# StarsX/FluidX12

Measured on AMD Instinct MI355X. Metric: voxel-updates/sec (advect+40 Jacobi) at 256^3; achieved HBM GB/s vs peak, higher is better.
Workload: dtype f32

## Files before the change

### fluidx12_amd/capi.py

```python
import ctypes as C
import os

from . import build as _build

FX_OK = 0
FX_E_INVALID, FX_E_DEVICE, FX_E_NOMEM, FX_E_STATE, FX_E_COMM, FX_E_HALO = -1, -2, -3, -4, -5, -6

RAY_MARCH_DIRECT, RAY_MARCH_CUBEMAP, SEPARATE_LIGHT_PASS, OPTIMIZED = 0, 1, 2, 3
FRAME_COUNT = 3
STORAGE_FP32, STORAGE_FP16 = 0, 1
JACOBI_FIXED, JACOBI_FAITHFUL = 0, 1
ADDRESS_CLAMP, ADDRESS_MIRROR = 0, 1
FLAG_JACOBI_FUSE_MASK, FLAG_NO_OVERLAP, FLAG_RENDER_ONLY = 0xF, 0x10, 0x20
OPT_OVERLAP, OPT_JACOBI_ROUND, OPT_ADAPTIVE_HALO, OPT_COUNT_SAMPLES, OPT_RENDER_ACCEL = 1, 2, 3, 4, 5
ABI_VERSION = 7
(FIELD_VELOCITY, FIELD_VELOCITY1, FIELD_COLOR, FIELD_COLOR_PREV, FIELD_PRESSURE, FIELD_DIVERGENCE,
 FIELD_LIGHTMAP, FIELD_CUBEMAP, FIELD_TARGET, FIELD_TARGET_FLOAT, FIELD_CUBE_DEPTH) = range(11)
DEPTH_DEVICE = 0x1
LIGHT_DIRECTIONAL, LIGHT_POINT = 0, 1
MAX_EMITTERS = 16
OBSTACLES_DEVICE = 0x1


class Desc(C.Structure):
    _fields_ = [("struct_size", C.c_uint32), ("grid_x", C.c_uint32), ("grid_y", C.c_uint32), ("grid_z", C.c_uint32),
                ("viewport_w", C.c_uint32), ("viewport_h", C.c_uint32), ("storage", C.c_uint32),
                ("jacobi_iters", C.c_uint32), ("jacobi_mode", C.c_uint32), ("advect_address", C.c_uint32),
                ("device", C.c_int32), ("slab_z0", C.c_uint32), ("slab_nz", C.c_uint32),
                ("halo_advect", C.c_uint32), ("halo_jacobi", C.c_uint32), ("flags", C.c_uint32)]


class FrameInfo(C.Structure):
    _fields_ = [("cube_lod", C.c_uint32), ("cube_size", C.c_uint32), ("ray_samples", C.c_uint32),
                ("visibility_mask", C.c_uint32), ("frame_parity", C.c_uint32), ("edge_pixels", C.c_float),
                ("time_step", C.c_float), ("world_view_proj_i", C.c_float * 16), ("screen_to_world", C.c_float * 16)]


class Light(C.Structure):
    _fields_ = [("struct_size", C.c_uint32), ("kind", C.c_uint32), ("position", C.c_float * 3), ("color", C.c_float * 4),
                ("ambient", C.c_float * 4)]


class Emitter(C.Structure):
    _fields_ = [("struct_size", C.c_uint32), ("flags", C.c_uint32), ("center", C.c_float * 3), ("radius", C.c_float),
                ("color_rate", C.c_float * 4), ("force", C.c_float * 3), ("swirl", C.c_float)]


class Timing(C.Structure):
    _fields_ = [("advect_ms", C.c_double), ("divergence_ms", C.c_double), ("jacobi_ms", C.c_double),
                ("project_ms", C.c_double), ("light_ms", C.c_double), ("view_ms", C.c_double),
                ("exchange_ms", C.c_double), ("steps", C.c_uint64), ("jacobi_launches", C.c_uint64),
                ("jacobi_sweeps", C.c_uint64), ("renders", C.c_uint64), ("resolve_ms", C.c_double),
                ("jacobi_main_ms", C.c_double), ("jacobi_main_launches", C.c_uint64), ("jacobi_main_sweeps", C.c_uint64),
                ("exchange_bytes", C.c_uint64), ("advect_halo_planes", C.c_uint64), ("chain_ms", C.c_double),
                ("freeze_solves", C.c_uint64), ("freeze_sweeps", C.c_uint64), ("exchange_calls", C.c_uint64),
                ("view_samples", C.c_uint64), ("light_samples", C.c_uint64), ("lightmap_fetches", C.c_uint64),
                ("freeze_strip_launches", C.c_uint64)]


_vp, _fp = C.c_void_p, C.POINTER(C.c_float)
SYMBOLS = {
    "fx_abi_version": (C.c_int, []),
    "fx_error_string": (C.c_char_p, [C.c_int]),
    "fx_create": (C.c_int, [C.POINTER(_vp), C.POINTER(Desc)]),
    "fx_destroy": (C.c_int, [_vp]),
    "fx_set_max_samples": (C.c_int, [_vp, C.c_uint32, C.c_uint32]),
    "fx_set_sh": (C.c_int, [_vp, _fp]),
    "fx_update_frame": (C.c_int, [_vp, C.c_float, C.c_uint8, _fp, _fp, _fp]),
    "fx_simulate": (C.c_int, [_vp, _vp, C.c_uint8]),
    "fx_render": (C.c_int, [_vp, _vp, C.c_uint8, C.c_uint8]),
    "fx_get_frame_info": (C.c_int, [_vp, C.POINTER(FrameInfo)]),
    "fx_synchronize": (C.c_int, [_vp]),
    "fx_last_error": (C.c_char_p, [_vp]),
    "fx_upload": (C.c_int, [_vp, C.c_int, _vp, C.c_size_t]),
    "fx_download": (C.c_int, [_vp, C.c_int, _vp, C.c_size_t]),
    "fx_field_bytes": (C.c_size_t, [_vp, C.c_int]),
    "fx_field_digest": (C.c_int, [_vp, C.c_int, C.c_uint32, C.c_uint32, C.POINTER(C.c_uint64)]),
    "fx_checkpoint_save": (C.c_int, [_vp, C.c_char_p]),
    "fx_checkpoint_load": (C.c_int, [_vp, C.c_char_p]),
    "fx_advect": (C.c_int, [_vp, _vp]),
    "fx_divergence": (C.c_int, [_vp, _vp]),
    "fx_jacobi": (C.c_int, [_vp, _vp, C.c_uint32]),
    "fx_project": (C.c_int, [_vp, _vp]),
    "fx_set_vorticity_confinement": (C.c_int, [_vp, C.c_float]),
    "fx_confine_vorticity": (C.c_int, [_vp, _vp]),
    "fx_set_emitters": (C.c_int, [_vp, C.POINTER(Emitter), C.c_uint32]),
    "fx_get_emitters": (C.c_int, [_vp, C.POINTER(Emitter), C.c_uint32, C.POINTER(C.c_uint32)]),
    "fx_set_impulse": (C.c_int, [_vp, C.c_int]),
    "fx_emit": (C.c_int, [_vp, _vp]),
    "fx_set_obstacles": (C.c_int, [_vp, _vp, _vp, C.c_size_t, C.c_uint32]),
    "fx_get_obstacles": (C.c_int, [_vp, _vp, C.c_size_t, C.POINTER(C.c_uint64)]),
    "fx_enforce_obstacles": (C.c_int, [_vp, _vp]),
    "fx_sh_transform": (C.c_int, [_vp, _fp, C.c_uint32, _fp]),
    "fx_set_environment": (C.c_int, [_vp, _fp, C.c_uint32]),
    "fx_render_environment": (C.c_int, [_vp, _vp, C.c_uint8]),
    "fx_clear_render_target": (C.c_int, [_vp, _vp, _fp]),
    "fx_render_cube": (C.c_int, [_vp, _vp, C.c_uint8]),
    "fx_set_scene_depth": (C.c_int, [_vp, _vp, _vp, C.c_uint32, C.c_uint32, C.c_float, C.c_float, C.c_uint32]),
    "fx_set_light": (C.c_int, [_vp, C.POINTER(Light)]),
    "fx_get_light": (C.c_int, [_vp, C.POINTER(Light)]),
    "fx_dds_cube_info": (C.c_int, [_vp, C.c_size_t, C.POINTER(C.c_uint32), C.POINTER(C.c_uint32)]),
    "fx_dds_decode_cube": (C.c_int, [_vp, _vp, C.c_size_t, C.c_uint32, _fp, C.c_size_t]),
    "fx_timing_enable": (C.c_int, [_vp, C.c_int]),
    "fx_set_option": (C.c_int, [_vp, C.c_uint32, C.c_uint32]),
    "fx_set_knob": (C.c_int, [C.c_char_p, C.c_char_p]),
    "fx_knob_name": (C.c_char_p, [C.c_uint32]),
    "fx_comm_gather_color": (C.c_int, [_vp, _vp, _vp, C.c_int, C.POINTER(C.c_uint32), C.POINTER(C.c_uint32)]),
    "fx_timing_read": (C.c_int, [_vp, C.POINTER(Timing), C.c_int]),
    "fx_comm_id_bytes": (C.c_size_t, []),
    "fx_comm_get_unique_id": (C.c_int, [_vp, C.c_size_t]),
    "fx_comm_init_rank": (C.c_int, [_vp, _vp, C.c_size_t, C.c_int, C.c_int]),
    "fx_comm_init_local": (C.c_int, [C.POINTER(_vp), C.c_int]),
    "fx_comm_init_peer": (C.c_int, [C.POINTER(_vp), C.c_int]),
}

_lib = None
LAB_KNOBS = {"ADVECT_BLOCK", "ADVECT_FAST", "ADVECT_LDS_HALF", "ADVECT_TILE_ROWS", "ADVECT_ZCHUNK", "BLOCK_REMAP", "BLOCK_SHAPE", "DEBUG_NO_COPY",
             "FREEZE_DENSE_LEVELS", "FREEZE_DENSE_ONE", "FREEZE_FAST", "FREEZE_FUSE_DIV", "FREEZE_NT", "FREEZE_SHRINK", "FREEZE_T", "FREEZE_WGS",
             "JACOBI2D_TILE", "JACOBI_BLOCK", "JACOBI_BLOCKG", "LIGHT_FILL_DIRTY", "LIGHT_RAY_NT", "LIGHT_RAY_WGS", "OBSTACLE_V4", "PROJECT_V4", "ROW_VW",
             "STRIP3H_PAIRS", "STRIP3_COOP", "STRIP3_NO512", "STRIP3_OFF", "STRIP3_ZCHUNK", "STRIP4T", "STRIP4T_256", "STRIP4T_512", "STRIP4T_FROM", "STRIP4T_GRID", "STRIP4T_NARROW", "STRIP4T_NARROW_FROM", "STRIP4T_PIECES", "STRIP4X", "STRIP4X_MINP", "STRIP4X_NT", "STRIP4X_ORDER", "STRIP4X_WGS",
             "STRIP4_OCTET", "STRIP4_ZCHUNK", "STRIP4_ZFLOOR", "STRIP_GENERIC", "STRIP_R", "STRIP_REMAP", "STRIP_WGS", "STRIP_WIDE", "STRIP_ZCHUNK", "VIEW_ORDER", "VIEW_WGS", "VORT_ZCHUNK", "XCD_REMAP"}


def lib_path():
    return _build.LIB


def load():
    global _lib
    if _lib is not None:
        return _lib
    try:
        import torch
    except Exception:
        pass
    path = _build.ensure_built()
    if os.environ.get("FLUIDX_LIB_PATH"):
        path = os.environ["FLUIDX_LIB_PATH"]
    if not os.path.exists(path):
        raise RuntimeError("libfluidx_hip.so is missing and could not be built")
    lib = C.CDLL(path, mode=C.RTLD_GLOBAL)
    lib.fx_abi_version.restype, lib.fx_abi_version.argtypes = C.c_int, []
    have = lib.fx_abi_version()
    if have != ABI_VERSION:
        raise RuntimeError("fluidx ABI version mismatch: %s speaks version %d, this harness version %d" % (path, have, ABI_VERSION))
    for name, (res, args) in SYMBOLS.items():
        fn = getattr(lib, name)
        fn.restype = res
        fn.argtypes = args
    _lib = lib
    offered = knob_names()
    for name in offered:
        v = os.environ.get("FLUIDX_" + name)
        if v is not None:
            set_knob(name, v)
    import sys
    for k in os.environ:
        if k.startswith("FLUIDX_") and k[7:] in LAB_KNOBS and k[7:] not in offered:
            sys.stderr.write("fluidx12_amd: %s is a lab-build switch (FLUIDX_BUILD_LAB=1 python -m fluidx12_amd.build); this library ignores it\n" % k)
    return lib


def knob_names():
    lib, out, i = load(), [], 0
    while True:
        n = lib.fx_knob_name(i)
        if n is None:
# ... 20 lines not shown
```

### fluidx12_amd/csrc/fx_advect_lds.hip

```cpp
#include "fx_internal.h"
#include <algorithm>
#include <cstdlib>
#include <cstdio>

namespace fx {

namespace {

constexpr int TX = 64;
constexpr int HX = TX + 2;
constexpr int NSLOT = 4;
template <bool HALF, int TY> struct Lay {
	static constexpr int NCELL = HX * (TY + 2);
	static constexpr int VEL_BYTES = NCELL * 4;
	static constexpr int COL_BYTES = HALF ? 2 * NCELL * 4 : NCELL * 16;
	static constexpr int SLOT_BYTES = COL_BYTES + 3 * VEL_BYTES;
};
typedef _Float16 h16;
typedef _Float16 h16x4 __attribute__((ext_vector_type(4)));
__device__ __forceinline__ h16 to_h16(float v) { asm("" : "+v"(v)); return (h16)v; }
__device__ __forceinline__ float lo_half(uint32_t d) { return (float)__builtin_bit_cast(h16, (uint16_t)(d & 0xffffu)); }
__device__ __forceinline__ float hi_half(uint32_t d) { return (float)__builtin_bit_cast(h16, (uint16_t)(d >> 16)); }

__device__ __forceinline__ float lerpf(float a, float b, float f) { return fmaf(f, b - a, a); }
__device__ __forceinline__ float saturatef(float x) { return fminf(fmaxf(x, 0.0f), 1.0f); }

__device__ __forceinline__ int addr_tap(int i, int n, int mode)
{
	if (mode == FX_ADDRESS_MIRROR) {
		const int period = 2 * n;
		int m = i % period;
		if (m < 0) m += period;
		return m < n ? m : period - 1 - m;
	}
	return min(max(i, 0), n - 1);
}

typedef __attribute__((address_space(3))) void lds_void;
typedef const __attribute__((address_space(1))) void glb_void;

template <int VEL_BYTES>
__device__ __forceinline__ void stage64(const void* col, const void* v0, const void* v1, const void* v2, uint32_t off_col, uint32_t off_vel, uint32_t lds_col, uint32_t lds_vel)
{
	uint32_t keep;
	lds_col = __builtin_amdgcn_readfirstlane(lds_col);
	lds_vel = __builtin_amdgcn_readfirstlane(lds_vel);
	asm volatile(
		"s_mov_b32 %0, m0\n\t"
		"s_mov_b32 m0, %7\n\t"
		"s_nop 0\n\t"
		"global_load_lds_dwordx4 %5, %1\n\t"
		"s_mov_b32 m0, %8\n\t"
		"s_nop 0\n\t"
		"global_load_lds_dword %6, %2\n\t"
		"s_add_u32 m0, m0, %9\n\t"
		"s_nop 0\n\t"
		"global_load_lds_dword %6, %3\n\t"
		"s_add_u32 m0, m0, %9\n\t"
		"s_nop 0\n\t"
		"global_load_lds_dword %6, %4\n\t"
		"s_mov_b32 m0, %0"
		: "=&s"(keep)
		: "s"(col), "s"(v0), "s"(v1), "s"(v2), "v"(off_col), "v"(off_vel), "s"(lds_col), "s"(lds_vel), "n"(VEL_BYTES)
		: "scc");
}

template <int VEL_BYTES>
__device__ __forceinline__ void stage64h(const void* col, const void* v0, const void* v1, const void* v2, uint32_t off_col, uint32_t off_vel, uint32_t lds_col, uint32_t lds_vel)
{
	uint32_t keep;
	lds_col = __builtin_amdgcn_readfirstlane(lds_col);
	lds_vel = __builtin_amdgcn_readfirstlane(lds_vel);
	const uint32_t off_col_hi = off_col + 4u;
	asm volatile(
		"s_mov_b32 %0, m0\n\t"
		"s_mov_b32 m0, %8\n\t"
		"s_nop 0\n\t"
		"global_load_lds_dword %5, %1\n\t"
		"s_add_u32 m0, m0, %10\n\t"
		"s_nop 0\n\t"
		"global_load_lds_dword %6, %1\n\t"
		"s_mov_b32 m0, %9\n\t"
		"s_nop 0\n\t"
		"global_load_lds_ushort %7, %2\n\t"
		"s_add_u32 m0, m0, %10\n\t"
		"s_nop 0\n\t"
		"global_load_lds_ushort %7, %3\n\t"
		"s_add_u32 m0, m0, %10\n\t"
		"s_nop 0\n\t"
		"global_load_lds_ushort %7, %4\n\t"
		"s_mov_b32 m0, %0"
		: "=&s"(keep)
		: "s"(col), "s"(v0), "s"(v1), "s"(v2), "v"(off_col), "v"(off_col_hi), "v"(off_vel), "s"(lds_col), "s"(lds_vel), "n"(VEL_BYTES)
		: "scc");
}

template <typename T>
__device__ __forceinline__ T ldg32(const void* base, uint32_t byte_off)
{
	return *reinterpret_cast<const T*>(static_cast<const char*>(base) + byte_off);
}


template <bool P2> __device__ __forceinline__ uint32_t rows(uint32_t y, int lgX, const Geom& g) { return P2 ? y << lgX : y * (uint32_t)g.X; }
template <bool P2> __device__ __forceinline__ uint32_t planes(uint32_t z, int lgP, const Geom& g) { return P2 ? z << lgP : z * ((uint32_t)g.X * (uint32_t)g.Y); }

template <bool HALF, bool P2>
__device__ __forceinline__ void advect_gather(const Geom& g, const SimParams& sp, int ix, int iy, int z0, int z1, bool z_present, float fx, float fy, float fz,
	const char* v0, const char* v1, const char* v2, const void* __restrict__ col_in, int lgX, int lgP, unsigned* halo_overflow, float (&u)[3], float (&c)[4])
{
	const int xa0 = addr_tap(ix, g.X, sp.address), xa1 = addr_tap(ix + 1, g.X, sp.address);
	const int ya0 = addr_tap(iy, g.Y, sp.address), ya1 = addr_tap(iy + 1, g.Y, sp.address);
	if (!z_present) {
		atomicOr(halo_overflow, 1u);
		z0 = min(max(z0, g.zlo), g.zhi);
		z1 = min(max(z1, g.zlo), g.zhi);
	}
	const uint32_t p0 = planes<P2>((uint32_t)g.lz(z0), lgP, g), p1 = planes<P2>((uint32_t)g.lz(z1), lgP, g);
	const uint32_t ry0 = rows<P2>((uint32_t)ya0, lgX, g), ry1 = rows<P2>((uint32_t)ya1, lgX, g);
	const uint32_t c000 = p0 + ry0 + (uint32_t)xa0, c100 = p0 + ry0 + (uint32_t)xa1;
	const uint32_t c010 = p0 + ry1 + (uint32_t)xa0, c110 = p0 + ry1 + (uint32_t)xa1;
	const uint32_t c001 = p1 + ry0 + (uint32_t)xa0, c101 = p1 + ry0 + (uint32_t)xa1;
	const uint32_t c011 = p1 + ry1 + (uint32_t)xa0, c111 = p1 + ry1 + (uint32_t)xa1;
	const char* vb[3] = { v0, v1, v2 };
	auto gv = [](const char* b, uint32_t cell) -> float { return HALF ? (float)ldg32<h16>(b, cell * 2u) : ldg32<float>(b, cell * 4u); };
	auto gc = [&](uint32_t cell) -> float4 {
		if (HALF) { const h16x4 h = ldg32<h16x4>(col_in, cell * 8u); return make_float4((float)h.x, (float)h.y, (float)h.z, (float)h.w); }
		return ldg32<float4>(col_in, cell * 16u);
	};
#pragma unroll
	for (int a = 0; a < 3; ++a) {
		const float c00 = lerpf(gv(vb[a], c000), gv(vb[a], c100), fx);
		const float c10 = lerpf(gv(vb[a], c010), gv(vb[a], c110), fx);
		const float c01 = lerpf(gv(vb[a], c001), gv(vb[a], c101), fx);
		const float c11 = lerpf(gv(vb[a], c011), gv(vb[a], c111), fx);
		u[a] = lerpf(lerpf(c00, c10, fy), lerpf(c01, c11, fy), fz);
	}
	const float4 t000 = gc(c000), t100 = gc(c100), t010 = gc(c010), t110 = gc(c110);
	const float4 t001 = gc(c001), t101 = gc(c101), t011 = gc(c011), t111 = gc(c111);
#define FX_TRI(m) lerpf(lerpf(lerpf(t000.m, t100.m, fx), lerpf(t010.m, t110.m, fx), fy), \
	lerpf(lerpf(t001.m, t101.m, fx), lerpf(t011.m, t111.m, fx), fy), fz)
	c[0] = FX_TRI(x); c[1] = FX_TRI(y); c[2] = FX_TRI(z); c[3] = FX_TRI(w);
#undef FX_TRI
}

template <bool HALF, bool ALPHA>
__device__ __forceinline__ void advect_finish(const SimParams& sp, float (&u)[3], float (&c)[4], float ex, float dx, float dz, float dt, float atten,
	uint32_t id, uint32_t stride, void* __restrict__ vel_out, void* __restrict__ col_out, float* __restrict__ alpha_out)
{
	if (__builtin_amdgcn_ballot_w64(sp.impulse && ex > -6.5f) != 0) {
		const float basis = exp2f(ex);
		if (basis >= 0.0183156393f) {
			float Fx, Fy, Fz;
			if (sp.is3d) {
				Fx = fmaf(basis, 0.0f, dz * -200.0f);
				Fy = fmaf(basis, 192.0f, 0.0f);
				Fz = fmaf(basis, 0.0f, dx * 200.0f);
			} else {
				Fx = 0.0f; Fy = basis * 48.0f; Fz = 0.0f;
			}
			u[0] = fmaf(Fx, dt, u[0]); u[1] = fmaf(Fy, dt, u[1]); u[2] = fmaf(Fz, dt, u[2]);
			const float bdt = basis * dt;
			c[0] = saturatef(fmaf(bdt, 8.0f, c[0]));
			c[1] = saturatef(fmaf(bdt, 16.0f, c[1]));
			c[2] = saturatef(fmaf(bdt, 40.0f, c[2]));
			c[3] = saturatef(fmaf(bdt, 40.0f, c[3]));
		}
	}
	char* vo = static_cast<char*>(vel_out);
	char* co = static_cast<char*>(col_out);
	if (HALF) {
		*reinterpret_cast<h16*>(vo + id * 2u) = to_h16(u[0] * atten);
		*reinterpret_cast<h16*>(vo + (stride + id) * 2u) = to_h16(u[1] * atten);
		*reinterpret_cast<h16*>(vo + (2u * stride + id) * 2u) = to_h16(u[2] * atten);
		h16x4 hc;
		hc.x = to_h16(c[0] * atten); hc.y = to_h16(c[1] * atten); hc.z = to_h16(c[2] * atten); hc.w = to_h16(c[3] * atten);
		*reinterpret_cast<h16x4*>(co + id * 8u) = hc;
		if (ALPHA) *reinterpret_cast<float*>(reinterpret_cast<char*>(alpha_out) + id * 4u) = (float)hc.w;
	} else {
		*reinterpret_cast<float*>(vo + id * 4u) = u[0] * atten;
		*reinterpret_cast<float*>(vo + (stride + id) * 4u) = u[1] * atten;
		*reinterpret_cast<float*>(vo + (2u * stride + id) * 4u) = u[2] * atten;
		*reinterpret_cast<float4*>(co + id * 16u) = make_float4(c[0] * atten, c[1] * atten, c[2] * atten, c[3] * atten);
		if (ALPHA) *reinterpret_cast<float*>(reinterpret_cast<char*>(alpha_out) + id * 4u) = c[3] * atten;
	}
}

}

template <bool HALF, int TY, bool DEFER, bool P2, bool ALPHA>
__global__ __launch_bounds__(64 * TY) __attribute__((amdgpu_waves_per_eu(4, 4))) void k_advect_lds(const Geom g, const SimParams sp,
	const void* __restrict__ vel_in, const void* __restrict__ col_in, void* __restrict__ vel_out, void* __restrict__ col_out, float* __restrict__ alpha_out,
	int z_begin, int nzp, int zchunk, int nchunks, unsigned* halo_overflow, float rX, float rY, float rZ, float inv_rr,
	int lgX, int lgY, int lg_gx, int lg_gy, uint32_t* __restrict__ far_list, uint32_t* __restrict__ far_flat, uint32_t* __restrict__ far_total, uint32_t far_cap)
{
	__shared__ uint32_t far_n, far_base;
	extern __shared__ __attribute__((aligned(16))) char lds[];

	const int tid = (int)threadIdx.x, lane = tid & 63, wave = __builtin_amdgcn_readfirstlane(tid >> 6);
	const int ntx = P2 ? 1 << lg_gx : lg_gx, nty = P2 ? 1 << lg_gy : lg_gy;
	const int ntiles = ntx * nty * nchunks;
	int tl = (int)blockIdx.x;
	{
		const int q = ntiles >> 3, r = ntiles & 7, xcd = tl & 7, j = tl >> 3;
		tl = xcd * q + min(xcd, r) + j;
	}
	const int tx = P2 ? tl & (ntx - 1) : tl % ntx, ty = P2 ? (tl >> lg_gx) & (nty - 1) : (tl / ntx) % nty, chunk = P2 ? tl >> (lg_gx + lg_gy) : tl / (ntx * nty);
	const int x0t = tx << 6, y0t = ty * TY;
	const int zb = z_begin + chunk * zchunk, ze = min(zb + zchunk, z_begin + nzp);
	if (zb >= ze) return;

	const int lgP = lgX + lgY;
	constexpr int COL_BYTES = Lay<HALF, TY>::COL_BYTES, SLOT_BYTES = Lay<HALF, TY>::SLOT_BYTES;
	constexpr int NCELL = Lay<HALF, TY>::NCELL, VEL_BYTES = Lay<HALF, TY>::VEL_BYTES, NT = 64 * TY;
	constexpr uint32_t ES = HALF ? 2 : 4, CS = HALF ? 8 : 16;
	const uint32_t stride = planes<P2>((uint32_t)g.nzl(), lgP, g);
	const char* v0 = reinterpret_cast<const char*>(vel_in);
	const char* v1 = v0 + (size_t)stride * ES;
	const char* v2 = v1 + (size_t)stride * ES;

	uint32_t src_a, src_b = 0;
	{
		const int c = tid, r = c / HX, cc = c - r * HX;
		src_a = rows<P2>((uint32_t)addr_tap(y0t - 1 + r, g.Y, sp.address), lgX, g) + (uint32_t)addr_tap(x0t - 1 + cc, g.X, sp.address);
	}
	const bool has_b = NT + tid < NCELL;
	if (has_b) {
		const int c = NT + tid, r = c / HX, cc = c - r * HX;
		src_b = rows<P2>((uint32_t)addr_tap(y0t - 1 + r, g.Y, sp.address), lgX, g) + (uint32_t)addr_tap(x0t - 1 + cc, g.X, sp.address);
	}
	const bool wave_has_b = NT + wave * 64 < NCELL;

	const uint32_t lds0 = (uint32_t)(size_t)(__attribute__((address_space(3))) char*)lds;
	auto fill = [&](int zq) {
		const int za = min(max(addr_tap(zq, g.Zg, sp.address), g.zlo), g.zhi);
		const size_t pz = planes<P2>((uint32_t)g.lz(za), lgP, g);
		const uint32_t slot = __builtin_amdgcn_readfirstlane(lds0 + (uint32_t)(((zq + 4) & 3) * SLOT_BYTES));
		const char* bc = reinterpret_cast<const char*>(col_in) + pz * CS;
		const char *b0 = v0 + pz * ES, *b1 = v1 + pz * ES, *b2 = v2 + pz * ES;
		if (HALF) stage64h<VEL_BYTES>(bc, b0, b1, b2, src_a * CS, src_a * ES, slot + (uint32_t)wave * (64 * 4), slot + COL_BYTES + (uint32_t)wave * (64 * 4));
		else stage64<VEL_BYTES>(bc, b0, b1, b2, src_a * CS, src_a * ES, slot + (uint32_t)wave * (64 * 16), slot + COL_BYTES + (uint32_t)wave * (64 * 4));
		if (wave_has_b) {
			if (has_b) {
				if (HALF) stage64h<VEL_BYTES>(bc, b0, b1, b2, src_b * CS, src_b * ES, slot + (NT + (uint32_t)wave * 64) * 4, slot + COL_BYTES + (NT + (uint32_t)wave * 64) * 4);
				else stage64<VEL_BYTES>(bc, b0, b1, b2, src_b * CS, src_b * ES, slot + (NT + (uint32_t)wave * 64) * 16, slot + COL_BYTES + (NT + (uint32_t)wave * 64) * 4);
			}
		}
	};

	if (DEFER && tid == 0) far_n = 0u;
	fill(zb - 1);
	fill(zb);
	fill(zb + 1);
	asm volatile("s_waitcnt vmcnt(0)" ::: "memory");
	__syncthreads();

	const int x = x0t + lane, y = y0t + wave;
	const bool has_voxel = P2 || (x < g.X && y < g.Y);
	const float dt = sp.dt;
	const float px = P2 ? ((float)x + 0.5f) * rX : ((float)x + 0.5f) / (float)g.X;
	const float py = P2 ? ((float)y + 0.5f) * rY : ((float)y + 0.5f) / (float)g.Y;
	const float dx = px + -0.5f, dy = py + -0.100000001f;
	const float dxy2 = fmaf(dy, dy, dx * dx);
	const uint32_t own = (uint32_t)((wave + 1) * HX + lane + 1);
	const float atten = fmaxf(fmaf(-dt, 0.200000003f, 1.0f), 0.0f);

	auto compute = [&](int z) {
		if (!has_voxel) return;
		const float pz = P2 ? ((float)z + 0.5f) * rZ : ((float)z + 0.5f) / (float)g.Zg;
		const float dz = pz + -0.5f;
		const float d2 = fmaf(dz, dz, dxy2);
		const float ex = ((d2 * -4.0f) * inv_rr) * 1.44269502f;

		const char* sc = lds + ((z + 4) & 3) * SLOT_BYTES;
		const uint32_t* vs = reinterpret_cast<const uint32_t*>(sc + COL_BYTES);
		auto vval = [](uint32_t d) -> float { return HALF ? lo_half(d) : __uint_as_float(d); };
		const float u0x = vval(vs[own]), u0y = vval(vs[NCELL + own]), u0z = vval(vs[2 * NCELL + own]);
		const float ax = fmaf(-u0x, dt, px), ay = fmaf(-u0y, dt, py), az = fmaf(-u0z, dt, pz);
		const float tx_ = ax * (float)g.X - 0.5f, ty_ = ay * (float)g.Y - 0.5f, tz_ = az * (float)g.Zg - 0.5f;
		const float flx = floorf(tx_), fly = floorf(ty_), flz = floorf(tz_);
		const float fx = tx_ - flx, fy = ty_ - fly, fz = tz_ - flz;
		const int ix = (int)flx, iy = (int)fly, iz = (int)flz;
		const int jx = ix - x, jy = iy - y, jz = iz - z;
		int z0 = addr_tap(iz, g.Zg, sp.address), z1 = addr_tap(iz + 1, g.Zg, sp.address);
		const bool z_present = z0 >= g.zlo && z0 <= g.zhi && z1 >= g.zlo && z1 <= g.zhi;
		const bool inwin = (unsigned)(jx + 1) <= 1u && (unsigned)(jy + 1) <= 1u && (unsigned)(jz + 1) <= 1u && z_present;

		float u[3], c[4];
		if (DEFER && !inwin) {
			const uint32_t slot = atomicAdd(&far_n, 1u);
			far_list[(size_t)blockIdx.x * far_cap + slot] = P2 ? (uint32_t)x | (uint32_t)y << lgX | (uint32_t)z << lgP
				: ((uint32_t)z * (uint32_t)g.Y + (uint32_t)y) * (uint32_t)g.X + (uint32_t)x;
		}
		if (DEFER || inwin) {
			const int kx = DEFER && !inwin ? 0 : jx, ky = DEFER && !inwin ? 0 : jy, kz = DEFER && !inwin ? z : iz;
			const uint32_t c0 = (uint32_t)((int)own + ky * HX + kx);
			const char* s0 = lds + ((kz + 4) & 3) * SLOT_BYTES;
			const char* s1 = lds + ((kz + 5) & 3) * SLOT_BYTES;
#pragma unroll
			for (int a = 0; a < 3; ++a) {
				const uint32_t* p0 = reinterpret_cast<const uint32_t*>(s0 + COL_BYTES + a * VEL_BYTES) + c0;
				const uint32_t* p1 = reinterpret_cast<const uint32_t*>(s1 + COL_BYTES + a * VEL_BYTES) + c0;
				const float c00 = lerpf(vval(p0[0]), vval(p0[1]), fx);
				const float c10 = lerpf(vval(p0[HX]), vval(p0[HX + 1]), fx);
				const float c01 = lerpf(vval(p1[0]), vval(p1[1]), fx);
				const float c11 = lerpf(vval(p1[HX]), vval(p1[HX + 1]), fx);
				u[a] = lerpf(lerpf(c00, c10, fy), lerpf(c01, c11, fy), fz);
			}
			float4 t000, t100, t010, t110, t001, t101, t011, t111;
			if (HALF) {
				auto tex = [](const char* slot, uint32_t c) -> float4 {
					const uint32_t rg = reinterpret_cast<const uint32_t*>(slot)[c], ba = reinterpret_cast<const uint32_t*>(slot)[NCELL + c];
					return make_float4(lo_half(rg), hi_half(rg), lo_half(ba), hi_half(ba));
				};
				t000 = tex(s0, c0); t100 = tex(s0, c0 + 1); t010 = tex(s0, c0 + HX); t110 = tex(s0, c0 + HX + 1);
				t001 = tex(s1, c0); t101 = tex(s1, c0 + 1); t011 = tex(s1, c0 + HX); t111 = tex(s1, c0 + HX + 1);
			} else {
				const float4* q0 = reinterpret_cast<const float4*>(s0) + c0;
				const float4* q1 = reinterpret_cast<const float4*>(s1) + c0;
				t000 = q0[0]; t100 = q0[1]; t010 = q0[HX]; t110 = q0[HX + 1];
				t001 = q1[0]; t101 = q1[1]; t011 = q1[HX]; t111 = q1[HX + 1];
			}
#define FX_TRI(m) lerpf(lerpf(lerpf(t000.m, t100.m, fx), lerpf(t010.m, t110.m, fx), fy), \
	lerpf(lerpf(t001.m, t101.m, fx), lerpf(t011.m, t111.m, fx), fy), fz)
			c[0] = FX_TRI(x); c[1] = FX_TRI(y); c[2] = FX_TRI(z); c[3] = FX_TRI(w);
#undef FX_TRI
		} else {
			advect_gather<HALF, P2>(g, sp, ix, iy, z0, z1, z_present, fx, fy, fz, v0, v1, v2, col_in, lgX, lgP, halo_overflow, u, c);
		}

		const uint32_t id = planes<P2>((uint32_t)g.lz(z), lgP, g) + rows<P2>((uint32_t)y, lgX, g) + (uint32_t)x;
		advect_finish<HALF, ALPHA>(sp, u, c, ex, dx, dz, dt, atten, id, stride, vel_out, col_out, alpha_out);
	};

	for (int z = zb; z < ze; ++z) {
		if (z + 2 <= ze) fill(z + 2);
		compute(z);
		if (!(P2 || y < g.Y)) asm volatile("s_waitcnt vmcnt(0)" ::: "memory");
		else if (ALPHA) asm volatile("s_waitcnt vmcnt(5)" ::: "memory");
		else asm volatile("s_waitcnt vmcnt(4)" ::: "memory");
		__syncthreads();
	}
	if (DEFER) {
		const uint32_t n = far_n;
		if (n != 0u) {
			if (tid == 0) far_base = atomicAdd(far_total, n);
			__syncthreads();
			const uint32_t base = far_base;
			const uint32_t* seg = far_list + (size_t)blockIdx.x * far_cap;
			for (uint32_t i = (uint32_t)tid; i < n; i += (uint32_t)NT) far_flat[base + i] = seg[i];
		}
	}
}

template <bool HALF, bool P2, bool ALPHA>
__global__ __launch_bounds__(256) void k_advect_far(const Geom g, const SimParams sp,
	const void* __restrict__ vel_in, const void* __restrict__ col_in, void* __restrict__ vel_out, void* __restrict__ col_out, float* __restrict__ alpha_out,
	const uint32_t* __restrict__ far_flat, const uint32_t* __restrict__ far_total, uint32_t* __restrict__ far_total_next, unsigned* halo_overflow,
	float rX, float rY, float rZ, float inv_rr, int lgX, int lgY)
{
	const uint32_t n = *far_total;
	if (blockIdx.x == 0 && threadIdx.x == 0) *far_total_next = 0u;
	const int lgP = lgX + lgY;
	constexpr uint32_t ES = HALF ? 2 : 4;
	const uint32_t stride = planes<P2>((uint32_t)g.nzl(), lgP, g);
	const char* v0 = reinterpret_cast<const char*>(vel_in);
	const char* v1 = v0 + (size_t)stride * ES;
	const char* v2 = v1 + (size_t)stride * ES;
	const float dt = sp.dt;
	const float atten = fmaxf(fmaf(-dt, 0.200000003f, 1.0f), 0.0f);
	for (uint32_t i = blockIdx.x * 256u + threadIdx.x; i < n; i += gridDim.x * 256u) {
		const uint32_t code = far_flat[i];
		int x, y, z;
		if (P2) { x = (int)(code & (uint32_t)(g.X - 1)); y = (int)((code >> lgX) & (uint32_t)(g.Y - 1)); z = (int)(code >> lgP); }
		else { const uint32_t XY = (uint32_t)g.X * (uint32_t)g.Y, rem = code % XY; z = (int)(code / XY); y = (int)(rem / (uint32_t)g.X); x = (int)(rem % (uint32_t)g.X); }
		const float px = P2 ? ((float)x + 0.5f) * rX : ((float)x + 0.5f) / (float)g.X;
		const float py = P2 ? ((float)y + 0.5f) * rY : ((float)y + 0.5f) / (float)g.Y;
		const float pz = P2 ? ((float)z + 0.5f) * rZ : ((float)z + 0.5f) / (float)g.Zg;
		const float dx = px + -0.5f, dy = py + -0.100000001f, dz = pz + -0.5f;
		const float dxy2 = fmaf(dy, dy, dx * dx);
		const float d2 = fmaf(dz, dz, dxy2);
		const float ex = ((d2 * -4.0f) * inv_rr) * 1.44269502f;
		const uint32_t id = planes<P2>((uint32_t)g.lz(z), lgP, g) + rows<P2>((uint32_t)y, lgX, g) + (uint32_t)x;
		auto gv = [](const char* b, uint32_t cell) -> float { return HALF ? (float)ldg32<h16>(b, cell * 2u) : ldg32<float>(b, cell * 4u); };
		const float u0x = gv(v0, id), u0y = gv(v1, id), u0z = gv(v2, id);
		const float ax = fmaf(-u0x, dt, px), ay = fmaf(-u0y, dt, py), az = fmaf(-u0z, dt, pz);
		const float tx_ = ax * (float)g.X - 0.5f, ty_ = ay * (float)g.Y - 0.5f, tz_ = az * (float)g.Zg - 0.5f;
		const float flx = floorf(tx_), fly = floorf(ty_), flz = floorf(tz_);
		const float fx = tx_ - flx, fy = ty_ - fly, fz = tz_ - flz;
		const int ix = (int)flx, iy = (int)fly, iz = (int)flz;
		const int z0 = addr_tap(iz, g.Zg, sp.address), z1 = addr_tap(iz + 1, g.Zg, sp.address);
		const bool z_present = z0 >= g.zlo && z0 <= g.zhi && z1 >= g.zlo && z1 <= g.zhi;
		float u[3], c[4];
		advect_gather<HALF, P2>(g, sp, ix, iy, z0, z1, z_present, fx, fy, fz, v0, v1, v2, col_in, lgX, lgP, halo_overflow, u, c);
		advect_finish<HALF, ALPHA>(sp, u, c, ex, dx, dz, dt, atten, id, stride, vel_out, col_out, alpha_out);
	}
}


hipError_t launch_advect_lds(const Geom& g, const SimParams& sp, int half_store, const void* vel_in, const void* col_in,
	void* vel_out, void* col_out, int z_begin, int z_end, unsigned* halo_overflow, uint32_t* far_scratch, size_t far_words, int far_parity, bool* far_used, hipStream_t s, bool force,
	AdvectAlpha* alpha)
{
	if (far_used) *far_used = false;
	if (alpha) alpha->written = false;
	auto pow2 = [](int v) { return v > 0 && (v & (v - 1)) == 0; };
	const int nzp = z_end - z_begin;
	const bool p2 = pow2(g.X) && pow2(g.Y) && pow2(g.Zg);
	const int TY = p2 && FX_KNOB_INT("ADVECT_TILE_ROWS", 8) == 16 ? 16 : 8;
	const size_t min_voxels = (size_t)1 << 22;
	if (g.Zg <= 1 || g.X < TX || g.Y < TY || nzp < 12 || (!force && (size_t)g.X * g.Y * (size_t)nzp < min_voxels) ||
		g.cells_local() * 16 >= ((size_t)1 << 32))
		return hipErrorNotSupported;
	const int half_on = FX_KNOB_INT("ADVECT_LDS_HALF", 1);
	if (half_store && !half_on) return hipErrorNotSupported;
	auto lg = [](int v) { int k = 0; while ((1 << k) < v) ++k; return k; };
	const int ntx = (g.X + TX - 1) / TX, nty = (g.Y + TY - 1) / TY;
	const int lgX = lg(g.X), lgY = lg(g.Y), lg_gx = p2 ? lg(ntx) : ntx, lg_gy = p2 ? lg(nty) : nty;
	const int tiles_xy = ntx * nty;
	const bool want_defer = far_scratch && FX_KNOB_INT("ADVECT_DEFER", 1) != 0;
	int zchunk = FX_KNOB_INT("ADVECT_ZCHUNK", want_defer ? 32 : 16);
	if (!p2 && !FX_KNOB("ADVECT_ZCHUNK")) {
		const int chunks = std::max(1, 512 / tiles_xy);
		zchunk = std::max(8, (nzp + chunks - 1) / chunks);
	}
	if (zchunk < 4) zchunk = 4;
	if (zchunk > nzp) zchunk = nzp;
	const int nchunks = (nzp + zchunk - 1) / zchunk;
	const float rX = 1.0f / (float)g.X, rY = 1.0f / (float)g.Y, rZ = 1.0f / (float)g.Zg, inv_rr = sp.is3d ? 256.0f : 1024.0f;
	const uint32_t nwg = (uint32_t)(tiles_xy * nchunks), far_cap = (uint32_t)(TX * TY * zchunk);
	const size_t flat_words = (size_t)g.X * g.Y * (size_t)nzp;
	const bool defer = want_defer && far_words >= 2 + flat_words + (size_t)nwg * far_cap && ((uint64_t)g.Zg << (lgX + lgY)) <= ((uint64_t)1 << 32);
	if (far_used) *far_used = defer;
	uint32_t* far_total = far_scratch ? far_scratch + (far_parity & 1) : nullptr;
	uint32_t* far_total_next = far_scratch ? far_scratch + ((far_parity & 1) ^ 1) : nullptr;
	uint32_t* far_flat = far_scratch ? far_scratch + 2 : nullptr;
	uint32_t* far_list = far_scratch ? far_scratch + 2 + flat_words : nullptr;
#define FX_ADV(H_, TY_, D_, P_, A_) do { \
		static bool attr_set = false; \
		if (!attr_set) { (void)hipFuncSetAttribute(reinterpret_cast<const void*>(k_advect_lds<H_, TY_, D_, P_, A_>), hipFuncAttributeMaxDynamicSharedMemorySize, NSLOT * Lay<H_, TY_>::SLOT_BYTES); attr_set = true; } \
		hipLaunchKernelGGL((k_advect_lds<H_, TY_, D_, P_, A_>), dim3(tiles_xy * nchunks), dim3(64 * TY_), (NSLOT * Lay<H_, TY_>::SLOT_BYTES), s, g, sp, vel_in, col_in, vel_out, col_out, alpha_out, \
			z_begin, nzp, zchunk, nchunks, halo_overflow, rX, rY, rZ, inv_rr, lgX, lgY, lg_gx, lg_gy, far_list, far_flat, far_total, far_cap); } while (0)
#define FX_FAR(H_, P_, A_) hipLaunchKernelGGL((k_advect_far<H_, P_, A_>), dim3(far_wgs), dim3(256), 0, s, g, sp, vel_in, col_in, vel_out, col_out, alpha_out, far_flat, far_total, far_total_next, halo_overflow, rX, rY, rZ, inv_rr, lgX, lgY)
	const int far_wgs = 1024;
	float* alpha_out = alpha && alpha->out && defer && TY == 8 && g.nzl() == g.Zg && z_begin == 0 && z_end == g.Zg ? alpha->out : nullptr;
	if (alpha_out) {
		if (half_store) { if (p2) { FX_ADV(true, 8, true, true, true); FX_FAR(true, true, true); } else { FX_ADV(true, 8, true, false, true); FX_FAR(true, false, true); } }
		else { if (p2) { FX_ADV(false, 8, true, true, true); FX_FAR(false, true, true); } else { FX_ADV(false, 8, true, false, true); FX_FAR(false, false, true); } }
		alpha->written = true;
	} else if (!p2) {
		if (defer) {
			if (half_store) { FX_ADV(true, 8, true, false, false); FX_FAR(true, false, false); } else { FX_ADV(false, 8, true, false, false); FX_FAR(false, false, false); }
		} else { if (half_store) FX_ADV(true, 8, false, false, false); else FX_ADV(false, 8, false, false, false); }
	} else if (defer) {
		if (TY == 16) { if (half_store) FX_ADV(true, 16, true, true, false); else FX_ADV(false, 16, true, true, false); }
		else { if (half_store) FX_ADV(true, 8, true, true, false); else FX_ADV(false, 8, true, true, false); }
		if (half_store) FX_FAR(true, true, false); else FX_FAR(false, true, false);
	} else {
		if (TY == 16) { if (half_store) FX_ADV(true, 16, false, true, false); else FX_ADV(false, 16, false, true, false); }
		else { if (half_store) FX_ADV(true, 8, false, true, false); else FX_ADV(false, 8, false, true, false); }
	}
#undef FX_FAR
#undef FX_ADV
	return hipGetLastError();
}

size_t advect_far_words(const Geom& g, int nzp)
{
	if (g.Zg <= 1 || g.X < TX || g.Y < 16 || nzp < 12) return 0;
	const size_t tiled = (size_t)((g.X + TX - 1) / TX * TX) * (size_t)((g.Y + 7) / 8 * 8);
	return 2 + (size_t)g.X * g.Y * (size_t)nzp + tiled * (size_t)(nzp + 32);
}

}
```

### fluidx12_amd/csrc/fx_api.cpp

```cpp
#include "fx_host.h"
#include <cstring>
#include "fx_hostmath.h"

using namespace fx;
using namespace fxh;

extern "C" {

int fx_abi_version(void) { return FX_ABI_VERSION; }

int fx_set_max_samples(fx_ctx* ctx, uint32_t max_ray, uint32_t max_light)
{
	if (!ctx || !max_ray || !max_light) return FX_E_INVALID;
	ctx->max_ray_samples = max_ray;
	ctx->max_light_samples = max_light;
	return FX_OK;
}

int fx_set_sh(fx_ctx* ctx, const float* coeffs27)
{
	if (!ctx) return FX_E_INVALID;
	if (!ctx->sh_dev) return FX_E_STATE;
	if (!coeffs27) { ctx->has_sh = false; return FX_OK; }
	DeviceGuard dg(ctx->device);
// ... 539 lines not shown
	if (!ctx || !out_cube) return FX_E_INVALID;
	DdsCube d;
	if (!dds_cube_layout(dds, bytes, &d) || mip >= d.mips) return FX_E_INVALID;
	const size_t* fo = d.face_offset; const size_t* mo = d.mip_offset;
	const uint32_t n = std::max<uint32_t>(d.size >> mip, 1), nb = (n + 3) / 4;
	const size_t face_floats = (size_t)n * n * 3, face_blocks = (size_t)nb * nb * 16;
	if (out_floats != 6 * face_floats) return FX_E_INVALID;
	if (d.kind != DDS_BC6H_UF16) {
		for (int f = 0; f < 6; ++f) dds_linear_face_to_rgb(static_cast<const char*>(dds) + fo[f] + mo[mip], d.kind, n, out_cube + f * face_floats);
		return FX_OK;
	}
	DeviceGuard dg(ctx->device);
	const size_t float_bytes = (6 * face_floats * 4 + 15) & ~(size_t)15;
	int rc = ensure_stage(ctx, float_bytes + 6 * face_blocks);
	if (rc) return rc;
	char* blocks_dev = reinterpret_cast<char*>(ctx->stage) + float_bytes;
	for (int f = 0; f < 6; ++f)
		FX_HIP(hipMemcpyAsync(blocks_dev + f * face_blocks, static_cast<const char*>(dds) + fo[f] + mo[mip], face_blocks, hipMemcpyHostToDevice, ctx->stream));
	for (int f = 0; f < 6; ++f)
		FX_HIP(launch_bc6h_decode(blocks_dev + f * face_blocks, (int)nb, (int)nb, (int)n, ctx->stage + f * face_floats, ctx->stream));
	FX_HIP(hipMemcpyAsync(out_cube, ctx->stage, 6 * face_floats * 4, hipMemcpyDeviceToHost, ctx->stream));
	FX_HIP(hipStreamSynchronize(ctx->stream));
	return FX_OK;
}

size_t fx_comm_id_bytes(void) { return rccl_id_bytes(); }

int fx_comm_get_unique_id(void* id_out, size_t bytes)
{
	if (!id_out) return FX_E_INVALID;
	std::string err;
	const int rc = rccl_get_unique_id(id_out, bytes, &err);
	if (rc) std::fprintf(stderr, "fluidx: %s\n", err.c_str());
	return rc;
}

static int check_slab_chain(fx_ctx* c, int rank, int nranks)
{
	if (nranks < 1 || rank < 0 || rank >= nranks) return FX_E_INVALID;
	if (c->group) return FX_E_STATE;
	if (nranks > 1 && c->g.nz == c->g.Zg) return FX_E_INVALID;
	if (rank == 0 && c->g.z0 != 0) return FX_E_INVALID;
	if (rank == nranks - 1 && c->g.z0 + c->g.nz != c->g.Zg) return FX_E_INVALID;
	return FX_OK;
}

static int make_lane(fx_comm_group* g, int device, hipStream_t compute)
{
	fx_lane l{};
	l.device = device;
	l.compute = compute;
	DeviceGuard dg(device);
	int lo = 0, hi = 0, prio = 0;
	const char* pe = FX_KNOB("COMM_PRIORITY");
	if (pe && pe[0] == '1' && hipDeviceGetStreamPriorityRange(&lo, &hi) == hipSuccess) prio = hi;
	bool ok = hipStreamCreateWithPriority(&l.comm, hipStreamNonBlocking, prio) == hipSuccess;
	ok = ok && hipStreamCreateWithFlags(&l.face, hipStreamNonBlocking) == hipSuccess;
	for (hipEvent_t* e : { &l.ev_ready, &l.ev_done, &l.ev_col_ready, &l.ev_col_done, &l.ev_int, &l.ev_face1, &l.x_ready, &l.x_done })
		ok = ok && hipEventCreateWithFlags(e, hipEventDisableTiming) == hipSuccess;
	g->lanes.push_back(l);
	return ok ? FX_OK : FX_E_DEVICE;
}

static int make_step_record(fx_ctx* ctx, int nrec, bool gathered)
{
	DeviceGuard dg(ctx->device);
	if (ctx->step_rec) return FX_OK;
	FX_HIP(hipMalloc((void**)&ctx->step_rec, 4 * sizeof(int)));
	FX_HIP(hipMemset(ctx->step_rec, 0, 4 * sizeof(int)));
	if (gathered) FX_HIP(hipMalloc((void**)&ctx->gath_dev, 4 * sizeof(int) * (size_t)nrec));
	FX_HIP(hipHostMalloc((void**)&ctx->rec_host, 4 * sizeof(int) * (size_t)nrec, hipHostMallocDefault));
	std::memset(ctx->rec_host, 0, 4 * sizeof(int) * (size_t)nrec);
	FX_HIP(hipEventCreateWithFlags(&ctx->rec_ev, hipEventDisableTiming));
	return FX_OK;
}

int fx_comm_init_rank(fx_ctx* ctx, const void* id, size_t bytes, int rank, int nranks)
{
	if (!ctx || !id) return FX_E_INVALID;
	int rc = check_slab_chain(ctx, rank, nranks);
	if (rc) return rc;
	Transport* t = make_rccl_transport(id, bytes, rank, nranks, ctx->device, &ctx->last_error);
	if (!t) { std::fprintf(stderr, "fluidx: %s\n", ctx->last_error.c_str()); return FX_E_COMM; }
	fx_comm_group* g = new fx_comm_group();
	g->members.push_back(ctx);
	g->transport = t;
	g->refs = 1;
	g->per_member = false; g->shared_stream = nullptr; g->broken = false;
	if ((rc = make_lane(g, ctx->device, nullptr))) { destroy_lanes(g); delete t; delete g; return rc; }
	if ((rc = t->min_over_ranks(ctx->g.nz, ctx->stream, &g->min_nz))) { destroy_lanes(g); delete t; delete g; return rc; }
	{
		const fx_desc& d = ctx->desc;
		uint32_t h = 2166136261u;
		for (uint32_t v : { d.grid_x, d.grid_y, d.grid_z, d.halo_advect, d.halo_jacobi, d.jacobi_iters, d.jacobi_mode, d.storage, d.advect_address, (uint32_t)nranks,
				d.flags & (FX_FLAG_NO_OVERLAP | FX_FLAG_JACOBI_FUSE_MASK), (uint32_t)ctx->opt_overlap, (uint32_t)ctx->opt_round, (uint32_t)ctx->opt_adaptive })
			h = (h ^ v) * 16777619u;
		const int digest = (int)(h & 0x3FFFFFFFu);
		int lo = 0, hi = 0;
		if ((rc = t->min_over_ranks(digest, ctx->stream, &lo)) || (rc = t->min_over_ranks(-digest, ctx->stream, &hi))) { destroy_lanes(g); delete t; delete g; return rc; }
		if (lo != digest || -hi != digest) {
			ctx->last_error = "fx_comm_init_rank: the ranks were created with different descriptors";
			std::fprintf(stderr, "fluidx: %s\n", ctx->last_error.c_str());
			destroy_lanes(g); delete t; delete g;
			return FX_E_INVALID;
		}
	}
	if (!ctx->step_rec && (rc = make_step_record(ctx, nranks, true))) { destroy_lanes(g); delete t; delete g; return rc; }
	{
		DeviceGuard dg(ctx->device);
		const int mine[4] = { ctx->g.z0, ctx->g.nz, 0, 0 };
		bool ok = hipMemcpy(ctx->step_rec, mine, sizeof mine, hipMemcpyHostToDevice) == hipSuccess &&
			t->allgather(ctx->step_rec, 4, ctx->gath_dev, ctx->stream) == FX_OK &&
			hipMemcpyAsync(ctx->rec_host, ctx->gath_dev, 4 * sizeof(int) * (size_t)nranks, hipMemcpyDeviceToHost, ctx->stream) == hipSuccess &&
			hipStreamSynchronize(ctx->stream) == hipSuccess;
		bool tiles = ok;
		for (int r = 0; ok && r + 1 < nranks; ++r) tiles = tiles && ctx->rec_host[4 * r] + ctx->rec_host[4 * r + 1] == ctx->rec_host[4 * (r + 1)];
		if (ok) ok = hipMemset(ctx->step_rec, 0, 4 * sizeof(int)) == hipSuccess;
		if (!ok || !tiles) {
			ctx->last_error = ok ? "fx_comm_init_rank: the slabs of the ranks do not tile the grid in rank order" : "fx_comm_init_rank: exchanging the slab ranges failed";
			std::fprintf(stderr, "fluidx: %s\n", ctx->last_error.c_str());
			destroy_lanes(g); delete t; delete g;
			return ok ? FX_E_INVALID : FX_E_COMM;
		}
	}
	ctx->group = g; ctx->rank = rank; ctx->nranks = nranks;
	return FX_OK;
}

int fx_comm_gather_color(fx_ctx* ctx, void* stream, fx_ctx* full, int root, const uint32_t* slab_z0, const uint32_t* slab_nz)
{
	if (!ctx || !ctx->group || root < 0 || root >= ctx->nranks) return FX_E_INVALID;
	if (group_broken(ctx)) return FX_E_STATE;
	if (!is_driver(ctx)) return FX_OK;
	const bool local = ctx->group->transport->is_local();
	const bool am_root = local || ctx->rank == root;
	if (am_root) {
		if (!full || full->g.X != ctx->g.X || full->g.Y != ctx->g.Y || full->g.Zg != ctx->g.Zg || full->g.nz != full->g.Zg ||
			full->half != ctx->half) return FX_E_INVALID;
		if (!local && full->device != ctx->device) return FX_E_INVALID;
		if (local && full->device != ctx->group->members[(size_t)root]->device) return FX_E_INVALID;
	}
	if (!local && (!slab_z0 || !slab_nz)) return FX_E_INVALID;
	const size_t plane_bytes = ctx->g.plane() * 4 * elem_size(ctx);
	std::vector<GatherPart> parts((size_t)ctx->nranks);
	for (int r = 0; r < ctx->nranks; ++r) {
		const fx_ctx* m = local ? ctx->group->members[r] : (r == ctx->rank ? ctx : nullptr);
		const uint32_t z0 = local ? (uint32_t)m->g.z0 : slab_z0[r], nz = local ? (uint32_t)m->g.nz : slab_nz[r];
		if (z0 > (uint32_t)ctx->g.Zg || nz > (uint32_t)ctx->g.Zg - z0) return FX_E_INVALID;
		if (!local && r == ctx->rank && (z0 != (uint32_t)ctx->g.z0 || nz != (uint32_t)ctx->g.nz)) return FX_E_INVALID;
		parts[r].rank = r;
		parts[r].bytes = (size_t)nz * plane_bytes;
		parts[r].src = m ? (const char*)m->col[m->frame_parity] + (size_t)m->g.H * plane_bytes : nullptr;
		parts[r].dst = am_root ? (char*)full->col[full->frame_parity] + (size_t)z0 * plane_bytes : nullptr;
		if (am_root) full->accel_alpha_of = nullptr;
	}
	DeviceGuard dg(ctx->device);
	hipStream_t s = pick_stream(ctx, stream);
	if (ctx->halo_fault) return FX_E_HALO;
	std::vector<hipStream_t> streams;
	if (ctx->group->per_member) for (fx_ctx* m : ctx->group->members) streams.push_back(m->stream);
	else streams.push_back(s);
	hipStream_t done_on = ctx->group->per_member ? streams[(size_t)root] : s;
	ScopedMark mk(ctx, s, MK_EXCH);
	int rc = ctx->group->transport->gather(ctx->group, parts, root, streams);
	if (rc) return rc;
	if (am_root && full->stream != done_on) {
		fx_lane& L = ctx->group->per_member ? ctx->group->lanes[(size_t)root] : ctx->group->lanes[0];
		DeviceGuard dgr(L.device);
		FX_HIP(hipEventRecord(L.ev_done, done_on));
		DeviceGuard dgf(full->device);
		FX_HIP(hipStreamWaitEvent(full->stream, L.ev_done, 0));
	}
	return FX_OK;
}

static int check_local_members(fx_ctx** ctxs, int nranks, bool one_device)
{
	if (!ctxs || nranks < 1) return FX_E_INVALID;
	int zexp = 0;
	for (int r = 0; r < nranks; ++r) {
		if (!ctxs[r]) return FX_E_INVALID;
		int rc = check_slab_chain(ctxs[r], r, nranks);
		if (rc) return rc;
		if (ctxs[r]->g.z0 != zexp || (one_device && ctxs[r]->device != ctxs[0]->device)) return FX_E_INVALID;
		const fx_desc &a = ctxs[r]->desc, &b = ctxs[0]->desc;
		if (a.grid_x != b.grid_x || a.grid_y != b.grid_y || a.grid_z != b.grid_z || a.halo_advect != b.halo_advect ||
			a.halo_jacobi != b.halo_jacobi || a.jacobi_iters != b.jacobi_iters || a.jacobi_mode != b.jacobi_mode ||
			a.storage != b.storage || a.advect_address != b.advect_address)
			return FX_E_INVALID;
		for (int q = 0; q < r; ++q) if (ctxs[q] == ctxs[r]) return FX_E_INVALID;
		zexp += ctxs[r]->g.nz;
	}
	return FX_OK;
}

static int init_in_process_group(fx_ctx** ctxs, int nranks, bool peer)
{
	int rc = check_local_members(ctxs, nranks, !peer);
	if (rc) return rc;
	if (peer) {
		for (int r = 0; r + 1 < nranks; ++r) {
			const int a = ctxs[r]->device, b = ctxs[r + 1]->device;
			if (a == b) continue;
			int ab = 0, ba = 0;
			if (hipDeviceCanAccessPeer(&ab, a, b) != hipSuccess || hipDeviceCanAccessPeer(&ba, b, a) != hipSuccess || !ab || !ba) {
				ctxs[0]->last_error = "fx_comm_init_peer: two neighbouring slabs live on devices without peer access";
				return FX_E_DEVICE;
			}
			for (int k = 0; k < 2; ++k) {
				DeviceGuard dg(k ? b : a);
				const hipError_t e = hipDeviceEnablePeerAccess(k ? a : b, 0);
				if (e != hipSuccess && e != hipErrorPeerAccessAlreadyEnabled) { (void)hipGetLastError(); return FX_E_DEVICE; }
				(void)hipGetLastError();
			}
		}
	}
	for (int r = 0; r < nranks; ++r)
		if (!ctxs[r]->step_rec) { if ((rc = make_step_record(ctxs[r], 1, false))) return rc; }
	fx_comm_group* g = new fx_comm_group();
	g->transport = make_local_transport();
	g->refs = nranks;
	g->per_member = peer; g->shared_stream = nullptr; g->broken = false;
	for (int r = 0; r < (peer ? nranks : 1); ++r)
		if ((rc = make_lane(g, ctxs[r]->device, peer ? ctxs[r]->stream : nullptr))) { destroy_lanes(g); delete g->transport; delete g; return rc; }
	g->min_nz = ctxs[0]->g.nz;
	for (int r = 1; r < nranks; ++r) g->min_nz = std::min(g->min_nz, ctxs[r]->g.nz);
	for (int r = 0; r < nranks; ++r) {
		g->members.push_back(ctxs[r]);
		ctxs[r]->group = g; ctxs[r]->rank = r; ctxs[r]->nranks = nranks;
		if (peer) continue;
		if (r > 0) {
			if (ctxs[r]->owns_stream) (void)hipStreamDestroy(ctxs[r]->stream);
			ctxs[r]->stream = ctxs[0]->stream;
		}
		ctxs[r]->owns_stream = false;
		g->shared_stream = ctxs[0]->stream;
	}
	return FX_OK;
}

int fx_comm_init_local(fx_ctx** ctxs, int nranks) { return init_in_process_group(ctxs, nranks, false); }
int fx_comm_init_peer(fx_ctx** ctxs, int nranks) { return init_in_process_group(ctxs, nranks, true); }

}
```

### fluidx12_amd/csrc/fx_context.cpp

```cpp
#include "fx_host.h"
#include <time.h>

using namespace fx;
using namespace fxh;

namespace fx {
bool digest_range_ok(const Geom& g, uint32_t z_begin, uint32_t z_count)
{
	if (!z_count) return true;
	if (g.nz < 0 || z_count > (uint32_t)g.nz) return false;
	const int64_t first = (int64_t)z_begin, end = first + (int64_t)z_count;
	return first >= (int64_t)g.z0 && end <= (int64_t)g.z0 + (int64_t)g.nz;
}
}

namespace fxh {

size_t ev_record(fx_ctx* c, hipStream_t s)
{
	if (c->ev_used == c->ev.size()) {
		hipEvent_t e;
		if (hipEventCreate(&e) != hipSuccess) return (size_t)-1;
		c->ev.push_back(e);
	}
	(void)hipEventRecord(c->ev[c->ev_used], s);
	return c->ev_used++;
}

int drain_timing(fx_ctx* c)
{
	for (const auto& m : c->marks) {
		float ms = 0.0f;
		if (hipEventSynchronize(c->ev[m.e1]) != hipSuccess) return FX_E_DEVICE;
		if (hipEventElapsedTime(&ms, c->ev[m.e0], c->ev[m.e1]) != hipSuccess) return FX_E_DEVICE;
		switch (m.kind) {
		case MK_ADVECT: c->acc.advect_ms += ms; break;
		case MK_DIV: c->acc.divergence_ms += ms; break;
		case MK_JACOBI: c->acc.jacobi_ms += ms; c->acc.jacobi_launches += m.launches; c->acc.jacobi_sweeps += m.sweeps;
			c->acc.jacobi_main_ms += ms; c->acc.jacobi_main_launches += m.launches; c->acc.jacobi_main_sweeps += m.sweeps; break;
		case MK_JACOBI_TAIL: c->acc.jacobi_ms += ms; c->acc.jacobi_launches += m.launches; c->acc.jacobi_sweeps += m.sweeps; break;
		case MK_PROJECT: c->acc.project_ms += ms; break;
		case MK_LIGHT: c->acc.light_ms += ms; break;
		case MK_VIEW: c->acc.view_ms += ms; break;
		case MK_EXCH: c->acc.exchange_ms += ms; break;
		case MK_RESOLVE: c->acc.resolve_ms += ms; break;
		case MK_CHAIN: c->acc.chain_ms += ms; break;
		}
	}
	c->marks.clear();
	c->ev_used = 0;
	return FX_OK;
}

int ensure_stage(fx_ctx* ctx, size_t bytes)
{
	if (ctx->stage_bytes >= bytes) return FX_OK;
	if (ctx->stage) { FX_HIP(hipFree(ctx->stage)); ctx->stage = nullptr; ctx->stage_bytes = 0; }
	FX_HIP(hipMalloc((void**)&ctx->stage, bytes));
	ctx->stage_bytes = bytes;
	return FX_OK;
}

void destroy_lanes(fx_comm_group* g)
{
	for (fx_lane& l : g->lanes) {
		DeviceGuard dg(l.device);
		if (l.comm) (void)hipStreamDestroy(l.comm);
		if (l.face) (void)hipStreamDestroy(l.face);
		for (hipEvent_t e : { l.ev_ready, l.ev_done, l.ev_col_ready, l.ev_col_done, l.ev_int, l.ev_face1, l.x_ready, l.x_done }) if (e) (void)hipEventDestroy(e);
	}
	g->lanes.clear();
}

void group_release(fx_comm_group* g)
{
	{
		DeviceGuard dg(g->lanes.empty() ? 0 : g->lanes[0].device);
		if (g->shared_stream) (void)hipStreamDestroy(g->shared_stream);
	}
	destroy_lanes(g);
	delete g->transport;
	delete g;
}

void free_all(fx_ctx* c)
{
	for (int i = 0; i < 2; ++i) {
		if (c->vel[i]) (void)hipFree(c->vel[i]);
		if (c->col[i]) (void)hipFree(c->col[i]);
		if (c->p[i]) (void)hipFree(c->p[i]);
	}
	void* others[] = { c->env, c->cube_depth, c->depth_own, c->accel.occ, c->accel.alpha, c->accel.bits, c->accel.list, c->accel.cells, c->accel.gi, c->accel.ctr, c->target, c->target_float, c->p_face[0], c->p_face[1], c->b, c->frozen, c->frozen_alt, c->lightmap, c->cube, c->sh_dev, c->halo_overflow, c->stage,
		c->sh_scratch[0], c->sh_scratch[1], c->sh_scratch[2], c->sh_scratch[3], c->p_aux, c->fz_mask[0], c->fz_mask[1], c->fz_mask[2], c->fz_tile_next, c->fz_stat, c->fz_list[0], c->fz_list[1], c->fz_counts, c->sample_counters, c->adv_far, c->obst_code, c->obst_spare, c->obst_stats };
	for (void* q : others) if (q) (void)hipFree(q);
	for (hipEvent_t e : c->ev) (void)hipEventDestroy(e);
	if (c->step_rec) (void)hipFree(c->step_rec);
	if (c->gath_dev) (void)hipFree(c->gath_dev);
	if (c->rec_host) (void)hipHostFree(c->rec_host);
	if (c->fz_active_host) (void)hipHostFree(c->fz_active_host);
	if (c->fz_active_ev) (void)hipEventDestroy(c->fz_active_ev);
	if (c->rec_ev) (void)hipEventDestroy(c->rec_ev);
	if (c->owns_stream && c->stream) (void)hipStreamDestroy(c->stream);
}

}

extern "C" {

const char* fx_error_string(int status)
{
	switch (status) {
	case FX_OK: return "ok";
	case FX_E_INVALID: return "invalid argument";
	case FX_E_DEVICE: return "HIP device/runtime error";
	case FX_E_NOMEM: return "out of memory";
	case FX_E_STATE: return "invalid call order";
	case FX_E_COMM: return "RCCL communication error";
	case FX_E_HALO: return "advection back-trace left the exchanged halo";
	default: return "unknown status";
	}
}

int fx_create(fx_ctx** out, const fx_desc* d)
{
	if (!out || !d || d->struct_size != sizeof(fx_desc)) return FX_E_INVALID;
	*out = nullptr;
	if (!d->grid_x || !d->grid_y || !d->grid_z) return FX_E_INVALID;
	if (d->grid_x != d->grid_y) return FX_E_INVALID;
	if (d->grid_x > 65535 || d->grid_z > 65535) return FX_E_INVALID;
	if (d->storage > FX_STORAGE_FP16 || d->jacobi_mode > FX_JACOBI_FAITHFUL || d->advect_address > FX_ADDRESS_MIRROR) return FX_E_INVALID;
	if (!d->jacobi_iters) return FX_E_INVALID;
	uint32_t z0 = d->slab_z0, nz = d->slab_nz ? d->slab_nz : d->grid_z;
	if (z0 + nz > d->grid_z) return FX_E_INVALID;
	const bool slab = nz != d->grid_z;

	int ndev = 0;
	if (hipGetDeviceCount(&ndev) != hipSuccess || ndev <= 0) return FX_E_DEVICE;
	int dev = d->device;
	if (dev < 0 && hipGetDevice(&dev) != hipSuccess) return FX_E_DEVICE;
	if (dev >= ndev) return FX_E_INVALID;

	fx_ctx* ctx = new (std::nothrow) fx_ctx();
	if (!ctx) return FX_E_NOMEM;
	ctx->desc = *d;
	ctx->desc.slab_z0 = z0; ctx->desc.slab_nz = nz;
	default_light(ctx);
	if (!ctx->desc.halo_advect) ctx->desc.halo_advect = kDefaultAdvectHalo;
	if (!ctx->desc.halo_jacobi) ctx->desc.halo_jacobi = kDefaultJacobiHalo;
	if (!slab) { ctx->desc.halo_advect = 0; }
	const int H = slab ? (int)std::max(ctx->desc.halo_advect, ctx->desc.halo_jacobi) : 0;
	if (slab && (int)nz < H) { delete ctx; return FX_E_INVALID; }
	if (slab && (d->flags & FX_FLAG_RENDER_ONLY)) { delete ctx; return FX_E_INVALID; }
	ctx->g = Geom{ (int)d->grid_x, (int)d->grid_y, (int)d->grid_z, (int)z0, (int)nz, H,
		std::max((int)z0 - H, 0), std::min((int)(z0 + nz) + H, (int)d->grid_z) - 1 };
	ctx->half = d->storage == FX_STORAGE_FP16;
	ctx->device = dev;
	ctx->max_ray_samples = 192; ctx->max_light_samples = 64;
	ctx->rank = 0; ctx->nranks = 1;
	ctx->opt_overlap = (d->flags & FX_FLAG_NO_OVERLAP) ? 0 : 2;
	ctx->opt_round = (int)ctx->desc.halo_jacobi;

	DeviceGuard dg(dev);
	if (!dg.ok) { delete ctx; return FX_E_DEVICE; }
	int rc = [&]() -> int {
		FX_HIP(hipStreamCreateWithFlags(&ctx->stream, hipStreamNonBlocking));
		ctx->owns_stream = true;
		const size_t cells = ctx->g.cells_local();
		const size_t es = elem_size(ctx);
		if (d->flags & FX_FLAG_RENDER_ONLY) {
			FX_HIP(hipMalloc(&ctx->col[0], 4 * cells * es));
			FX_HIP(hipMemsetAsync(ctx->col[0], 0, 4 * cells * es, ctx->stream));
		}
		for (int i = 0; i < 2 && !(d->flags & FX_FLAG_RENDER_ONLY); ++i) {
			FX_HIP(hipMalloc(&ctx->vel[i], 3 * cells * es));
			FX_HIP(hipMalloc(&ctx->col[i], 4 * cells * es));
			FX_HIP(hipMalloc((void**)&ctx->p[i], cells * 4));
			FX_HIP(hipMemsetAsync(ctx->vel[i], 0, 3 * cells * es, ctx->stream));
			FX_HIP(hipMemsetAsync(ctx->col[i], 0, 4 * cells * es, ctx->stream));
			FX_HIP(hipMemsetAsync(ctx->p[i], 0, cells * 4, ctx->stream));
		}
		if (slab && !(d->flags & FX_FLAG_RENDER_ONLY))
			for (int i = 0; i < 2; ++i) {
				FX_HIP(hipMalloc((void**)&ctx->p_face[i], cells * 4));
				FX_HIP(hipMemsetAsync(ctx->p_face[i], 0, cells * 4, ctx->stream));
			}
		if (!(d->flags & FX_FLAG_RENDER_ONLY)) {
			FX_HIP(hipMalloc((void**)&ctx->b, cells * 4));
			FX_HIP(hipMemsetAsync(ctx->b, 0, cells * 4, ctx->stream));
		}
		if (d->jacobi_mode == FX_JACOBI_FAITHFUL && !(d->flags & FX_FLAG_RENDER_ONLY)) {
			FX_HIP(hipMalloc((void**)&ctx->frozen, cells));
			FX_HIP(hipMemsetAsync(ctx->frozen, 0, cells, ctx->stream));
			if (ctx->g.Zg == 1) {
				FX_HIP(hipMalloc((void**)&ctx->frozen_alt, cells));
				FX_HIP(hipMemsetAsync(ctx->frozen_alt, 0, cells, ctx->stream));
			}
			if (jacobi_freeze_supported(ctx->g)) {
				const size_t mb = jacobi_freeze_mask_bytes(ctx->g), nt = (size_t)jacobi_freeze_tiles(ctx->g);
				FX_HIP(hipMalloc((void**)&ctx->p_aux, cells * 4));
				FX_HIP(hipMemsetAsync(ctx->p_aux, 0, cells * 4, ctx->stream));
				for (int i = 0; i < 3; ++i) {
					FX_HIP(hipMalloc((void**)&ctx->fz_mask[i], mb));
					FX_HIP(hipMemsetAsync(ctx->fz_mask[i], 0, mb, ctx->stream));
				}
				FX_HIP(hipMalloc((void**)&ctx->fz_tile_next, nt * sizeof(uint32_t)));
				FX_HIP(hipMemsetAsync(ctx->fz_tile_next, 0, nt * sizeof(uint32_t), ctx->stream));
				for (int i = 0; i < 2; ++i) FX_HIP(hipMalloc(&ctx->fz_list[i], jacobi_freeze_list_bytes(ctx->g)));
				FX_HIP(hipMalloc((void**)&ctx->fz_counts, 2 * jacobi_freeze_count_words() * sizeof(uint32_t)));
				FX_HIP(hipMemsetAsync(ctx->fz_counts, 0, 2 * jacobi_freeze_count_words() * sizeof(uint32_t), ctx->stream));
				FX_HIP(hipMalloc((void**)&ctx->fz_stat, kFreezeStatRing * sizeof(uint32_t)));
				FX_HIP(hipMemsetAsync(ctx->fz_stat, 0, kFreezeStatRing * sizeof(uint32_t), ctx->stream));
				ctx->fz_iters.assign(kFreezeStatRing, 0);
				if (jacobi_freeze_strip_supported(ctx->g) && hipHostMalloc((void**)&ctx->fz_active_host, 64, hipHostMallocMapped) == hipSuccess) {
					ctx->fz_active_host[0] = 0u;
					if (hipHostGetDevicePointer((void**)&ctx->fz_active_dev, ctx->fz_active_host, 0) != hipSuccess) ctx->fz_active_dev = nullptr;
				} else (void)hipGetLastError();
			}
		}
		FX_HIP(hipMalloc((void**)&ctx->halo_overflow, sizeof(unsigned)));
		FX_HIP(hipMemsetAsync(ctx->halo_overflow, 0, sizeof(unsigned), ctx->stream));
		if (!(d->flags & FX_FLAG_RENDER_ONLY)) {
			ctx->adv_far_tried = true;
			const size_t words = advect_far_words(ctx->g, ctx->g.nz);
			if (words) {
				if (hipMalloc((void**)&ctx->adv_far, words * sizeof(uint32_t)) == hipSuccess) {
					FX_HIP(hipMemsetAsync(ctx->adv_far, 0, 2 * sizeof(uint32_t), ctx->stream));
					ctx->adv_far_words = words;
				} else { (void)hipGetLastError(); ctx->adv_far = nullptr; }
			}
		}
		if (d->grid_z > 1) {
			FX_HIP(hipMalloc((void**)&ctx->lightmap, ctx->g.cells_owned() * 4));
			FX_HIP(hipMemsetAsync(ctx->lightmap, 0, ctx->g.cells_owned() * 4, ctx->stream));
			size_t off = 0;
			for (uint32_t m = 0; m < kNumMips; ++m) {
				ctx->cube_mip_offset[m] = off;
				const size_t sz = std::max<uint32_t>(d->grid_x >> m, 1);
				off += 6 * sz * sz * 4;
			}
			FX_HIP(hipMalloc((void**)&ctx->cube, off));
			FX_HIP(hipMemsetAsync(ctx->cube, 0, off, ctx->stream));
			if (d->viewport_w && d->viewport_h) {
				FX_HIP(hipMalloc((void**)&ctx->cube_depth, off));
				FX_HIP(hipMemsetD32Async((hipDeviceptr_t)ctx->cube_depth, 0x3f800000, off / 4, ctx->stream));
			}
			if (!slab && ctx->g.cells_owned() <= ((size_t)1 << 28) && ctx->g.X >= 4) {
				RenderAccel& A = ctx->accel;
				render_accel_layout(ctx->g, &A);
				const size_t ncell = (size_t)A.CX * A.CY * A.CZ, vox = ctx->g.cells_owned(), bw = render_accel_bits_words(A);
				FX_HIP(hipMalloc((void**)&A.occ, 2 * ncell * sizeof(float)));
				FX_HIP(hipMalloc((void**)&A.alpha, vox * sizeof(float)));
				FX_HIP(hipMalloc((void**)&A.bits, bw * sizeof(uint32_t)));
				FX_HIP(hipMemsetAsync(A.bits, 0, bw * sizeof(uint32_t), ctx->stream));
				FX_HIP(hipMalloc((void**)&A.list, vox * sizeof(uint32_t)));
				FX_HIP(hipMalloc((void**)&A.cells, ncell * sizeof(uint32_t)));
				FX_HIP(hipMalloc((void**)&A.ctr, render_accel_ctr_words(ctx->g) * sizeof(uint32_t)));
				FX_HIP(hipMemsetAsync(A.ctr, 0, render_accel_ctr_words(ctx->g) * sizeof(uint32_t), ctx->stream));
				ctx->accel_ok = true;
			}
			FX_HIP(hipMalloc((void**)&ctx->sh_dev, 27 * sizeof(float)));
			FX_HIP(hipMemsetAsync(ctx->sh_dev, 0, 27 * sizeof(float), ctx->stream));
		}
		FX_HIP(hipStreamSynchronize(ctx->stream));
		return FX_OK;
	}();
	if (rc != FX_OK) { free_all(ctx); delete ctx; return rc; }
	*out = ctx;
	return FX_OK;
}

int fx_destroy(fx_ctx* ctx)
{
	if (!ctx) return FX_E_INVALID;
	DeviceGuard dg(ctx->device);
	(void)hipDeviceSynchronize();
	if (ctx->group) {
		fx_comm_group* g = ctx->group;
		for (auto& m : g->members) if (m == ctx) m = nullptr;
		g->broken = true;
		if (--g->refs == 0) group_release(g);
	}
	free_all(ctx);
	delete ctx;
	return FX_OK;
}

static int halo_fault_status(fx_ctx* c)
{
	if (!c->halo_overflow) return FX_OK;
	unsigned flag = 0;
	if (hipMemcpy(&flag, c->halo_overflow, sizeof flag, hipMemcpyDeviceToHost) != hipSuccess) return FX_E_DEVICE;
	if (flag) c->halo_fault = true;
	return c->halo_fault ? FX_E_HALO : FX_OK;
}

static int wait_for_device(fx_ctx* c)
{
	Transport* t = c->group && c->group->transport && !c->group->transport->is_local() ? c->group->transport : nullptr;
	if (!t || !t->can_poll()) return hipDeviceSynchronize() == hipSuccess ? FX_OK : FX_E_DEVICE;
	std::vector<hipStream_t> streams{ c->stream, c->last_step_stream };
	for (const fx_lane& L : c->group->lanes) { streams.push_back(L.comm); streams.push_back(L.face); }
	std::vector<hipEvent_t> evs;
	int rc = FX_OK;
	for (hipStream_t s : streams) {
		if (!s) continue;
		hipEvent_t e;
		if (hipEventCreateWithFlags(&e, hipEventDisableTiming) != hipSuccess) { rc = FX_E_DEVICE; break; }
		evs.push_back(e);
		if (hipEventRecord(e, s) != hipSuccess) { rc = FX_E_DEVICE; break; }
	}
	for (size_t i = 0; i < evs.size() && rc == FX_OK;) {
		const hipError_t q = hipEventQuery(evs[i]);
		if (q == hipSuccess) { ++i; continue; }
		if (q != hipErrorNotReady) { rc = FX_E_DEVICE; break; }
		if ((rc = t->poll_error(&c->last_error))) break;
		struct timespec ts = { 0, 200000 };
		nanosleep(&ts, nullptr);
	}
	for (hipEvent_t e : evs) (void)hipEventDestroy(e);
	if (rc == FX_OK && (rc = t->poll_error(&c->last_error)) == FX_OK && hipDeviceSynchronize() != hipSuccess) rc = FX_E_DEVICE;
	return rc;
}

const char* fx_last_error(fx_ctx* ctx) { return ctx ? ctx->last_error.c_str() : ""; }

int fx_synchronize(fx_ctx* ctx)
{
	if (!ctx) return FX_E_INVALID;
	std::vector<fx_ctx*> M;
	for_members(ctx, M);
	int rc = FX_OK;
	for (fx_ctx* c : M) {
		DeviceGuard dg(c->device);
		if (const int w = wait_for_device(c)) return w;
		unsigned f3 = 0, f4 = 0;
		if (strip3_fault_take(&f3) != hipSuccess || strip4_fault_take(&f4) != hipSuccess) return FX_E_DEVICE;
		if (f3 | f4) {
			c->last_error = f4 ? "k_jacobi_strip4o / k_freeze_strip4o: an LDS hand-over wait ran out (pressure field invalid)"
			                   : "k_jacobi_strip3c / k_jacobi_strip3h: an LDS hand-over wait ran out (pressure field invalid)";
			return FX_E_DEVICE;
		}
		const int st = halo_fault_status(c);
		if (st == FX_E_DEVICE) return st;
		if (st == FX_E_HALO) {
			(void)hipMemset(c->halo_overflow, 0, sizeof(unsigned));
			(void)hipDeviceSynchronize();
			c->halo_fault = false;
			rc = FX_E_HALO;
		}
	}
	return rc;
}

static int field_info(fx_ctx* c, int field, size_t* host_bytes)
{
	const size_t n = c->g.cells_owned();
	switch (field) {
	case FX_FIELD_VELOCITY: case FX_FIELD_VELOCITY1: if (!c->vel[0]) return FX_E_STATE; *host_bytes = 3 * n * 4; return FX_OK;
	case FX_FIELD_COLOR_PREV: if (!c->col[1]) return FX_E_STATE;
	case FX_FIELD_COLOR: *host_bytes = 4 * n * 4; return FX_OK;
	case FX_FIELD_PRESSURE: case FX_FIELD_DIVERGENCE: if (!c->b) return FX_E_STATE; *host_bytes = n * 4; return FX_OK;
	case FX_FIELD_LIGHTMAP: if (!c->lightmap) return FX_E_INVALID; *host_bytes = 3 * n * 4; return FX_OK;
	case FX_FIELD_CUBEMAP: {
		if (!c->cube) return FX_E_INVALID;
		const size_t s = (size_t)c->g.X >> c->cube_lod;
		*host_bytes = 6 * s * s * 4;
		return FX_OK;
	}
	case FX_FIELD_CUBE_DEPTH: {
		if (!c->cube_depth) return FX_E_INVALID;
		const size_t s = (size_t)c->g.X >> c->cube_lod;
		*host_bytes = 6 * s * s * 4;
		return FX_OK;
	}
	case FX_FIELD_TARGET: case FX_FIELD_TARGET_FLOAT:
		if (!c->target) return FX_E_STATE;
		*host_bytes = (size_t)c->desc.viewport_w * c->desc.viewport_h * (field == FX_FIELD_TARGET ? 4 : 16);
		return FX_OK;
	}
	return FX_E_INVALID;
}

size_t fx_field_bytes(fx_ctx* ctx, int field)
{
	size_t b = 0;
	if (!ctx || field_info(ctx, field, &b) != FX_OK) return 0;
	return b;
}

int fx_field_digest(fx_ctx* ctx, int field, uint32_t z_begin, uint32_t z_count, uint64_t out[2])
{
	if (!ctx || !out) return FX_E_INVALID;
	size_t need = 0;
	int rc = field_info(ctx, field, &need);
	if (rc) return rc;
	if (field > FX_FIELD_DIVERGENCE) return FX_E_INVALID;
	const Geom& g = ctx->g;
	if (!digest_range_ok(g, z_begin, z_count)) return FX_E_INVALID;
	if (!z_count) { z_begin = (uint32_t)g.z0; z_count = (uint32_t)g.nz; }
	DeviceGuard dg(ctx->device);
	FX_HIP(hipDeviceSynchronize());
	if ((rc = halo_fault_status(ctx))) return rc;
	if ((rc = ensure_stage(ctx, 16))) return rc;
	unsigned long long* acc = reinterpret_cast<unsigned long long*>(ctx->stage);
	FX_HIP(hipMemsetAsync(acc, 0, 16, ctx->stream));
	const size_t plane = g.plane(), cl = g.cells_local(), first = (size_t)g.lz((int)z_begin) * plane, n = (size_t)z_count * plane;
	const size_t es = elem_size(ctx);
	const unsigned long long gfirst = (unsigned long long)z_begin * plane, gcells = (unsigned long long)g.Zg * plane;
	switch (field) {
	case FX_FIELD_VELOCITY: case FX_FIELD_VELOCITY1: {
		const char* src = (const char*)ctx->vel[field == FX_FIELD_VELOCITY1];
		for (int a = 0; a < 3; ++a) FX_HIP(launch_digest(src + (a * cl + first) * es, n, (int)es, a * gcells + gfirst, acc, ctx->stream));
		break;
	}
	case FX_FIELD_COLOR: case FX_FIELD_COLOR_PREV: {
		const char* src = (const char*)ctx->col[field == FX_FIELD_COLOR ? ctx->frame_parity : 1 - ctx->frame_parity];
		FX_HIP(launch_digest(src + first * 4 * es, 4 * n, (int)es, 4 * gfirst, acc, ctx->stream));
		break;
	}
	case FX_FIELD_PRESSURE: FX_HIP(launch_digest(ctx->p[ctx->p_cur] + first, n, 4, gfirst, acc, ctx->stream)); break;
	default: FX_HIP(launch_digest(ctx->b + first, n, 4, gfirst, acc, ctx->stream)); break;
	}
	FX_HIP(hipStreamSynchronize(ctx->stream));
	FX_HIP(hipMemcpy(out, acc, 16, hipMemcpyDeviceToHost));
	return FX_OK;
}

int fx_upload(fx_ctx* ctx, int field, const void* host, size_t bytes)
{
	if (!ctx || !host) return FX_E_INVALID;
	size_t need = 0;
	int rc = field_info(ctx, field, &need);
	if (rc) return rc;
	if (bytes != need) return FX_E_INVALID;
	DeviceGuard dg(ctx->device);
	FX_HIP(hipDeviceSynchronize());
	if (field <= FX_FIELD_DIVERGENCE) { ctx->fz_dense_n = 0; ctx->fz_active_pending = false; }
	const size_t n = ctx->g.cells_owned(), off = (size_t)ctx->g.H * ctx->g.plane(), cl = ctx->g.cells_local();
	const size_t es = elem_size(ctx);
	switch (field) {
	case FX_FIELD_VELOCITY: case FX_FIELD_VELOCITY1: {
		if (field == FX_FIELD_VELOCITY && ctx->group) {
			if (!ctx->group->transport->is_local() && ctx->opt_adaptive && ctx->rec_pending && !ctx->collective_upload) return FX_E_STATE;
			ctx->need_valid = false;
		}
		char* dst = (char*)ctx->vel[field == FX_FIELD_VELOCITY1];
		if ((rc = ensure_stage(ctx, need))) return rc;
		FX_HIP(hipMemcpy(ctx->stage, host, need, hipMemcpyHostToDevice));
		for (int a = 0; a < 3; ++a)
			FX_HIP(launch_to_storage(ctx->stage + a * n, dst + (a * cl + off) * es, n, ctx->half, ctx->stream));
		break;
	}
	case FX_FIELD_COLOR: case FX_FIELD_COLOR_PREV: {
		if (ctx->col_halo_buf >= 0 && ctx->group) {
			if (!ctx->group->transport->is_local() && !ctx->collective_upload) return FX_E_STATE;
			if (ctx->group->transport->is_local()) { for (fx_ctx* m : ctx->group->members) if (m) m->col_halo_buf = -1; }
			else ctx->col_halo_buf = -1;
		}
		char* dst = (char*)ctx->col[field == FX_FIELD_COLOR ? ctx->frame_parity : 1 - ctx->frame_parity];
		if (ctx->accel_alpha_of == dst) ctx->accel_alpha_of = nullptr;
		if ((rc = ensure_stage(ctx, need))) return rc;
		FX_HIP(hipMemcpy(ctx->stage, host, need, hipMemcpyHostToDevice));
		FX_HIP(launch_to_storage(ctx->stage, dst + off * 4 * es, 4 * n, ctx->half, ctx->stream));
		break;
	}
	case FX_FIELD_PRESSURE:
		FX_HIP(hipMemcpy(ctx->p[ctx->p_cur] + off, host, need, hipMemcpyHostToDevice));
		break;
	case FX_FIELD_DIVERGENCE:
		FX_HIP(hipMemcpy(ctx->b + off, host, need, hipMemcpyHostToDevice));
		break;
	case FX_FIELD_CUBEMAP:
		FX_HIP(hipMemcpy(ctx->cube + ctx->cube_mip_offset[ctx->cube_lod], host, need, hipMemcpyHostToDevice));
		ctx->cube_depth_on[ctx->cube_lod] = false;
		break;
	default:
		return FX_E_INVALID;
	}
	FX_HIP(hipStreamSynchronize(ctx->stream));
	return FX_OK;
}

int fx_download(fx_ctx* ctx, int field, void* host, size_t bytes)
{
	if (!ctx || !host) return FX_E_INVALID;
	size_t need = 0;
	int rc = field_info(ctx, field, &need);
	if (rc) return rc;
	if (bytes != need) return FX_E_INVALID;
	DeviceGuard dg(ctx->device);
	FX_HIP(hipDeviceSynchronize());
	if (field <= FX_FIELD_DIVERGENCE && (rc = halo_fault_status(ctx))) return rc;
	const size_t n = ctx->g.cells_owned(), off = (size_t)ctx->g.H * ctx->g.plane(), cl = ctx->g.cells_local();
	const size_t es = elem_size(ctx);
	switch (field) {
	case FX_FIELD_VELOCITY: case FX_FIELD_VELOCITY1: {
		const char* src = (const char*)ctx->vel[field == FX_FIELD_VELOCITY1];
		if ((rc = ensure_stage(ctx, need))) return rc;
		for (int a = 0; a < 3; ++a)
			FX_HIP(launch_from_storage(src + (a * cl + off) * es, ctx->stage + a * n, n, ctx->half, ctx->stream));
		FX_HIP(hipStreamSynchronize(ctx->stream));
		FX_HIP(hipMemcpy(host, ctx->stage, need, hipMemcpyDeviceToHost));
		break;
	}
	case FX_FIELD_COLOR: case FX_FIELD_COLOR_PREV: {
		const char* src = (const char*)ctx->col[field == FX_FIELD_COLOR ? ctx->frame_parity : 1 - ctx->frame_parity];
		if ((rc = ensure_stage(ctx, need))) return rc;
		FX_HIP(launch_from_storage(src + off * 4 * es, ctx->stage, 4 * n, ctx->half, ctx->stream));
		FX_HIP(hipStreamSynchronize(ctx->stream));
		FX_HIP(hipMemcpy(host, ctx->stage, need, hipMemcpyDeviceToHost));
		break;
	}
	case FX_FIELD_PRESSURE:
		FX_HIP(hipMemcpy(host, ctx->p[ctx->p_cur] + off, need, hipMemcpyDeviceToHost));
		break;
	case FX_FIELD_DIVERGENCE:
		FX_HIP(hipMemcpy(host, ctx->b + off, need, hipMemcpyDeviceToHost));
		break;
	case FX_FIELD_LIGHTMAP:
		if ((rc = ensure_stage(ctx, need))) return rc;
		FX_HIP(launch_lightmap_decode(ctx->lightmap, ctx->stage, n, ctx->stream));
		FX_HIP(hipStreamSynchronize(ctx->stream));
		FX_HIP(hipMemcpy(host, ctx->stage, need, hipMemcpyDeviceToHost));
		break;
	case FX_FIELD_CUBEMAP:
		FX_HIP(hipMemcpy(host, ctx->cube + ctx->cube_mip_offset[ctx->cube_lod], need, hipMemcpyDeviceToHost));
		break;
	case FX_FIELD_CUBE_DEPTH:
		FX_HIP(hipMemcpy(host, (const char*)ctx->cube_depth + ctx->cube_mip_offset[ctx->cube_lod], need, hipMemcpyDeviceToHost));
		break;
	case FX_FIELD_TARGET:
		FX_HIP(hipMemcpy(host, ctx->target, need, hipMemcpyDeviceToHost));
		break;
	case FX_FIELD_TARGET_FLOAT:
		FX_HIP(hipMemcpy(host, ctx->target_float, need, hipMemcpyDeviceToHost));
		break;
	default:
		return FX_E_INVALID;
	}
	return FX_OK;
}

int fx_timing_enable(fx_ctx* ctx, int enable)
{
	if (!ctx) return FX_E_INVALID;
	std::vector<fx_ctx*> M;
	for_members(ctx, M);
	for (fx_ctx* c : M) {
		c->timing_on = enable != 0;
		if (enable) {
			DeviceGuard dg(c->device);
			while (c->ev.size() < 4096) {
				hipEvent_t e;
				if (hipEventCreate(&e) != hipSuccess) return FX_E_DEVICE;
				c->ev.push_back(e);
			}
		}
	}
	return FX_OK;
}

int fx_timing_read(fx_ctx* ctx, fx_timing* out, int reset)
{
	if (!ctx || !out) return FX_E_INVALID;
	DeviceGuard dg(ctx->device);
	int rc = drain_timing(ctx);
	if (rc) return rc;
	if (ctx->sample_counters) {
		unsigned long long h[kSampleShards * 3];
		FX_HIP(hipDeviceSynchronize());
		FX_HIP(hipMemcpy(h, ctx->sample_counters, sizeof h, hipMemcpyDeviceToHost));
		FX_HIP(hipMemset(ctx->sample_counters, 0, sizeof h));
		for (int i = 0; i < kSampleShards; ++i) { ctx->acc.view_samples += h[3 * i]; ctx->acc.light_samples += h[3 * i + 1]; ctx->acc.lightmap_fetches += h[3 * i + 2]; }
	}
	*out = ctx->acc;
	if (ctx->fz_stat && ctx->fz_gen > ctx->fz_gen_mark) {
		std::vector<uint32_t> ring(kFreezeStatRing);
		FX_HIP(hipDeviceSynchronize());
		FX_HIP(hipMemcpy(ring.data(), ctx->fz_stat, kFreezeStatRing * sizeof(uint32_t), hipMemcpyDeviceToHost));
		const uint32_t first = std::max(ctx->fz_gen_mark + 1, ctx->fz_gen >= kFreezeStatRing ? ctx->fz_gen - kFreezeStatRing + 1 : 1u);
		for (uint32_t gtag = first; gtag <= ctx->fz_gen; ++gtag) {
			const uint32_t w = ring[gtag % kFreezeStatRing], lvl = (w >> 8) == gtag ? (w & 0xFFu) : 0u;
			out->freeze_sweeps += std::min(ctx->fz_iters[gtag % kFreezeStatRing], 1u + lvl);
			out->freeze_solves += 1;
		}
	}
	if (reset) { std::memset(&ctx->acc, 0, sizeof ctx->acc); ctx->fz_gen_mark = ctx->fz_gen; }
	return FX_OK;
}

int fx_set_option(fx_ctx* ctx, uint32_t option, uint32_t value)
{
	if (!ctx) return FX_E_INVALID;
	int* slot = nullptr;
	switch (option) {
	case FX_OPT_OVERLAP: if (value > 3) return FX_E_INVALID; slot = &ctx->opt_overlap; break;
	case FX_OPT_JACOBI_ROUND: if (value < 1 || value > ctx->desc.halo_jacobi) return FX_E_INVALID; slot = &ctx->opt_round; break;
	case FX_OPT_ADAPTIVE_HALO: if (value > 1) return FX_E_INVALID; slot = &ctx->opt_adaptive; break;
	case FX_OPT_RENDER_ACCEL:
		if (value > 1) return FX_E_INVALID;
		ctx->opt_render_accel = (int)value;
		return FX_OK;
	case FX_OPT_COUNT_SAMPLES: {
		if (value > 1) return FX_E_INVALID;
		DeviceGuard dgc(ctx->device);
		if (value && !ctx->sample_counters) {
			FX_HIP(hipMalloc((void**)&ctx->sample_counters, kSampleShards * 3 * sizeof(unsigned long long)));
			FX_HIP(hipMemset(ctx->sample_counters, 0, kSampleShards * 3 * sizeof(unsigned long long)));
		}
		ctx->opt_count_samples = (int)value;
		return FX_OK;
	}
	default: return FX_E_INVALID;
	}
	if (ctx->group && !ctx->group->transport->is_local() && ctx->nranks > 1) {
		DeviceGuard dg(ctx->device);
		const int key = (int)(((option & 0xFu) << 8) | (value & 0xFFu));
		int lo = 0, hi = 0, rc;
		if ((rc = ctx->group->transport->min_over_ranks(key, ctx->stream, &lo)) || (rc = ctx->group->transport->min_over_ranks(-key, ctx->stream, &hi))) return rc;
		if (lo != key || -hi != key) {
			ctx->last_error = "fx_set_option: the ranks of the chain asked for different options";
			return FX_E_INVALID;
		}
	}
	*slot = (int)value;
	if (option == FX_OPT_ADAPTIVE_HALO) {
		std::vector<fx_ctx*> M;
		for_members(ctx, M);
		for (fx_ctx* m : M) { m->need_valid = false; if (m != ctx) m->opt_adaptive = (int)value; }
	}
	return FX_OK;
}

}
```

### fluidx12_amd/csrc/fx_context.h

```cpp
#pragma once
#include "fx_internal.h"
#include <vector>
#include <string>

struct fx_comm_group;
struct fx_lane;

struct fx_ctx {
	fx_desc desc;
	fx::Geom g;
	int half;
	int device;
	hipStream_t stream;
	bool owns_stream;

	void* vel[2];
	void* col[2];
	float* p[2];
	int p_cur;
	float* p_face[2];
	float* b;
	uint8_t* frozen;
	uint8_t* frozen_alt = nullptr;
	float* p_aux = nullptr;
	uint32_t* fz_active_host = nullptr;
	uint32_t* fz_active_dev = nullptr;
	hipEvent_t fz_active_ev = nullptr;
	bool fz_active_pending = false;
	int fz_dense_n = 0;
	uint8_t* fz_mask[3] = { nullptr, nullptr, nullptr };
	uint32_t* fz_tile_next = nullptr;
	void* fz_list[2] = { nullptr, nullptr };
	uint32_t* fz_counts = nullptr;
	uint32_t* fz_stat = nullptr;
	float* fz_x_p = nullptr;
	uint8_t* fz_x_m = nullptr;
	bool fz_fuse_div = false;
	uint32_t* adv_far = nullptr;
	bool adv_far_tried = false;
	size_t adv_far_words = 0;
	uint32_t adv_far_turn = 0;
	uint32_t fz_gen = 0;
	uint32_t fz_gen_mark = 0;
	std::vector<uint32_t> fz_iters;
	uint32_t* lightmap;
	uint8_t* cube;
	size_t cube_mip_offset[5];
	float* cube_depth;
	bool cube_depth_on[5];
	const float* depth;
	float* depth_own;
	float depth_zn, depth_zf;
	float vort_eps = 0.0f;
	std::vector<fx_emitter> emitters;
	bool impulse_on = true;
	uint8_t* obst_code = nullptr;
	uint8_t* obst_spare = nullptr;
	unsigned* obst_stats = nullptr;
	uint64_t obst_cells = 0;
	int obst_lo[3] = { 0, 0, 0 }, obst_hi[3] = { 0, 0, 0 };
	uint32_t light_kind = 0;
	float wvp[16];
	float* env;
	uint32_t env_n;
	fx::RenderAccel accel = {};
	bool accel_ok = false;
	const void* accel_alpha_of = nullptr;
	bool rendered_since_step = false;
	bool lightmap_filled = false;
	float lightmap_key[9] = {};
	hipStream_t last_step_stream = nullptr;
	hipStream_t rendered_on = nullptr;
	int opt_render_accel = 1;
	uint8_t* target;
	float* target_float;
	float* sh_dev;
	bool has_sh;
	unsigned* halo_overflow;
	float* stage;
	size_t stage_bytes;
	float* sh_scratch[4];
	size_t sh_scratch_n;

	uint32_t max_ray_samples, max_light_samples;
	uint32_t ray_samples, cube_lod, visibility_mask;
	uint8_t frame_parity;
	float time_step;
	float edge_pixels;
	bool frame_valid, view_valid;
	fx::FrameConsts fc;

	bool timing_on;
	std::vector<hipEvent_t> ev;
	size_t ev_used;
	struct Mark { int kind; size_t e0, e1; uint64_t launches, sweeps; };
	std::vector<Mark> marks;
	fx_timing acc;

	fx_comm_group* group;
	int rank, nranks;
	int opt_overlap;
	int opt_round;
	int opt_count_samples = 0;
	unsigned long long* sample_counters = nullptr;
	std::string last_error;
	int col_halo_buf = -1;
	uint64_t steps_simulated = 0;
	int* step_rec = nullptr;
	int* gath_dev = nullptr;
	int* rec_host = nullptr;
	hipEvent_t rec_ev = nullptr;
	bool rec_pending = false;
	bool need_valid = false;
	float rec_dt = 0.0f;
	int opt_adaptive = 1;
	int adv_w_lo = 0, adv_w_hi = 0;
	bool halo_fault = false;
	bool collective_upload = false;
	bool rec_in_project = false;
};

namespace fx {

struct ExchItem { char* base; size_t plane_bytes; int ncomp; int k; char* recv_base; int k_lo = -1, k_hi = -1; };

struct Seg { char* send; char* recv; size_t bytes; int dir; };

struct GatherPart { int rank; const char* src; char* dst; size_t bytes; };

struct Transport {
	virtual ~Transport() {}
	virtual int exchange(fx_comm_group* grp, const std::vector<std::vector<Seg>>& segs, const std::vector<hipStream_t>& streams, int channel = 0) = 0;
	virtual int gather(fx_comm_group* grp, const std::vector<GatherPart>& parts, int root, const std::vector<hipStream_t>& streams) = 0;
	virtual bool is_local() const = 0;
	virtual int min_over_ranks(int v, hipStream_t s, int* out) = 0;
	virtual int allgather(const int* send_dev, int count, int* recv_dev, hipStream_t s) = 0;
	virtual int poll_error(std::string* err) { (void)err; return FX_OK; }
	virtual bool can_poll() const { return false; }
};

}

struct fx_lane {
	int device;
	hipStream_t compute;
	hipStream_t comm;
	hipEvent_t ev_ready, ev_done;
	hipStream_t face;
	hipEvent_t ev_col_ready, ev_col_done;
	hipEvent_t ev_int, ev_face1;
	hipEvent_t x_ready, x_done;
};

struct fx_comm_group {
	std::vector<fx_ctx*> members;
	fx::Transport* transport;
	int refs;
	std::vector<fx_lane> lanes;
	bool per_member;
	int min_nz;
	hipStream_t shared_stream;
	bool broken;
	fx_lane& lane_of(const fx_ctx* m);
};

inline fx_lane& fx_comm_group::lane_of(const fx_ctx* m) { return per_member ? lanes[(size_t)m->rank] : lanes[0]; }

namespace fx {
enum ExchSet {
	EX_ADVECT_IN = 0,
	EX_UZ1 = 1,
	EX_DIV = 2,
	EX_PRESSURE = 3,
	EX_PRESSURE_FACE = 4,
	EX_ADVECT_VEL = 5,
	EX_COLOR_CUR = 6,
	EX_FREEZE = 7
};
int exchange_items(fx_ctx* c, int which_set, int k, int pidx, ExchItem out[4]);
void halo_segments(const fx_ctx* c, const ExchItem* items, int n, std::vector<Seg>& out);
Transport* make_local_transport();
Transport* make_rccl_transport(const void* id, size_t bytes, int rank, int nranks, int device, std::string* err);
size_t rccl_id_bytes();
int rccl_get_unique_id(void* out, size_t bytes, std::string* err);
}
```

### fluidx12_amd/csrc/fx_internal.h

```cpp
#pragma once
#include <hip/hip_runtime.h>
#include <stdint.h>
#include <stddef.h>
#include "../../include/fluidx_hip.h"
#include "fx_knobs.h"

namespace fx {

struct Geom {
	int X, Y;
	int Zg;
	int z0;
	int nz;
	int H;
	int zlo, zhi;
	__host__ __device__ size_t plane() const { return (size_t)X * Y; }
	__host__ __device__ int nzl() const { return nz + 2 * H; }
	__host__ __device__ size_t cells_local() const { return plane() * (size_t)nzl(); }
	__host__ __device__ size_t cells_owned() const { return plane() * (size_t)nz; }
	__host__ __device__ int lz(int z) const { return z - z0 + H; }
};

struct FrameConsts {
	float world_i[12];
	float world[12];
	float eye_pt[3];
	float light_pt[3];
	float light_color[4];
	float ambient[4];
	float wvp_i[16];
	float s2w[16];
};

struct DepthArgs {
	const float* depth;
	int W, H;
	float wvp[16];
	float z_near, z_far;
	float* cube_depth;
};

struct SimParams {
	float dt;
	int address;
	int is3d;
	int impulse = 1;
};

struct AdvectAlpha { float* out; bool written; };
hipError_t launch_advect(const Geom& g, const SimParams& sp, int half_store, const void* vel_in, const void* col_in,
	void* vel_out, void* col_out, int z_begin, int z_end, unsigned* halo_overflow, hipStream_t s, uint32_t* far_scratch = nullptr, size_t far_words = 0, int far_parity = 0, bool* far_used = nullptr,
	AdvectAlpha* alpha = nullptr);
hipError_t launch_advect_lds(const Geom& g, const SimParams& sp, int half_store, const void* vel_in, const void* col_in,
	void* vel_out, void* col_out, int z_begin, int z_end, unsigned* halo_overflow, uint32_t* far_scratch, size_t far_words, int far_parity, bool* far_used, hipStream_t s, bool force,
	AdvectAlpha* alpha = nullptr);
size_t advect_far_words(const Geom& g, int nzp);
hipError_t launch_confine_vorticity(const Geom& g, int half_store, const void* vel_in, void* vel_out, float eps, float dt, hipStream_t s);
const int kEmitTileX = 64, kEmitTileY = 4;
struct EmitBall { float c[3], rr, rate[4], force[3], swirl; int lo[3], hi[3]; };
struct EmitArgs { int n, x0, y0, z0, tiles_x, tiles_y, tiles_z; EmitBall e[FX_MAX_EMITTERS]; };
int emit_plan(const Geom& g, const fx_emitter* list, int count, EmitArgs* out);
hipError_t launch_emit(const Geom& g, int half_store, void* vel, void* col, float* alpha, const fx_emitter* list, int count, float dt, hipStream_t s);
hipError_t launch_divergence(const Geom& g, int half_store, const void* vel, float* b, int z_begin, int z_end, hipStream_t s);
hipError_t launch_obstacle_codes(const Geom& g, const uint8_t* solid_dev, uint8_t* code, unsigned* stats_dev, hipStream_t s);
hipError_t launch_obstacle_mask(const uint8_t* code, uint8_t* solid_dev, size_t n, hipStream_t s);
long long obstacle_enforce_tiles(const int lo[3], const int hi[3], int* x0, int* y0, int* tiles_x, int* tiles_y);
hipError_t launch_obstacle_enforce(const Geom& g, int half_store, const uint8_t* code, const int lo[3], const int hi[3], void* vel, void* col,
	float* alpha, hipStream_t s);
hipError_t launch_divergence_obs(const Geom& g, int half_store, const void* vel, const uint8_t* code, float* b, int z_begin, int z_end, hipStream_t s);
bool jacobi_obs_takes_v4(const Geom& g);
hipError_t launch_jacobi_obs(const Geom& g, const float* p_in, const float* b, const uint8_t* code, float* p_out, int z_begin, int z_end, hipStream_t s);
hipError_t launch_project_obs(const Geom& g, const SimParams& sp, int half_store, const void* vel_in, const float* p, const uint8_t* code,
	void* vel_out, int z_begin, int z_end, hipStream_t s);
enum SimStage { SIM_DIVERGENCE = 0, SIM_PROJECT = 1 };
enum SimRowKernel { ROW_SCALAR = 0, ROW_V4 = 4, ROW_VW2 = 2, ROW_VW3 = 3 };
int sim_row_kernel(const Geom& g, int half_store, int stage, int is3d);
bool digest_range_ok(const Geom& g, uint32_t z_begin, uint32_t z_count);
hipError_t launch_jacobi_sweep(const Geom& g, const float* p_in, const float* b, float* p_out, uint8_t* frozen,
	int z_begin, int z_end, hipStream_t s);
hipError_t launch_jacobi_sweep2(const Geom& g, const float* p_in, const float* b, float* p_out, uint8_t* frozen,
	int z_begin, int z_end, int z_begin2, int z_end2, hipStream_t s);
bool jacobi_strip_supported(const Geom& g);
bool jacobi_strip_wide(const Geom& g);
hipError_t launch_jacobi_strip(const Geom& g, const float* p_in, const float* b, float* p_out, int sweeps, int z_begin, int z_end, hipStream_t s);
bool jacobi_strip3_supported(const Geom& g);
hipError_t launch_jacobi_strip3(const Geom& g, const float* p_in, const float* b, float* p_out, int z_begin, int z_end, hipStream_t s);
bool jacobi_strip4_supported(const Geom& g);
hipError_t launch_jacobi_strip4(const Geom& g, const float* p_in, const float* b, float* p_out, int z_begin, int z_end, hipStream_t s);
bool jacobi_block2_supported(const Geom& g);
hipError_t launch_jacobi_block2(const Geom& g, const float* p_in, const float* b, float* p_out, int z_begin, int z_end, hipStream_t s);
bool jacobi_blockg_supported(const Geom& g);
hipError_t launch_jacobi_blockg(const Geom& g, const float* p_in, const float* b, float* p_out, int z_begin, int z_end, hipStream_t s);
bool jacobi_freeze_supported(const Geom& g);
int jacobi_freeze_tiles(const Geom& g);
size_t jacobi_freeze_mask_bytes(const Geom& g);
size_t jacobi_freeze_list_bytes(const Geom& g);
const int kFreezeSlots = 128;
size_t jacobi_freeze_count_words();
int jacobi_freeze_levels_per_launch();
struct FreezeWork { uint32_t* tile_mark; uint32_t gen; void* list[2]; int cap; uint32_t* counts; uint32_t* counts_next; };
Geom jacobi_freeze_view(const Geom& g, int* first_plane, int* own_begin);
hipError_t launch_freeze_dense(const Geom& g, const float* p_in, const float* b, float* pA, float* pB, uint8_t* mA, uint8_t* mB,
	const FreezeWork& w, hipStream_t s, const void* vel = nullptr, int vel_half = 0, int z_begin = 0, int nzp = 0, size_t vel_comp_cells = 0);
bool jacobi_freeze_can_fuse_divergence(const Geom& g);
hipError_t launch_freeze_tiles(const Geom& g, const float* p_src, const float* b, float* p_dst, const uint8_t* m_src, uint8_t* m_dst,
	const FreezeWork& w, int n, int levels, int level_base, uint32_t* stat, uint32_t stat_hi, hipStream_t s, int z_begin = 0, int nzp = 0, uint32_t flag_tag = 0);
bool jacobi_freeze_strip_supported(const Geom& g);
hipError_t launch_count_marks(const uint32_t* tile_mark, uint32_t gen, int ntiles, uint32_t* out, hipStream_t s);
hipError_t launch_freeze_strip3(const Geom& g, const float* p_in, const float* b, float* p_outA, float* p_outB, const uint8_t* m_in, uint8_t* m_outA, uint8_t* m_outB,
	uint32_t* tile_mark, uint32_t tag, uint32_t* stat, uint32_t stat_hi, int level_in, hipStream_t s);
bool jacobi_freeze_strip4_supported(const Geom& g);
hipError_t launch_freeze_strip4(const Geom& g, const float* p_in, const float* b, float* p_outA, float* p_outB, const uint8_t* m_in, uint8_t* m_outA, uint8_t* m_outB,
	uint32_t* tile_mark, uint32_t tag, uint32_t* stat, uint32_t stat_hi, int level_in, hipStream_t s);
int jacobi2d_max_sweeps(const Geom& g);
hipError_t launch_jacobi2d(const Geom& g, const float* p_in, const float* b, float* p_out, const uint8_t* frozen_in, uint8_t* frozen_out, int sweeps, hipStream_t s);
enum JacobiFamily { JF_NONE = 0, JF_SWEEP1, JF_TILE2D, JF_STRIP, JF_STRIP3, JF_STRIP4, JF_BLOCK2, JF_BLOCKG };
struct JacobiLaunch { int family, sweeps; };
struct JacobiPolicy { int fam[5]; int unit, three, four; };
JacobiPolicy jacobi_policy(const Geom& g, int fuse, bool frozen, bool second_mask);
int jacobi_plan(const JacobiPolicy& p, int n, JacobiLaunch* out);
hipError_t launch_jacobi(const Geom& g, JacobiLaunch l, const float* p_in, const float* b, float* p_out, uint8_t* frozen, uint8_t* frozen_out,
	int z_begin, int z_end, hipStream_t s);
int jacobi_group_sweeps(const JacobiPolicy* p, int n);
int jacobi_group_parts(const JacobiPolicy& lead, int t, int cnt, int* parts);
const int kFreezeHalo = 4;
bool freeze_takes_sparse_solver(const Geom& g, uint32_t iters, bool masks, bool slab, int min_nz);
enum FreezeKind { FZ_DENSE = 0, FZ_DENSE_ONE, FZ_STRIP, FZ_TILES };
struct FreezeLaunch { int kind, levels, base; };
int freeze_plan(const Geom& g, uint32_t iters, bool slab, bool third_mask, int strips_in_use, FreezeLaunch* out);
int freeze_strip_width(const Geom& g, bool slab, bool third_mask, int* forced);
struct FreezeCadence { bool count, take_over; };
FreezeCadence freeze_cadence(uint32_t gen);
int freeze_strip_hysteresis(int n, uint32_t active, uint32_t tiles, bool four);
hipError_t launch_digest(const void* v, size_t count, int elem_bytes, unsigned long long key0, unsigned long long* out, hipStream_t s);
hipError_t strip3_fault_take(unsigned* out);
hipError_t strip4_fault_take(unsigned* out);
hipError_t launch_project(const Geom& g, const SimParams& sp, int half_store, const void* vel_in, const float* p,
	void* vel_out, int z_begin, int z_end, hipStream_t s, int* rec = nullptr, int digest = 0, const unsigned* halo_overflow = nullptr,
	bool* rec_done = nullptr);
hipError_t launch_face_need(const Geom& g, int half_store, const void* vel, float dt, int address, int digest, const unsigned* halo_overflow, int* rec, hipStream_t s);
hipError_t launch_copy_bytes(void* dst, const void* src, size_t bytes, hipStream_t s);
hipError_t launch_copy_velocity(const Geom& g, int half_store, const void* vel_in, void* vel_out, hipStream_t s);

hipError_t launch_to_storage(const float* src, void* dst, size_t n, int half_store, hipStream_t s);
hipError_t launch_from_storage(const void* src, float* dst, size_t n, int half_store, hipStream_t s);

const int kSampleShards = 64;
hipError_t launch_raymarch_light(const Geom& g, int half_store, const void* color, uint32_t* lightmap,
	const FrameConsts& fc, const float* sh, uint32_t num_samples, hipStream_t s, unsigned long long* counters = nullptr, int point_light = 0);
hipError_t launch_raymarch_view(const Geom& g, int half_store, const void* color, const uint32_t* lightmap,
	const FrameConsts& fc, const float* sh, int cube_size, uint32_t mask, uint32_t num_samples,
	uint32_t num_light_samples, int separate, uint8_t* cube, hipStream_t s, unsigned long long* counters = nullptr, const DepthArgs* depth = nullptr, int point_light = 0);
hipError_t launch_raycast_direct(const Geom& g, int half_store, const void* color, const uint32_t* lightmap,
	const FrameConsts& fc, const float* sh, int W, int H, uint32_t num_samples, uint32_t num_light_samples, int separate,
	uint8_t* target, float* out_float, hipStream_t s, unsigned long long* counters = nullptr, const DepthArgs* depth = nullptr, int point_light = 0);
struct RenderAccel {
	float* occ;
	float* alpha;
	uint32_t* bits;
	uint32_t* list;
	float* gi;
	uint32_t* cells;
	uint32_t* ctr;
	int CX, CY, CZ;
	int msh, MX, MY, MZ;
	uint32_t fine_words, mask_words;
	uint32_t frame;
	uint32_t fill_frame;
};
void render_accel_layout(const Geom& g, RenderAccel* a);
size_t render_accel_bits_words(const RenderAccel& a);
size_t render_accel_ctr_words(const Geom& g);
struct LightFill { uint32_t* lightmap; const FrameConsts* fc; int has_sh; bool incremental; };
hipError_t launch_accel_build(const Geom& g, int half_store, const void* color, const RenderAccel& a, hipStream_t s, bool alpha_current = false,
	const LightFill* fill = nullptr, bool* filled = nullptr);
hipError_t launch_accel_light(const Geom& g, const RenderAccel& a, uint32_t* lightmap, const FrameConsts& fc, const float* sh,
	uint32_t num_samples, hipStream_t s, unsigned long long* counters = nullptr, bool filled = false, int point_light = 0);
hipError_t launch_accel_view(const Geom& g, int half_store, const void* color, const uint32_t* lightmap, const FrameConsts& fc, const float* sh,
	int cube_size, uint32_t mask, uint32_t num_samples, uint32_t num_light_samples, int separate, uint8_t* cube, const RenderAccel& a, hipStream_t s,
	unsigned long long* counters = nullptr, const DepthArgs* depth = nullptr, int point_light = 0);
hipError_t launch_accel_direct(const Geom& g, int half_store, const void* color, const uint32_t* lightmap, const FrameConsts& fc, const float* sh,
	int W, int H, uint32_t num_samples, uint32_t num_light_samples, int separate, uint8_t* target, float* out_float, const RenderAccel& a, hipStream_t s,
	unsigned long long* counters = nullptr, const DepthArgs* depth = nullptr, int point_light = 0);
hipError_t launch_visualize_color(const Geom& g, int half_store, const void* color, int W, int H, uint8_t* target, float* out_float, hipStream_t s);
hipError_t launch_lightmap_decode(const uint32_t* lightmap, float* out, size_t n, hipStream_t s);

hipError_t launch_resolve_cube(const uint8_t* cube_mip, int N, const FrameConsts& fc, int W, int H, uint8_t* target,
	float* out_float, hipStream_t s, const DepthArgs* depth = nullptr);
hipError_t launch_clear_target(uint8_t* target, int W, int H, const float rgba[4], hipStream_t s);
hipError_t launch_environment(const float* cube, int n, const FrameConsts& fc, int W, int H, uint8_t* target, float* out_float, hipStream_t s);

hipError_t launch_bc6h_decode(const void* blocks_dev, int nbx, int nby, int n, float* out_dev, hipStream_t s);
enum { DDS_BC6H_UF16 = 0, DDS_RGBA32F = 1, DDS_RGB32F = 2, DDS_RGBA16F = 3, DDS_RGBA8 = 4 };
struct DdsCube { uint32_t size, mips; int kind; size_t face_offset[6], mip_offset[16]; };
bool dds_cube_layout(const void* dds, size_t bytes, DdsCube* out);
void dds_linear_face_to_rgb(const void* texels, int kind, size_t n, float* out);

hipError_t launch_sh_transform(const float* cube, int n, float* scratch0, float* scratch1, float* w0, float* w1,
	float* out27, hipStream_t s);
size_t sh_scratch_floats(int n, int which);

}
```

### fluidx12_amd/csrc/fx_schedule.cpp

```cpp
#include "fx_host.h"
#include <memory>

using namespace fx;

namespace fxh {

int for_members(fx_ctx* ctx, std::vector<fx_ctx*>& out)
{
	out.clear();
	if (ctx->group && ctx->group->transport->is_local() && !ctx->group->broken) out = ctx->group->members;
	else out.push_back(ctx);
	return FX_OK;
}


static inline bool peer_group(const fx_ctx* c) { return c->group && c->group->per_member; }
static inline hipStream_t CS(const fx_ctx* m, hipStream_t s) { return peer_group(m) ? m->group->lane_of(m).compute : s; }
struct LaneRef { fx_lane* lane; hipStream_t compute; };
static std::vector<LaneRef> lanes_of(fx_ctx* lead, const std::vector<fx_ctx*>& M, hipStream_t s)
{
	std::vector<LaneRef> out;
	if (!lead->group) return out;
	if (lead->group->per_member) for (fx_ctx* m : M) out.push_back(LaneRef{ &lead->group->lane_of(m), lead->group->lane_of(m).compute });
	else out.push_back(LaneRef{ &lead->group->lanes[0], s });
	return out;
}
enum StreamKind { ON_COMPUTE = 0, ON_COMM = 1 };

int overlap_level(const fx_ctx* lead)
{
	if (!multi_rank(lead) || lead->group->lanes.empty() || !lead->group->lanes[0].comm) return 0;
	return lead->opt_overlap;
}

struct ExchSpec { int set, k, pidx; };

static int do_exchange(fx_ctx* ctx, const std::vector<fx_ctx*>& M, const ExchSpec* specs, int nspec, StreamKind kind, hipStream_t s, int channel = 0)
{
	if (!multi_rank(ctx)) return FX_OK;
	DeviceGuard dg(ctx->device);
	std::vector<hipStream_t> streams;
	for (const LaneRef& L : lanes_of(ctx, M, s)) streams.push_back(kind == ON_COMM ? L.lane->comm : L.compute);
	ScopedMark mk(ctx, peer_group(ctx) ? streams[(size_t)ctx->rank] : streams[0], MK_EXCH);
	std::vector<std::vector<Seg>> segs(M.size());
	size_t total = 0;
	for (size_t i = 0; i < M.size(); ++i) {
		for (int j = 0; j < nspec; ++j) {
			if (specs[j].k <= 0) continue;
			ExchItem it[4];
			const int n = exchange_items(M[i], specs[j].set, specs[j].k, specs[j].pidx, it);
			halo_segments(M[i], it, n, segs[i]);
		}
		total += segs[i].size();
		if (M[i]->timing_on) for (const Seg& sg : segs[i]) M[i]->acc.exchange_bytes += sg.bytes;
	}
	if (!total) return FX_OK;
	for (fx_ctx* m : M) if (m->timing_on) m->acc.exchange_calls += 1;
	return ctx->group->transport->exchange(ctx->group, segs, streams, channel);
}

#define FX_LANES(body) do { for (const LaneRef& L : lanes_of(ctx, M, s)) { DeviceGuard dgl_(L.lane->device); body } } while (0)
static int comm_fork(fx_ctx* ctx, const std::vector<fx_ctx*>& M, hipStream_t s)
{
	FX_LANES(FX_HIP(hipEventRecord(L.lane->ev_ready, L.compute)); FX_HIP(hipStreamWaitEvent(L.lane->comm, L.lane->ev_ready, 0)););
	return FX_OK;
}
static int comm_mark_done(fx_ctx* ctx, const std::vector<fx_ctx*>& M, hipStream_t s) { FX_LANES(FX_HIP(hipEventRecord(L.lane->ev_done, L.lane->comm));); return FX_OK; }
static int comm_join(fx_ctx* ctx, const std::vector<fx_ctx*>& M, hipStream_t s) { FX_LANES(FX_HIP(hipStreamWaitEvent(L.compute, L.lane->ev_done, 0));); return FX_OK; }


int advect_range(fx_ctx* ctx, hipStream_t s, Range r, bool own_only)
{
	if (r.hi <= r.lo) return FX_OK;
	DeviceGuard dg(ctx->device);
	const SimParams sp{ ctx->time_step, (int)ctx->desc.advect_address, ctx->g.Zg > 1 ? 1 : 0, ctx->impulse_on ? 1 : 0 };
	const int par = ctx->frame_parity;
	Geom g = ctx->g;
	g.zlo = std::max(g.zlo, g.z0 - ctx->adv_w_lo); g.zhi = std::min(g.zhi, g.z0 + g.nz - 1 + ctx->adv_w_hi);
	if (own_only) { g.zlo = std::max(g.zlo, g.z0); g.zhi = std::min(g.zhi, g.z0 + g.nz - 1); }
	if (!ctx->adv_far && !ctx->adv_far_tried) {
		ctx->adv_far_tried = true;
		const size_t words = advect_far_words(g, g.nz);
		if (words) {
			if (hipMalloc((void**)&ctx->adv_far, words * sizeof(uint32_t)) == hipSuccess) {
				FX_HIP(hipMemsetAsync(ctx->adv_far, 0, 2 * sizeof(uint32_t), s));
				ctx->adv_far_words = words;
			} else {
				(void)hipGetLastError();
				ctx->adv_far = nullptr;
			}
		}
	}
	const bool lend = ctx->adv_far != nullptr;
	bool far_used = false;
	const bool frame_was_rendered = ctx->rendered_since_step && ctx->rendered_on == s;
	ctx->rendered_since_step = false;
	AdvectAlpha aa{ frame_was_rendered && ctx->accel_ok && ctx->opt_render_accel && FX_KNOB_INT("ADVECT_ALPHA", 1) ? ctx->accel.alpha : nullptr, false };
	if (ctx->accel_alpha_of == ctx->col[par]) ctx->accel_alpha_of = nullptr;
	FX_HIP(launch_advect(g, sp, ctx->half, ctx->vel[0], ctx->col[1 - par], ctx->vel[1], ctx->col[par],
		r.lo, r.hi, ctx->halo_overflow, s, lend ? ctx->adv_far : nullptr, lend ? ctx->adv_far_words : 0, (int)(ctx->adv_far_turn & 1u), &far_used, &aa));
	if (aa.written) ctx->accel_alpha_of = ctx->col[par];
	if (far_used) ++ctx->adv_far_turn;
	return FX_OK;
}

int options_digest(const fx_ctx* c)
{
	uint32_t h = 2166136261u;
	uint32_t dt_bits;
	std::memcpy(&dt_bits, &c->time_step, 4);
	for (uint32_t v : { (uint32_t)c->opt_overlap, (uint32_t)c->opt_round, (uint32_t)c->opt_adaptive, dt_bits }) h = (h ^ v) * 16777619u;
	return (int)(h & 0x3FFFFFFFu);
}

static int record_step(fx_ctx* ctx, std::vector<fx_ctx*>& M, hipStream_t s)
{
	if (!multi_rank(ctx) || !ctx->step_rec) return FX_OK;
	for (fx_ctx* m : M) {
		if (m->rec_in_project) { m->rec_in_project = false; continue; }
		DeviceGuard dg(m->device);
		FX_HIP(launch_face_need(m->g, m->half, m->vel[0], m->time_step, (int)m->desc.advect_address, options_digest(m), m->halo_overflow, m->step_rec, CS(m, s)));
	}
	DeviceGuard dg(ctx->device);
	if (ctx->group->transport->is_local()) {
		for (fx_ctx* m : M) {
			DeviceGuard dgm(m->device);
			FX_HIP(hipMemcpyAsync(m->rec_host, m->step_rec, 4 * sizeof(int), hipMemcpyDeviceToHost, CS(m, s)));
			FX_HIP(hipEventRecord(m->rec_ev, CS(m, s)));
		}
	} else {
		hipStream_t cs = s;
		if (overlap_level(ctx) >= 1) { int rc = comm_fork(ctx, M, s); if (rc) return rc; cs = ctx->group->lanes[0].comm; }
		if (ctx->group->transport->allgather(ctx->step_rec, 4, ctx->gath_dev, cs) != FX_OK) { ctx->last_error = "rccl: all-gather of the step record failed"; return FX_E_COMM; }
		FX_HIP(hipMemcpyAsync(ctx->rec_host, ctx->gath_dev, 4 * sizeof(int) * (size_t)ctx->nranks, hipMemcpyDeviceToHost, cs));
		FX_HIP(hipEventRecord(ctx->rec_ev, cs));
	}
	for (fx_ctx* m : M) { m->rec_pending = true; m->need_valid = true; m->rec_dt = m->time_step; }
	return FX_OK;
}

static int consume_record(fx_ctx* ctx, std::vector<fx_ctx*>& M)
{
	const int Ha = (int)ctx->desc.halo_advect;
	for (fx_ctx* m : M) { m->adv_w_lo = has_lower(m) ? Ha : 0; m->adv_w_hi = has_upper(m) ? Ha : 0; }
	if (!multi_rank(ctx) || !ctx->rec_pending) return FX_OK;
	const bool local = ctx->group->transport->is_local();
	for (fx_ctx* m : M) {
		DeviceGuard dg(m->device);
		FX_HIP(hipEventSynchronize(m->rec_ev));
		if (!local) break;
	}
	const int n = ctx->nranks;
	auto rec = [&](int r) -> const int* { return local ? M[(size_t)r]->rec_host : ctx->rec_host + 4 * r; };
	bool fault = false, mismatch = false, usable = ctx->opt_adaptive != 0;
	for (int r = 0; r < n; ++r) { fault = fault || rec(r)[3] != 0; mismatch = mismatch || rec(r)[2] != rec(0)[2]; }
	for (fx_ctx* m : M) { usable = usable && m->need_valid && m->time_step <= m->rec_dt; m->rec_pending = false; }
	if (fault) {
		for (fx_ctx* m : M) {
			if (!rec(m->rank)[3] || !m->halo_overflow) continue;
			DeviceGuard dg(m->device);
			FX_HIP(hipDeviceSynchronize());
			unsigned flag = 0;
			FX_HIP(hipMemcpy(&flag, m->halo_overflow, sizeof flag, hipMemcpyDeviceToHost));
			if (!flag) continue;
			FX_HIP(hipMemset(m->halo_overflow, 0, sizeof(unsigned)));
			FX_HIP(hipDeviceSynchronize());
			m->halo_fault = true;
		}
		ctx->last_error = "the previous step's advection left the exchanged halo on at least one rank";
		return FX_E_HALO;
	}
	if (mismatch) { ctx->last_error = "the ranks of the chain run with different schedule options (fx_set_option) or time steps"; return FX_E_STATE; }
	if (!usable) return FX_OK;
	for (int r = 0; r + 1 < n; ++r)
		if (std::max(rec(r)[1], rec(r + 1)[0]) > Ha) {
			ctx->last_error = "the next advection needs more planes across a slab face than halo_advect provides";
			return FX_E_HALO;
		}
	for (fx_ctx* m : M) {
		const int r = m->rank;
		m->adv_w_lo = r > 0 ? std::max(rec(r - 1)[1], rec(r)[0]) : 0;
		m->adv_w_hi = r + 1 < n ? std::max(rec(r)[1], rec(r + 1)[0]) : 0;
	}
	return FX_OK;
}

int advect_all(fx_ctx* ctx, std::vector<fx_ctx*>& M, hipStream_t s)
{
	int rc;
	const int Ha = (int)ctx->desc.halo_advect;
	bool col_ready = multi_rank(ctx);
	for (fx_ctx* m : M) col_ready = col_ready && m->col_halo_buf == 1 - (int)m->frame_parity;
	for (fx_ctx* m : M) m->col_halo_buf = -1;
	bool ov = overlap_level(ctx) >= 1;
	if (ov && ctx->group->min_nz <= 2 * Ha) ov = false;
	if (!ov) {
		if ((rc = consume_record(ctx, M))) return rc;
		if (col_ready) FX_LANES(FX_HIP(hipStreamWaitEvent(L.compute, L.lane->ev_col_done, 0)););
		const ExchSpec spec{ col_ready ? EX_ADVECT_VEL : EX_ADVECT_IN, Ha, 0 };
		if ((rc = do_exchange(ctx, M, &spec, 1, ON_COMPUTE, s))) return rc;
		for (fx_ctx* m : M) {
			ScopedMark mk(m, CS(m, s), MK_ADVECT);
			if (m->timing_on) m->acc.advect_halo_planes += (uint64_t)(m->adv_w_lo + m->adv_w_hi);
			if ((rc = advect_range(m, CS(m, s), owned(m), false))) return rc;
		}
		return FX_OK;
	}
	if ((rc = comm_fork(ctx, M, s))) return rc;
	for (fx_ctx* m : M) {
		ScopedMark mk(m, CS(m, s), MK_ADVECT);
		const Range o = owned(m);
		if ((rc = advect_range(m, CS(m, s), Range{ o.lo + (has_lower(m) ? Ha : 0), o.hi - (has_upper(m) ? Ha : 0) }, true))) return rc;
	}
	if ((rc = consume_record(ctx, M))) return rc;
	if (col_ready) FX_LANES(FX_HIP(hipStreamWaitEvent(L.lane->comm, L.lane->ev_col_done, 0)););
	const ExchSpec spec{ col_ready ? EX_ADVECT_VEL : EX_ADVECT_IN, Ha, 0 };
	if ((rc = do_exchange(ctx, M, &spec, 1, ON_COMM, s))) return rc;
	if ((rc = comm_mark_done(ctx, M, s))) return rc;
	if ((rc = comm_join(ctx, M, s))) return rc;
	for (fx_ctx* m : M) {
		ScopedMark mk(m, CS(m, s), MK_ADVECT);
		if (m->timing_on) m->acc.advect_halo_planes += (uint64_t)(m->adv_w_lo + m->adv_w_hi);
		const Range o = owned(m);
		if (has_lower(m) && (rc = advect_range(m, CS(m, s), Range{ o.lo, o.lo + Ha }, false))) return rc;
		if (has_upper(m) && (rc = advect_range(m, CS(m, s), Range{ o.hi - Ha, o.hi }, false))) return rc;
	}
	return FX_OK;
}

int confine_phase(fx_ctx* ctx, hipStream_t s)
{
	if (!(ctx->vort_eps > 0.0f) || !(ctx->time_step > 0.0f)) return FX_OK;
	DeviceGuard dg(ctx->device);
	ScopedMark mk(ctx, s, MK_ADVECT);
	FX_HIP(launch_confine_vorticity(ctx->g, ctx->half, ctx->vel[1], ctx->vel[0], ctx->vort_eps, ctx->time_step, s));
	std::swap(ctx->vel[0], ctx->vel[1]);
	return FX_OK;
}

int emit_phase(fx_ctx* ctx, hipStream_t s)
{
	if (ctx->emitters.empty() || !(ctx->time_step > 0.0f)) return FX_OK;
	DeviceGuard dg(ctx->device);
	ScopedMark mk(ctx, s, MK_ADVECT);
	const int par = ctx->frame_parity;
	float* alpha = ctx->accel_alpha_of == ctx->col[par] ? ctx->accel.alpha : nullptr;
	FX_HIP(launch_emit(ctx->g, ctx->half, ctx->vel[1], ctx->col[par], alpha, ctx->emitters.data(), (int)ctx->emitters.size(), ctx->time_step, s));
	return FX_OK;
}

int enforce_phase(fx_ctx* ctx, hipStream_t s)
{
	if (!ctx->obst_code || !ctx->obst_cells || !(ctx->time_step > 0.0f)) return FX_OK;
	DeviceGuard dg(ctx->device);
	ScopedMark mk(ctx, s, MK_ADVECT);
	const int par = ctx->frame_parity;
	float* alpha = ctx->accel_alpha_of == ctx->col[par] ? ctx->accel.alpha : nullptr;
	FX_HIP(launch_obstacle_enforce(ctx->g, ctx->half, ctx->obst_code, ctx->obst_lo, ctx->obst_hi, ctx->vel[1], ctx->col[par], alpha, s));
	return FX_OK;
}

int divergence_phase(fx_ctx* ctx, hipStream_t s)
{
	DeviceGuard dg(ctx->device);
	ScopedMark mk(ctx, s, MK_DIV);
	const Range r = owned(ctx);
	if (ctx->obst_code) {
		FX_HIP(launch_divergence_obs(ctx->g, ctx->half, ctx->vel[1], ctx->obst_code, ctx->b, r.lo, r.hi, s));
		return FX_OK;
	}
	FX_HIP(launch_divergence(ctx->g, ctx->half, ctx->vel[1], ctx->b, r.lo, r.hi, s));
	return FX_OK;
}

static JacobiPolicy policy_of(const fx_ctx* c)
{
	return jacobi_policy(c->g, (int)(c->desc.flags & FX_FLAG_JACOBI_FUSE_MASK), c->frozen != nullptr, c->frozen_alt != nullptr);
}

static int jacobi_launch(fx_ctx* ctx, hipStream_t s, int src, JacobiLaunch l, Range r, ScopedMark* mk)
{
	r.lo = std::max(r.lo, 0); r.hi = std::min(r.hi, ctx->g.Zg);
	if (r.hi <= r.lo) return FX_OK;
	DeviceGuard dg(ctx->device);
	FX_HIP(launch_jacobi(ctx->g, l, ctx->p[src], ctx->b, ctx->p[src ^ 1], ctx->frozen, ctx->frozen ? ctx->frozen_alt : nullptr, r.lo, r.hi, s));
	if (l.family == JF_TILE2D && ctx->frozen) std::swap(ctx->frozen, ctx->frozen_alt);
	if (mk) { mk->launches += 1; mk->sweeps += l.sweeps; }
	return FX_OK;
}

static int jacobi_round(fx_ctx* ctx, hipStream_t s, int count, ScopedMark* mk)
{
	std::vector<JacobiLaunch> plan(count);
	plan.resize(jacobi_plan(policy_of(ctx), count, plan.data()));
	int left = count;
	for (const JacobiLaunch& l : plan) {
		const int t = l.sweeps;
		if (mk && mk->kind == MK_JACOBI && mk->launches && t * mk->launches < mk->sweeps) mk->split(MK_JACOBI_TAIL);
		left -= t;
		const int rc = jacobi_launch(ctx, s, ctx->p_cur, l, grown(ctx, multi_rank(ctx) ? left : 0), mk);
		if (rc) return rc;
		ctx->p_cur ^= 1;
	}
	return FX_OK;
}

static int clear_freeze_masks(std::vector<fx_ctx*>& M, hipStream_t s)
{
	for (fx_ctx* m : M)
		if (m->frozen) { DeviceGuard dg(m->device); if (hipMemsetAsync(m->frozen, 0, m->g.cells_local(), s) != hipSuccess) return FX_E_DEVICE; }
	return FX_OK;
}

static bool takes_sparse_solver(const fx_ctx* c, uint32_t iters) { return freeze_takes_sparse_solver(c->g, iters, c->frozen && c->fz_tile_next, multi_rank(c), multi_rank(c) ? c->group->min_nz : 0); }

template <class T> static void freeze_rotate(T*& a, T*& d, T*& spare, bool strip) { std::swap(a, d); if (strip) std::swap(d, spare); }

static int jacobi_freeze(fx_ctx* lead, std::vector<fx_ctx*>& M, hipStream_t s, uint32_t iters)
{
	fx_ctx* ctx = lead;
	const bool multi = multi_rank(lead);
	struct Run { Geom v; size_t off, moff; int own0; FreezeWork w; float *src, *a, *d; uint8_t *ma, *md, *mx; uint32_t* stat; uint32_t stat_hi; };
	std::vector<Run> R(M.size());
	std::vector<std::unique_ptr<ScopedMark>> mk(M.size());
	const bool fuse = lead->fz_fuse_div;
	lead->fz_fuse_div = false;
	FreezeLaunch plan[kFreezeSlots];
	int launches = 0;
	for (size_t i = 0; i < M.size(); ++i) {
		fx_ctx* m = M[i];
		DeviceGuard dg(m->device);
		hipStream_t ms = CS(m, s);
		if (++m->fz_gen >= (1u << 23)) {
			FX_HIP(hipMemsetAsync(m->fz_tile_next, 0, (size_t)jacobi_freeze_tiles(m->g) * sizeof(uint32_t), ms));
			FX_HIP(hipMemsetAsync(m->fz_stat, 0, kFreezeStatRing * sizeof(uint32_t), ms));
			FX_HIP(hipMemsetAsync(m->fz_counts, 0, 2 * jacobi_freeze_count_words() * sizeof(uint32_t), ms));
			m->fz_gen = 2; m->fz_gen_mark = 0;
		}
		Run& r = R[i];
		int first = 0;
		r.v = jacobi_freeze_view(m->g, &first, &r.own0);
		r.off = (size_t)first * m->g.plane();
		r.moff = (size_t)first * (size_t)((m->g.X + 3) / 4) * m->g.Y;
		const uint32_t gen = m->fz_gen;
		r.stat_hi = gen << 8;
		r.stat = m->fz_stat + gen % kFreezeStatRing;
		m->fz_iters[gen % kFreezeStatRing] = iters;
		const size_t cw = jacobi_freeze_count_words(), es = elem_size(m);
		r.w = FreezeWork{ m->fz_tile_next, gen, { m->fz_list[0], m->fz_list[1] }, jacobi_freeze_tiles(m->g),
			m->fz_counts + (gen & 1u) * cw, m->fz_counts + ((gen & 1u) ^ 1u) * cw };
		r.src = m->p[m->p_cur]; r.a = m->p[m->p_cur ^ 1]; r.d = m->p_aux;
		r.ma = m->fz_mask[0]; r.md = m->fz_mask[1]; r.mx = m->fz_mask[2];
		int forced;
		const int width = freeze_strip_width(m->g, multi, m->fz_mask[2] != nullptr, &forced);
		const bool adaptive = width && forced < 0 && m->fz_active_dev;
		const FreezeCadence cadence = freeze_cadence(gen);
		if (adaptive && cadence.take_over && m->fz_active_pending) {
			FX_HIP(hipEventSynchronize(m->fz_active_ev));
			m->fz_active_pending = false;
			m->fz_dense_n = freeze_strip_hysteresis(m->fz_dense_n, *(volatile uint32_t*)m->fz_active_host, (uint32_t)jacobi_freeze_tiles(m->g), width == 4);
		}
		launches = freeze_plan(m->g, iters, multi, m->fz_mask[2] != nullptr, adaptive ? m->fz_dense_n : 0, plan);
		if (!launches) return FX_E_STATE;
		const bool one_copy = plan[0].kind == FZ_DENSE_ONE;
		mk[i].reset(new ScopedMark(m, ms, MK_JACOBI));
		FX_HIP(launch_freeze_dense(r.v, r.src + r.off, m->b + r.off, r.a + r.off, one_copy ? nullptr : r.d + r.off, r.ma + r.moff, one_copy ? nullptr : r.md + r.moff, r.w, ms,
			fuse ? (const char*)m->vel[1] + r.off * es : nullptr, m->half, r.own0, m->g.nz, m->g.cells_local()));
		mk[i]->launches = 1; mk[i]->sweeps = 1;
		if (multi || iters == 1) mk[i].reset(); else mk[i]->split(MK_JACOBI_TAIL);
		if (adaptive && cadence.count) {
			FX_HIP(launch_count_marks(r.w.tile_mark, gen, jacobi_freeze_tiles(m->g), m->fz_active_dev, ms));
			if (!m->fz_active_ev) FX_HIP(hipEventCreateWithFlags(&m->fz_active_ev, hipEventDisableTiming));
			FX_HIP(hipEventRecord(m->fz_active_ev, ms));
			m->fz_active_pending = true;
		}
	}
	auto exchange = [&](bool with_b) -> int {
		if (!multi) return FX_OK;
		for (size_t i = 0; i < M.size(); ++i) { M[i]->fz_x_p = R[i].a; M[i]->fz_x_m = R[i].ma; }
		const ExchSpec specs[2] = { { EX_FREEZE, kFreezeHalo, 0 }, { EX_DIV, kFreezeHalo, 0 } };
		return do_exchange(lead, M, specs, with_b ? 2 : 1, ON_COMPUTE, s);
	};
	int rc = exchange(true);
	if (rc) return rc;
	uint32_t flag_tag = 0;
	for (int j = 1, n = 0; j < launches; ++j) {
		const FreezeLaunch& l = plan[j];
		const bool strip = l.kind == FZ_STRIP;
		if (strip) flag_tag = R[0].w.gen | ((uint32_t)j << 24);
		for (size_t i = 0; i < M.size(); ++i) {
			fx_ctx* m = M[i];
			Run& r = R[i];
			DeviceGuard dg(m->device);
			if (!mk[i]) mk[i].reset(new ScopedMark(m, CS(m, s), MK_JACOBI_TAIL));
			if (strip)
				FX_HIP((l.levels == 4 ? launch_freeze_strip4 : launch_freeze_strip3)(r.v, r.a, m->b, r.d, r.src, r.ma, r.md, r.mx, r.w.tile_mark, flag_tag, r.stat, r.stat_hi, l.base, CS(m, s)));
			else
				FX_HIP(launch_freeze_tiles(r.v, r.a + r.off, m->b + r.off, r.d + r.off, r.ma + r.moff, r.md + r.moff, r.w, n, l.levels, l.base, r.stat, r.stat_hi, CS(m, s), r.own0, m->g.nz, n == 0 ? flag_tag : 0u));
			m->acc.freeze_strip_launches += strip;
			mk[i]->launches += 1; mk[i]->sweeps += (uint64_t)l.levels;
			if (multi) mk[i].reset();
			freeze_rotate(r.a, r.d, r.src, strip);
			freeze_rotate(r.ma, r.md, r.mx, strip);
		}
		if (!strip) ++n;
		if ((rc = exchange(false))) return rc;
	}
	mk.clear();
	for (size_t i = 0; i < M.size(); ++i) { fx_ctx* m = M[i]; m->p[0] = R[i].a; m->p[1] = R[i].d; m->p_aux = R[i].src; m->fz_mask[0] = R[i].ma; m->fz_mask[1] = R[i].md; m->fz_mask[2] = R[i].mx; m->p_cur = 0; }
	return FX_OK;
}
// ... 189 lines not shown
```

### fluidx12_amd/csrc/fx_sim.hip

```cpp
#include "fx_internal.h"
#include <algorithm>
#include <cstdlib>
#include <cstdio>

namespace fx {

typedef _Float16 h16;
typedef _Float16 h16x4 __attribute__((ext_vector_type(4)));

struct __attribute__((packed, aligned(4))) F32Pair { float a, b; };
struct __attribute__((packed, aligned(2))) F16Pair { _Float16 a, b; };

template <bool HALF> struct Store;
template <> struct Store<false> {
	typedef float S;
	typedef float4 S4;
	static __device__ __forceinline__ void ld2(const S* p, size_t i, float& a, float& b)
	{
		const F32Pair v = *reinterpret_cast<const F32Pair*>(p + i);
		a = v.a; b = v.b;
	}
	static __device__ __forceinline__ float ld(const S* p, size_t i) { return p[i]; }
	static __device__ __forceinline__ float stored(float v) { return v; }
	static __device__ __forceinline__ void st(S* p, size_t i, float v) { p[i] = v; }
// ... 604 lines not shown
	const float R = xw < XW - 1 ? St::ld(vel, off + W) : cx.v[W - 1];
	const CellsW<W> U = ldwv<W, HALF>(vel, stride + zrow + (uint32_t)yu * g.X + col), D = ldwv<W, HALF>(vel, stride + zrow + (uint32_t)yd * g.X + col);
	const CellsW<W> F = ldwv<W, HALF>(vel, 2u * stride + (uint32_t)g.lz(zf) * plane + (uint32_t)y * g.X + col);
	const CellsW<W> B = ldwv<W, HALF>(vel, 2u * stride + (uint32_t)g.lz(zb) * plane + (uint32_t)y * g.X + col);
	CellsW<W> o;
#pragma unroll
	for (int i = 0; i < W; ++i) {
		const float l = i == 0 ? L : cx.v[i > 0 ? i - 1 : 0], r = i == W - 1 ? R : cx.v[i < W - 1 ? i + 1 : 0];
		o.v[i] = 0.5f * ((-F.v[i] + B.v[i]) + ((-U.v[i] + D.v[i]) + (-l + r)));
	}
	stw<W>(b, off, o);
}

template <int W, bool HALF>
__global__ __launch_bounds__(256) void k_project_vw(const Geom g, const typename Store<HALF>::S* __restrict__ vel_in, const float* __restrict__ p,
	typename Store<HALF>::S* __restrict__ vel_out, int z_begin, int nzp, int remap, int rows_per_block)
{
	const int XW = g.X / W;
	const Tile3 tile = xcd_tile((XW + (int)blockDim.x - 1) / (int)blockDim.x, (g.Y + rows_per_block - 1) / rows_per_block, nzp, remap);
	const int xw = tile.x * blockDim.x + threadIdx.x;
	const int y = tile.y * rows_per_block + threadIdx.y;
	const int z = z_begin + tile.z;
	if (xw >= XW || y >= g.Y) return;
	const uint32_t plane = (uint32_t)g.plane(), stride = (uint32_t)g.cells_local();
	const int yu = max(y, 1) - 1, yd = min(y + 1, g.Y - 1);
	const int zf = max(z, 1) - 1, zb = min(z + 1, g.Zg - 1);
	const uint32_t zrow = (uint32_t)g.lz(z) * plane, col = (uint32_t)(W * xw), off = zrow + (uint32_t)y * g.X + col;
	const CellsW<W> c = ldw<W>(p, off);
	const float L = xw > 0 ? p[off - 1] : c.v[0];
	const float R = xw < XW - 1 ? p[off + W] : c.v[W - 1];
	const CellsW<W> U = ldw<W>(p, zrow + (uint32_t)yu * g.X + col), D = ldw<W>(p, zrow + (uint32_t)yd * g.X + col);
	const CellsW<W> F = ldw<W>(p, (uint32_t)g.lz(zf) * plane + (uint32_t)y * g.X + col);
	const CellsW<W> B = ldw<W>(p, (uint32_t)g.lz(zb) * plane + (uint32_t)y * g.X + col);
	const CellsW<W> ux = ldwv<W, HALF>(vel_in, off), uy = ldwv<W, HALF>(vel_in, stride + off), uz = ldwv<W, HALF>(vel_in, 2u * stride + off);
	const float k = __uint_as_float(0x3f855556u);
	float py = ((float)y + 0.5f) / (float)g.Y, pz = ((float)z + 0.5f) / (float)g.Zg;
	py = fmaf(py, 2.0f, -1.0f); pz = fmaf(pz, 2.0f, -1.0f);
	float fy = (-fabsf(py) + 0.970000029f) * 33.3333359f, fz = (-fabsf(pz) + 0.970000029f) * 33.3333359f;
	fy = fminf(fmaxf(fy, -1.0f), 1.0f); fz = fminf(fmaxf(fz, -1.0f), 1.0f);
	CellsW<W> ox, oy, oz;
#pragma unroll
	for (int i = 0; i < W; ++i) {
		const float pl = i == 0 ? L : c.v[i > 0 ? i - 1 : 0], pr = i == W - 1 ? R : c.v[i < W - 1 ? i + 1 : 0];
		const float gx = -pl + pr, gy = -U.v[i] + D.v[i], gz = -F.v[i] + B.v[i];
		const float wz_ = fmaf(-gz, k, uz.v[i]);
		const float wx_ = fmaf(-gx, k, ux.v[i]), wy_ = fmaf(-gy, k, uy.v[i]);
		float px = ((float)(W * xw + i) + 0.5f) / (float)g.X;
		px = fmaf(px, 2.0f, -1.0f);
		float fxw = (-fabsf(px) + 0.970000029f) * 33.3333359f;
		fxw = fminf(fmaxf(fxw, -1.0f), 1.0f);
		ox.v[i] = wx_ * ((0.0f < wx_ * px) ? fxw : 1.0f);
		oy.v[i] = wy_ * ((0.0f < wy_ * py) ? fy : 1.0f);
		oz.v[i] = wz_ * ((0.0f < wz_ * pz) ? fz : 1.0f);
	}
	stwv<W, HALF>(vel_out, off, ox);
	stwv<W, HALF>(vel_out, stride + off, oy);
	stwv<W, HALF>(vel_out, 2u * stride + off, oz);
}

int sim_row_kernel(const Geom& g, int half_store, int stage, int is3d)
{
	const bool rows16 = (g.X & 3) == 0 && (g.cells_local() & 3) == 0, small = g.cells_local() * 3 < ((size_t)1 << 30);
	if (stage == SIM_DIVERGENCE) {
		if (g.Zg > 1 && rows16) return ROW_V4;
	} else {
		if (!is3d) return ROW_SCALAR;
		if (FX_KNOB_INT("PROJECT_V4", 1) && rows16 && small) return ROW_V4;
	}
	if (!FX_KNOB_INT("ROW_VW", 1) || g.Zg <= 1 || !small) return ROW_SCALAR;
	if (half_store) return g.X % 2 == 0 ? ROW_VW2 : ROW_SCALAR;
	return g.X % 3 == 0 ? ROW_VW3 : (g.X % 2 == 0 ? ROW_VW2 : ROW_SCALAR);
}

template <bool HALF>
__global__ __launch_bounds__(256) void k_face_need(const Geom g, const typename Store<HALF>::S* __restrict__ uz, float dt, int address, int* __restrict__ rec,
	int digest, const unsigned* __restrict__ halo_overflow)
{
	typedef Store<HALF> St;
	const size_t plane = g.plane();
	const int z = g.z0 + (int)blockIdx.y;
	const float pz = ((float)z + 0.5f) / (float)g.Zg;
	const typename St::S* row = uz + (size_t)g.lz(z) * plane;
	int lo = 0, hi = 0;
	auto one = [&](float u) {
		const float az = fmaf(-u, dt, pz);
		const int iz = (int)floorf(az * (float)g.Zg - 0.5f);
		const int a = addr_tap(iz, g.Zg, address), b_ = addr_tap(iz + 1, g.Zg, address);
		lo = max(lo, g.z0 - min(a, b_));
		hi = max(hi, max(a, b_) - (g.z0 + g.nz - 1));
	};
	if (!HALF && (plane & 3) == 0) {
		const float4* row4 = reinterpret_cast<const float4*>(row);
		for (size_t i = (size_t)blockIdx.x * blockDim.x + threadIdx.x; i < plane / 4; i += (size_t)gridDim.x * blockDim.x) {
			const float4 v = row4[i];
			one(v.x); one(v.y); one(v.z); one(v.w);
		}
	} else {
		for (size_t i = (size_t)blockIdx.x * blockDim.x + threadIdx.x; i < plane; i += (size_t)gridDim.x * blockDim.x) one(St::ld(row, i));
	}
	if (blockIdx.x == 0 && blockIdx.y == 0 && threadIdx.x == 0) { rec[2] = digest; rec[3] = (int)*halo_overflow; }
	if (__builtin_amdgcn_ballot_w64(lo > 0 || hi > 0) == 0) return;
#pragma unroll
	for (int o = 32; o > 0; o >>= 1) { lo = max(lo, __shfl_xor(lo, o)); hi = max(hi, __shfl_xor(hi, o)); }
	if ((threadIdx.x & 63) == 0) { if (lo > 0) atomicMax(rec, lo); if (hi > 0) atomicMax(rec + 1, hi); }
}

template <bool HALF>
__global__ __launch_bounds__(256) void k_copy_owned(const Geom g, const typename Store<HALF>::S* __restrict__ src,
	typename Store<HALF>::S* __restrict__ dst)
{
	const size_t n = g.cells_owned();
	const size_t off = (size_t)g.H * g.plane();
	for (size_t i = (size_t)blockIdx.x * blockDim.x + threadIdx.x; i < 3 * n; i += (size_t)gridDim.x * blockDim.x) {
		const size_t a = i / n, r = i - a * n;
		dst[a * g.cells_local() + off + r] = src[a * g.cells_local() + off + r];
	}
}

template <bool HALF>
__global__ __launch_bounds__(256) void k_to_storage(const float* __restrict__ src, typename Store<HALF>::S* __restrict__ dst, size_t n)
{
	for (size_t i = (size_t)blockIdx.x * blockDim.x + threadIdx.x; i < n; i += (size_t)gridDim.x * blockDim.x)
		Store<HALF>::st(dst, i, src[i]);
}
template <bool HALF>
__global__ __launch_bounds__(256) void k_from_storage(const typename Store<HALF>::S* __restrict__ src, float* __restrict__ dst, size_t n)
{
	for (size_t i = (size_t)blockIdx.x * blockDim.x + threadIdx.x; i < n; i += (size_t)gridDim.x * blockDim.x)
		dst[i] = Store<HALF>::ld(src, i);
}

static inline dim3 grid_xyz(const Geom& g, int nzp) { return dim3(((g.X + 63) / 64) * ((g.Y + 3) / 4) * nzp, 1, 1); }
static inline unsigned grid_1d(size_t n) { return (unsigned)((n + 255) / 256 < 4096 ? (n + 255) / 256 : 4096); }
enum { REMAP_JACOBI = 0, REMAP_ADVECT = 1, REMAP_DIV = 2, REMAP_PROJECT = 3 };
static int xcd_remap_on(int which)
{
	int mode[4] = { 1, 0, 0, 0 };
	const char* e = FX_KNOB("XCD_REMAP");
	int a, b_, c, d;
	if (e && sscanf(e, "%d,%d,%d,%d", &a, &b_, &c, &d) == 4) { mode[0] = a; mode[1] = b_; mode[2] = c; mode[3] = d; }
	return mode[which];
}

static int xcd_remap_for(int which, const Geom& g)
{
	const char* fe_ = FX_KNOB("XCD_REMAP");
	const bool forced = fe_ && *fe_;
	if (forced || which == REMAP_JACOBI) return xcd_remap_on(which);
	return g.Zg > 1 && g.plane() <= 32768 && g.cells_local() < (size_t)6 << 20 ? 1 : 0;
}

hipError_t launch_advect(const Geom& g, const SimParams& sp, int half_store, const void* vel_in, const void* col_in,
	void* vel_out, void* col_out, int z_begin, int z_end, unsigned* halo_overflow, hipStream_t s, uint32_t* far_scratch, size_t far_words, int far_parity, bool* far_used,
	AdvectAlpha* alpha)
{
	if (far_used) *far_used = false;
	if (alpha) alpha->written = false;
	if (z_end <= z_begin) return hipSuccess;
	int bx = 64, by = 4, bz = 1;
	if (const char* e = FX_KNOB("ADVECT_BLOCK")) {
		int a, b_, c;
		if (sscanf(e, "%d,%d,%d", &a, &b_, &c) == 3 && a > 0 && b_ > 0 && c > 0 && a * b_ * c <= 256) { bx = a; by = b_; bz = c; }
	}
	const int nzp = z_end - z_begin;
	{
		const char* le = FX_KNOB("ADVECT_LDS");
		if (!(le && le[0] == '0') && bx == 64 && by == 4 && bz == 1 && !xcd_remap_on(REMAP_ADVECT)) {
			const hipError_t e = launch_advect_lds(g, sp, half_store, vel_in, col_in, vel_out, col_out, z_begin, z_end, halo_overflow, far_scratch, far_words, far_parity, far_used, s, le && le[0] == '2', alpha);
			if (e != hipErrorNotSupported) return e;
		}
	}
	float* alpha_out = alpha && alpha->out && g.nzl() == g.Zg && z_begin == 0 && z_end == g.Zg ? alpha->out : nullptr;
	if (alpha_out) alpha->written = true;
	const char* fe = FX_KNOB("ADVECT_FAST");
	const bool fast_off = fe && fe[0] == '0';
	auto pow2 = [](int v) { return v > 0 && (v & (v - 1)) == 0; };
	if (!fast_off && pow2(g.X) && pow2(g.Y) && pow2(g.Zg) && g.X >= 2 && g.cells_local() * 16 < ((size_t)1 << 32) &&
		bx == 64 && by == 4 && bz == 1 && !xcd_remap_on(REMAP_ADVECT)) {
		const dim3 block(64, 4, 1), grid(((g.X + 63) / 64) * ((g.Y + 3) / 4) * nzp, 1, 1);
		const float rX = 1.0f / (float)g.X, rY = 1.0f / (float)g.Y, rZ = 1.0f / (float)g.Zg, inv_rr = sp.is3d ? 256.0f : 1024.0f;
		auto lg = [](int v) { int k = 0; while ((1 << k) < v) ++k; return k; };
		const int lgX = lg(g.X), lgY = lg(g.Y), lg_gx = lg((g.X + 63) / 64), lg_gy = lg((g.Y + 3) / 4);
		if (half_store)
			hipLaunchKernelGGL(k_advect_fast<true>, grid, block, 0, s, g, sp, (const h16*)vel_in, (const h16x4*)col_in,
				(h16*)vel_out, (h16x4*)col_out, z_begin, nzp, halo_overflow, rX, rY, rZ, inv_rr, lgX, lgY, lg_gx, lg_gy, alpha_out);
		else
			hipLaunchKernelGGL(k_advect_fast<false>, grid, block, 0, s, g, sp, (const float*)vel_in, (const float4*)col_in,
				(float*)vel_out, (float4*)col_out, z_begin, nzp, halo_overflow, rX, rY, rZ, inv_rr, lgX, lgY, lg_gx, lg_gy, alpha_out);
		return hipGetLastError();
	}
	const int cbz = g.Zg > 1 ? bz : 1;
	const dim3 block(bx, by, cbz), grid(((g.X + bx - 1) / bx) * ((g.Y + by - 1) / by) * ((nzp + cbz - 1) / cbz), 1, 1);
	if (half_store)
		hipLaunchKernelGGL(k_advect<true>, grid, block, 0, s, g, sp, (const h16*)vel_in, (const h16x4*)col_in,
			(h16*)vel_out, (h16x4*)col_out, z_begin, nzp, xcd_remap_for(REMAP_ADVECT, g), halo_overflow, alpha_out);
	else
		hipLaunchKernelGGL(k_advect<false>, grid, block, 0, s, g, sp, (const float*)vel_in, (const float4*)col_in,
			(float*)vel_out, (float4*)col_out, z_begin, nzp, xcd_remap_for(REMAP_ADVECT, g), halo_overflow, alpha_out);
	return hipGetLastError();
}

hipError_t launch_divergence(const Geom& g, int half_store, const void* vel, float* b, int z_begin, int z_end, hipStream_t s)
{
	if (z_end <= z_begin) return hipSuccess;
	const int w = sim_row_kernel(g, half_store, SIM_DIVERGENCE, g.Zg > 1);
	if (w == ROW_V4) {
		const int nzp = z_end - z_begin, X4 = g.X >> 2;
		const int bx = X4 < 64 ? X4 : 64;
		int by = 256 / bx; if (by > g.Y) by = g.Y;
		const dim3 block(bx, by, 1), grid(((X4 + bx - 1) / bx) * ((g.Y + by - 1) / by) * nzp, 1, 1);
		if (half_store) hipLaunchKernelGGL(k_divergence_v4<true>, grid, block, 0, s, g, (const h16*)vel, b, z_begin, nzp, xcd_remap_for(REMAP_DIV, g), by);
		else hipLaunchKernelGGL(k_divergence_v4<false>, grid, block, 0, s, g, (const float*)vel, b, z_begin, nzp, xcd_remap_for(REMAP_DIV, g), by);
		return hipGetLastError();
	}
	if (w != ROW_SCALAR) {
		const int nzp = z_end - z_begin, XW = g.X / w;
		const int bx = XW < 64 ? XW : 64;
		int by = 256 / bx; if (by > g.Y) by = g.Y;
		const dim3 block(bx, by, 1), grid(((XW + bx - 1) / bx) * ((g.Y + by - 1) / by) * nzp, 1, 1);
		if (half_store) hipLaunchKernelGGL((k_divergence_vw<2, true>), grid, block, 0, s, g, (const h16*)vel, b, z_begin, nzp, xcd_remap_for(REMAP_DIV, g), by);
		else if (w == 3) hipLaunchKernelGGL((k_divergence_vw<3, false>), grid, block, 0, s, g, (const float*)vel, b, z_begin, nzp, xcd_remap_for(REMAP_DIV, g), by);
		else hipLaunchKernelGGL((k_divergence_vw<2, false>), grid, block, 0, s, g, (const float*)vel, b, z_begin, nzp, xcd_remap_for(REMAP_DIV, g), by);
		return hipGetLastError();
	}
	const dim3 grid = grid_xyz(g, z_end - z_begin), block(64, 4, 1);
	if (half_store) hipLaunchKernelGGL(k_divergence<true>, grid, block, 0, s, g, (const h16*)vel, b, z_begin, z_end - z_begin, xcd_remap_for(REMAP_DIV, g));
	else hipLaunchKernelGGL(k_divergence<false>, grid, block, 0, s, g, (const float*)vel, b, z_begin, z_end - z_begin, xcd_remap_for(REMAP_DIV, g));
	return hipGetLastError();
}

hipError_t launch_jacobi_sweep(const Geom& g, const float* p_in, const float* b, float* p_out, uint8_t* frozen,
	int z_begin, int z_end, hipStream_t s)
{
	return launch_jacobi_sweep2(g, p_in, b, p_out, frozen, z_begin, z_end, 0, 0, s);
}

hipError_t launch_jacobi_sweep2(const Geom& g, const float* p_in, const float* b, float* p_out, uint8_t* frozen,
	int z_begin, int z_end, int z_begin2, int z_end2, hipStream_t s)
{
	if (z_end < z_begin) z_end = z_begin;
	if (z_end2 < z_begin2) z_end2 = z_begin2;
	const int split = z_end - z_begin;
	const int nzp = split + (z_end2 - z_begin2);
	if (nzp <= 0) return hipSuccess;
	if (!frozen && g.Zg > 1 && (g.X & 3) == 0) {
		const int X4 = g.X >> 2;
		const int bx = X4 < 64 ? X4 : 64;
		int by = 256 / bx; if (by < 1) by = 1; if (by > g.Y) by = g.Y;
		const dim3 block(bx, by, 1), grid(((X4 + bx - 1) / bx) * ((g.Y + by - 1) / by) * nzp, 1, 1);
		hipLaunchKernelGGL(k_jacobi_v4, grid, block, 0, s, g, p_in, b, p_out, z_begin, nzp, xcd_remap_on(REMAP_JACOBI), by, split, z_begin2);
	} else {
		hipLaunchKernelGGL(k_jacobi_generic, grid_xyz(g, nzp), dim3(64, 4, 1), 0, s, g, p_in, b, p_out, frozen, z_begin, nzp, xcd_remap_on(REMAP_JACOBI),
			split, z_begin2);
	}
	return hipGetLastError();
}

__global__ __launch_bounds__(256) void k_copy16(uint4* __restrict__ dst, const uint4* __restrict__ src, size_t n)
{
	for (size_t i = (size_t)blockIdx.x * blockDim.x + threadIdx.x; i < n; i += (size_t)gridDim.x * blockDim.x) dst[i] = src[i];
}

__device__ __forceinline__ unsigned long long mix64(unsigned long long x)
{
	x += 0x9E3779B97F4A7C15ull;
	x = (x ^ (x >> 30)) * 0xBF58476D1CE4E5B9ull;
	x = (x ^ (x >> 27)) * 0x94D049BB133111EBull;
	return x ^ (x >> 31);
}
template <typename T>
__global__ __launch_bounds__(256) void k_digest(const T* __restrict__ v, size_t count, unsigned long long key0, unsigned long long* __restrict__ out)
{
	unsigned long long a = 0, c = 0;
	for (size_t i = (size_t)blockIdx.x * blockDim.x + threadIdx.x; i < count; i += (size_t)gridDim.x * blockDim.x) {
		const unsigned long long h = mix64(((key0 + i) << 32) ^ ((key0 + i) >> 32) ^ ((unsigned long long)v[i] * 0xD6E8FEB86659FD93ull));
		a += h;
		c += mix64(h ^ 0xA5A5A5A55A5A5A5Aull);
	}
	for (int o = 32; o > 0; o >>= 1) { a += __shfl_down(a, o); c += __shfl_down(c, o); }
	if ((threadIdx.x & 63) == 0) { atomicAdd(out, a); atomicAdd(out + 1, c); }
}

hipError_t launch_digest(const void* v, size_t count, int elem_bytes, unsigned long long key0, unsigned long long* out, hipStream_t s)
{
	if (!count) return hipSuccess;
	const unsigned grid = (unsigned)std::min<size_t>((count + 255) / 256, 4096);
	if (elem_bytes == 4) hipLaunchKernelGGL(k_digest<uint32_t>, dim3(grid), dim3(256), 0, s, static_cast<const uint32_t*>(v), count, key0, out);
	else hipLaunchKernelGGL(k_digest<uint16_t>, dim3(grid), dim3(256), 0, s, static_cast<const uint16_t*>(v), count, key0, out);
	return hipGetLastError();
}

hipError_t launch_copy_bytes(void* dst, const void* src, size_t bytes, hipStream_t s)
{
	if (!bytes) return hipSuccess;
	if ((bytes & 15) || ((uintptr_t)dst & 15) || ((uintptr_t)src & 15)) return hipMemcpyAsync(dst, src, bytes, hipMemcpyDeviceToDevice, s);
	const size_t n = bytes / 16;
	const unsigned grid = (unsigned)((n + 255) / 256 < 2048 ? (n + 255) / 256 : 2048);
	hipLaunchKernelGGL(k_copy16, dim3(grid), dim3(256), 0, s, static_cast<uint4*>(dst), static_cast<const uint4*>(src), n);
	return hipGetLastError();
}

hipError_t launch_project(const Geom& g, const SimParams& sp, int half_store, const void* vel_in, const float* p,
	void* vel_out, int z_begin, int z_end, hipStream_t s, int* rec, int digest, const unsigned* halo_overflow, bool* rec_done)
{
	if (rec_done) *rec_done = false;
	if (z_end <= z_begin) return hipSuccess;
	const int w = sim_row_kernel(g, half_store, SIM_PROJECT, sp.is3d);
	if (w == ROW_V4) {
		auto pow2 = [](int v) { return v > 0 && (v & (v - 1)) == 0; };
		const int nzp = z_end - z_begin, X4 = g.X >> 2;
		const int bx = X4 < 64 ? X4 : 64;
		int by = 256 / bx; if (by > g.Y) by = g.Y;
		const dim3 block(bx, by, 1), grid(((X4 + bx - 1) / bx) * ((g.Y + by - 1) / by) * nzp, 1, 1);
		const float rX = 1.0f / (float)g.X, rY = 1.0f / (float)g.Y, rZ = 1.0f / (float)g.Zg;
		int* r = (rec && z_begin == g.z0 && z_end == g.z0 + g.nz) ? rec : nullptr;
		if (r) {
			const hipError_t e = hipMemsetAsync(r, 0, 2 * sizeof(int), s);
			if (e != hipSuccess) return e;
			if (rec_done) *rec_done = true;
		}
		const bool rcp = pow2(g.X) && pow2(g.Y) && pow2(g.Zg);
// ... 65 lines not shown
```

### include/fluidx_hip.h

```cpp
#ifndef FLUIDX_HIP_H
#define FLUIDX_HIP_H

#include <stddef.h>
#include <stdint.h>

#ifdef __cplusplus
extern "C" {
#endif

#define FX_ABI_VERSION 7

enum fx_status {
	FX_OK = 0,
	FX_E_INVALID = -1,
	FX_E_DEVICE = -2,
	FX_E_NOMEM = -3,
	FX_E_STATE = -4,
	FX_E_COMM = -5,
	FX_E_HALO = -6
};

enum fx_render_flags {
	FX_RAY_MARCH_DIRECT = 0,
	FX_RAY_MARCH_CUBEMAP = 1,
// ... 1 lines not shown
	FX_OPTIMIZED = 3
};
#define FX_FRAME_COUNT 3

enum fx_storage { FX_STORAGE_FP32 = 0, FX_STORAGE_FP16 = 1 };
enum fx_jacobi_mode { FX_JACOBI_FIXED = 0,
                      FX_JACOBI_FAITHFUL = 1 };
enum fx_address { FX_ADDRESS_CLAMP = 0,
                  FX_ADDRESS_MIRROR = 1 };

enum fx_field {
	FX_FIELD_VELOCITY = 0, FX_FIELD_VELOCITY1 = 1, FX_FIELD_COLOR = 2, FX_FIELD_COLOR_PREV = 3,
	FX_FIELD_PRESSURE = 4, FX_FIELD_DIVERGENCE = 5, FX_FIELD_LIGHTMAP = 6, FX_FIELD_CUBEMAP = 7,
	FX_FIELD_TARGET = 8,
	FX_FIELD_TARGET_FLOAT = 9,
	FX_FIELD_CUBE_DEPTH = 10
};

typedef struct fx_ctx fx_ctx;

typedef struct fx_desc {
	uint32_t struct_size;
	uint32_t grid_x, grid_y, grid_z;
	uint32_t viewport_w, viewport_h;
	uint32_t storage;
	uint32_t jacobi_iters;
	uint32_t jacobi_mode;
	uint32_t advect_address;
	int32_t  device;
	uint32_t slab_z0, slab_nz;
	uint32_t halo_advect;
	uint32_t halo_jacobi;
	uint32_t flags;
} fx_desc;

#define FX_FLAG_JACOBI_FUSE_MASK 0xFu
#define FX_FLAG_NO_OVERLAP 0x10u
#define FX_FLAG_RENDER_ONLY 0x20u

typedef struct fx_frame_info {
	uint32_t cube_lod;
	uint32_t cube_size;
	uint32_t ray_samples;
	uint32_t visibility_mask;
	uint32_t frame_parity;
	float    edge_pixels;
	float    time_step;
	float    world_view_proj_i[16];
	float    screen_to_world[16];
} fx_frame_info;

typedef struct fx_timing {
	double   advect_ms, divergence_ms, jacobi_ms, project_ms, light_ms, view_ms, exchange_ms;
	uint64_t steps, jacobi_launches, jacobi_sweeps, renders;
	double   resolve_ms;
	double   jacobi_main_ms;
	uint64_t jacobi_main_launches, jacobi_main_sweeps;
	uint64_t exchange_bytes, advect_halo_planes;
	double   chain_ms;
	uint64_t freeze_solves, freeze_sweeps;
	uint64_t exchange_calls;
	uint64_t view_samples, light_samples, lightmap_fetches;
	uint64_t freeze_strip_launches;
} fx_timing;

int fx_abi_version(void);
const char* fx_error_string(int status);

int fx_create(fx_ctx** out, const fx_desc* desc);
int fx_destroy(fx_ctx* ctx);
int fx_set_max_samples(fx_ctx* ctx, uint32_t max_ray_samples, uint32_t max_light_samples);
int fx_set_sh(fx_ctx* ctx, const float* coeffs27);
int fx_update_frame(fx_ctx* ctx, float time_step, uint8_t frame_index,
	const float view[16], const float proj[16], const float eye[3]);
int fx_simulate(fx_ctx* ctx, void* stream, uint8_t frame_index);
int fx_render(fx_ctx* ctx, void* stream, uint8_t frame_index, uint8_t flags);
int fx_clear_render_target(fx_ctx* ctx, void* stream, const float rgba[4]);
int fx_render_cube(fx_ctx* ctx, void* stream, uint8_t frame_index);

#define FX_DEPTH_DEVICE 0x1u
int fx_set_scene_depth(fx_ctx* ctx, void* stream, const float* depth, uint32_t width, uint32_t height,
	float z_near, float z_far, uint32_t flags);

#define FX_LIGHT_DIRECTIONAL 0u
#define FX_LIGHT_POINT       1u
typedef struct fx_light {
	uint32_t struct_size, kind;
	float position[3];
	float color[4];
	float ambient[4];
} fx_light;
int fx_set_light(fx_ctx* ctx, const fx_light* light);
int fx_get_light(fx_ctx* ctx, fx_light* out);

int fx_set_environment(fx_ctx* ctx, const float* cube, uint32_t n);
int fx_render_environment(fx_ctx* ctx, void* stream, uint8_t frame_index);

int fx_get_frame_info(fx_ctx* ctx, fx_frame_info* out);

int fx_synchronize(fx_ctx* ctx);
const char* fx_last_error(fx_ctx* ctx);

int fx_upload(fx_ctx* ctx, int field, const void* host, size_t bytes);
int fx_download(fx_ctx* ctx, int field, void* host, size_t bytes);
size_t fx_field_bytes(fx_ctx* ctx, int field);
int fx_field_digest(fx_ctx* ctx, int field, uint32_t z_begin, uint32_t z_count, uint64_t out[2]);

int fx_checkpoint_save(fx_ctx* ctx, const char* path);
int fx_checkpoint_load(fx_ctx* ctx, const char* path);

int fx_advect(fx_ctx* ctx, void* stream);
int fx_divergence(fx_ctx* ctx, void* stream);
int fx_jacobi(fx_ctx* ctx, void* stream, uint32_t iters);
int fx_project(fx_ctx* ctx, void* stream);

int fx_set_vorticity_confinement(fx_ctx* ctx, float epsilon);
int fx_confine_vorticity(fx_ctx* ctx, void* stream);

#define FX_MAX_EMITTERS 16u
typedef struct fx_emitter {
	uint32_t struct_size, flags;
	float center[3];
	float radius;
	float color_rate[4];
	float force[3];
	float swirl;
} fx_emitter;
int fx_set_emitters(fx_ctx* ctx, const fx_emitter* list, uint32_t count);
int fx_get_emitters(fx_ctx* ctx, fx_emitter* out, uint32_t capacity, uint32_t* count);
int fx_set_impulse(fx_ctx* ctx, int enabled);
int fx_emit(fx_ctx* ctx, void* stream);

#define FX_OBSTACLES_DEVICE 0x1u
int fx_set_obstacles(fx_ctx* ctx, void* stream, const uint8_t* solid, size_t bytes, uint32_t flags);
int fx_get_obstacles(fx_ctx* ctx, uint8_t* solid_out, size_t bytes, uint64_t* solid_cells);
int fx_enforce_obstacles(fx_ctx* ctx, void* stream);

int fx_sh_transform(fx_ctx* ctx, const float* cube, uint32_t n, float* out27);

int fx_dds_cube_info(const void* dds, size_t bytes, uint32_t* size, uint32_t* mips);
int fx_dds_decode_cube(fx_ctx* ctx, const void* dds, size_t bytes, uint32_t mip, float* out_cube, size_t out_floats);

int fx_timing_enable(fx_ctx* ctx, int enable);
int fx_timing_read(fx_ctx* ctx, fx_timing* out, int reset);

size_t fx_comm_id_bytes(void);
int fx_comm_get_unique_id(void* id_out, size_t bytes);
int fx_comm_init_rank(fx_ctx* ctx, const void* id, size_t bytes, int rank, int nranks);
int fx_comm_init_local(fx_ctx** ctxs, int nranks);
int fx_comm_init_peer(fx_ctx** ctxs, int nranks);

int fx_comm_gather_color(fx_ctx* ctx, void* stream, fx_ctx* full, int root, const uint32_t* slab_z0, const uint32_t* slab_nz);

enum fx_option { FX_OPT_OVERLAP = 1, FX_OPT_JACOBI_ROUND = 2, FX_OPT_ADAPTIVE_HALO = 3, FX_OPT_COUNT_SAMPLES = 4, FX_OPT_RENDER_ACCEL = 5 };
int fx_set_option(fx_ctx* ctx, uint32_t option, uint32_t value);

int fx_set_knob(const char* name, const char* value);
const char* fx_knob_name(uint32_t index);

#ifdef __cplusplus
}
#endif
#endif
```

Measured before the change: 22.60 billion.

## Add sparse advection path that skips loading and storing empty colour tiles

Adds a sparse advect kernel that keeps per-tile emptiness flags for the colour field. Tiles whose source neighbourhood is all zero skip the colour loads and zero the LDS instead. Tiles that stay zero and were already flagged empty in the destination skip the colour store. Flags are kept valid across frames and cleared after uploads, emitters and obstacle writes. This targets HBM traffic on colour, the largest field. It costs extra flag loads and stores, more state tracking, and a risk of stale-flag correctness bugs.

```diff
diff --git a/fluidx12_amd/capi.py b/fluidx12_amd/capi.py
--- a/fluidx12_amd/capi.py
+++ b/fluidx12_amd/capi.py
@@ -12,7 +12,7 @@
 JACOBI_FIXED, JACOBI_FAITHFUL = 0, 1
 ADDRESS_CLAMP, ADDRESS_MIRROR = 0, 1
 FLAG_JACOBI_FUSE_MASK, FLAG_NO_OVERLAP, FLAG_RENDER_ONLY = 0xF, 0x10, 0x20
-OPT_OVERLAP, OPT_JACOBI_ROUND, OPT_ADAPTIVE_HALO, OPT_COUNT_SAMPLES, OPT_RENDER_ACCEL = 1, 2, 3, 4, 5
+OPT_OVERLAP, OPT_JACOBI_ROUND, OPT_ADAPTIVE_HALO, OPT_COUNT_SAMPLES, OPT_RENDER_ACCEL, OPT_ADVECT_SPARSE = 1, 2, 3, 4, 5, 6
 ABI_VERSION = 7
 (FIELD_VELOCITY, FIELD_VELOCITY1, FIELD_COLOR, FIELD_COLOR_PREV, FIELD_PRESSURE, FIELD_DIVERGENCE,
  FIELD_LIGHTMAP, FIELD_CUBEMAP, FIELD_TARGET, FIELD_TARGET_FLOAT, FIELD_CUBE_DEPTH) = range(11)
diff --git a/fluidx12_amd/csrc/fx_advect_lds.hip b/fluidx12_amd/csrc/fx_advect_lds.hip
--- a/fluidx12_amd/csrc/fx_advect_lds.hip
+++ b/fluidx12_amd/csrc/fx_advect_lds.hip
@@ -93,6 +93,59 @@
 		: "=&s"(keep)
 		: "s"(col), "s"(v0), "s"(v1), "s"(v2), "v"(off_col), "v"(off_col_hi), "v"(off_vel), "s"(lds_col), "s"(lds_vel), "n"(VEL_BYTES)
 		: "scc");
+}
+
+template <int VEL_BYTES, bool HALF>
+__device__ __forceinline__ void stage64_vel(const void* v0, const void* v1, const void* v2, uint32_t off_vel, uint32_t lds_vel)
+{
+	uint32_t keep;
+	lds_vel = __builtin_amdgcn_readfirstlane(lds_vel);
+	if (HALF)
+		asm volatile(
+			"s_mov_b32 %0, m0\n\t"
+			"s_mov_b32 m0, %5\n\t"
+			"s_nop 0\n\t"
+			"global_load_lds_ushort %4, %1\n\t"
+			"s_add_u32 m0, m0, %6\n\t"
+			"s_nop 0\n\t"
+			"global_load_lds_ushort %4, %2\n\t"
+			"s_add_u32 m0, m0, %6\n\t"
+			"s_nop 0\n\t"
+			"global_load_lds_ushort %4, %3\n\t"
+			"s_mov_b32 m0, %0"
+			: "=&s"(keep)
+			: "s"(v0), "s"(v1), "s"(v2), "v"(off_vel), "s"(lds_vel), "n"(VEL_BYTES)
+			: "scc");
+	else
+		asm volatile(
+			"s_mov_b32 %0, m0\n\t"
+			"s_mov_b32 m0, %5\n\t"
+			"s_nop 0\n\t"
+			"global_load_lds_dword %4, %1\n\t"
+			"s_add_u32 m0, m0, %6\n\t"
+			"s_nop 0\n\t"
+			"global_load_lds_dword %4, %2\n\t"
+			"s_add_u32 m0, m0, %6\n\t"
+			"s_nop 0\n\t"
+			"global_load_lds_dword %4, %3\n\t"
+			"s_mov_b32 m0, %0"
+			: "=&s"(keep)
+			: "s"(v0), "s"(v1), "s"(v2), "v"(off_vel), "s"(lds_vel), "n"(VEL_BYTES)
+			: "scc");
+}
+
+__device__ __forceinline__ void stage64_flags(const void* base, uint32_t off, uint32_t lds_dst)
+{
+	uint32_t keep;
+	lds_dst = __builtin_amdgcn_readfirstlane(lds_dst);
+	asm volatile(
+		"s_mov_b32 %0, m0\n\t"
+		"s_mov_b32 m0, %3\n\t"
+		"s_nop 0\n\t"
+		"global_load_lds_dword %2, %1\n\t"
+		"s_mov_b32 m0, %0"
+		: "=&s"(keep)
+		: "s"(base), "v"(off), "s"(lds_dst));
 }
 
 template <typename T>
@@ -144,9 +197,7 @@
 #undef FX_TRI
 }
 
-template <bool HALF, bool ALPHA>
-__device__ __forceinline__ void advect_finish(const SimParams& sp, float (&u)[3], float (&c)[4], float ex, float dx, float dz, float dt, float atten,
-	uint32_t id, uint32_t stride, void* __restrict__ vel_out, void* __restrict__ col_out, float* __restrict__ alpha_out)
+__device__ __forceinline__ void advect_impulse(const SimParams& sp, float (&u)[3], float (&c)[4], float ex, float dx, float dz, float dt)
 {
 	if (__builtin_amdgcn_ballot_w64(sp.impulse && ex > -6.5f) != 0) {
 		const float basis = exp2f(ex);
@@ -167,6 +218,13 @@
 			c[3] = saturatef(fmaf(bdt, 40.0f, c[3]));
 		}
 	}
+}
+
+template <bool HALF, bool ALPHA>
+__device__ __forceinline__ void advect_finish(const SimParams& sp, float (&u)[3], float (&c)[4], float ex, float dx, float dz, float dt, float atten,
+	uint32_t id, uint32_t stride, void* __restrict__ vel_out, void* __restrict__ col_out, float* __restrict__ alpha_out)
+{
+	advect_impulse(sp, u, c, ex, dx, dz, dt);
 	char* vo = static_cast<char*>(vel_out);
 	char* co = static_cast<char*>(col_out);
 	if (HALF) {
@@ -398,12 +456,259 @@
 }
 
 
+constexpr int FLAG_SET_WORDS = 64, FLAG_LDS_BYTES = 4 * FLAG_SET_WORDS * 4;
+
+template <bool HALF>
+__global__ __launch_bounds__(512) __attribute__((amdgpu_waves_per_eu(4, 4))) void k_advect_sparse(const Geom g, const SimParams sp,
+	const void* __restrict__ vel_in, const void* __restrict__ col_in, void* __restrict__ vel_out, void* __restrict__ col_out,
+	int z_begin, int nzp, int zchunk, int nchunks, unsigned* halo_overflow, float rX, float rY, float rZ, float inv_rr,
+	int lgX, int lgY, int lg_gx, int lg_gy, uint32_t* __restrict__ far_list, uint32_t* __restrict__ far_flat, uint32_t* __restrict__ far_total, uint32_t far_cap,
+	uint32_t* flags, uint32_t src_word0, uint32_t dst_word0, int dst_valid)
+{
+	constexpr int TY = 8;
+	constexpr bool P2 = true;
+	__shared__ uint32_t far_n, far_base;
+	extern __shared__ __attribute__((aligned(16))) char lds[];
+
+	const int tid = (int)threadIdx.x, lane = tid & 63, wave = __builtin_amdgcn_readfirstlane(tid >> 6);
+	const int ntx = 1 << lg_gx, nty = 1 << lg_gy;
+	const int ntiles = ntx * nty * nchunks;
+	int tl = (int)blockIdx.x;
+	{
+		const int q = ntiles >> 3, r = ntiles & 7, xcd = tl & 7, j = tl >> 3;
+		tl = xcd * q + min(xcd, r) + j;
+	}
+	const int tx = tl & (ntx - 1), ty = (tl >> lg_gx) & (nty - 1), chunk = tl >> (lg_gx + lg_gy);
+	const int x0t = tx << 6, y0t = ty * TY;
+	const int zb = z_begin + chunk * zchunk, ze = min(zb + zchunk, z_begin + nzp);
+	if (zb >= ze) return;
+
+	const int lgP = lgX + lgY, lgF = lgY + lg_gx;
+	constexpr int COL_BYTES = Lay<HALF, TY>::COL_BYTES, SLOT_BYTES = Lay<HALF, TY>::SLOT_BYTES;
+	constexpr int NCELL = Lay<HALF, TY>::NCELL, VEL_BYTES = Lay<HALF, TY>::VEL_BYTES, NT = 64 * TY;
+	constexpr uint32_t ES = HALF ? 2 : 4, CS = HALF ? 8 : 16;
+	const uint32_t stride = planes<P2>((uint32_t)g.nzl(), lgP, g);
+	const char* v0 = reinterpret_cast<const char*>(vel_in);
+	const char* v1 = v0 + (size_t)stride * ES;
+	const char* v2 = v1 + (size_t)stride * ES;
+
+	uint32_t src_a, src_b = 0;
+	{
+		const int c = tid, r = c / HX, cc = c - r * HX;
+		src_a = rows<P2>((uint32_t)addr_tap(y0t - 1 + r, g.Y, sp.address), lgX, g) + (uint32_t)addr_tap(x0t - 1 + cc, g.X, sp.address);
+	}
+	const bool has_b = NT + tid < NCELL;
+	if (has_b) {
+		const int c = NT + tid, r = c / HX, cc = c - r * HX;
+		src_b = rows<P2>((uint32_t)addr_tap(y0t - 1 + r, g.Y, sp.address), lgX, g) + (uint32_t)addr_tap(x0t - 1 + cc, g.X, sp.address);
+	}
+	const bool wave_has_b = NT + wave * 64 < NCELL;
+
+	const bool fl_dst = lane >= 32 && lane < 40;
+	uint32_t fl_lane;
+	{
+		const int r = lane < 30 ? lane / 3 : 1, k = lane < 30 ? lane - 3 * (lane / 3) : 1;
+		const int xc = k == 0 ? x0t - 1 : k == 1 ? x0t : x0t + TX;
+		fl_lane = ((uint32_t)addr_tap(y0t - 1 + r, g.Y, sp.address) << lg_gx) + ((uint32_t)addr_tap(xc, g.X, sp.address) >> 6);
+		if (fl_dst) fl_lane = ((uint32_t)(y0t + lane - 32) << lg_gx) + (uint32_t)tx;
+	}
+	const uint32_t lds0 = (uint32_t)(size_t)(__attribute__((address_space(3))) char*)lds;
+	const uint32_t* fl_lds = reinterpret_cast<const uint32_t*>(lds + NSLOT * SLOT_BYTES);
+	auto fetch_flags = [&](int q) {
+		const int za = min(max(addr_tap(q, g.Zg, sp.address), g.zlo), g.zhi);
+		const int zd = min(max(q - 2, zb), ze - 1);
+		const uint32_t ps = src_word0 + ((uint32_t)g.lz(za) << lgF), pd = dst_word0 + ((uint32_t)g.lz(zd) << lgF);
+		stage64_flags(flags, ((fl_dst ? pd : ps) + fl_lane) * 4u, lds0 + (uint32_t)(NSLOT * SLOT_BYTES + ((q + 4) & 3) * (FLAG_SET_WORDS * 4)));
+	};
+
+	uint32_t empty = 0u, zeroed = 0u;
+	auto fill = [&](int zq) {
+		const int za = min(max(addr_tap(zq, g.Zg, sp.address), g.zlo), g.zhi);
+		const size_t pz = planes<P2>((uint32_t)g.lz(za), lgP, g);
+		const int sl = (zq + 4) & 3;
+		const uint32_t slot = __builtin_amdgcn_readfirstlane(lds0 + (uint32_t)(sl * SLOT_BYTES));
+		const char* bc = reinterpret_cast<const char*>(col_in) + pz * CS;
+		const char *b0 = v0 + pz * ES, *b1 = v1 + pz * ES, *b2 = v2 + pz * ES;
+		const uint32_t fw = fl_lds[sl * FLAG_SET_WORDS + (lane < 30 ? lane : 0)];
+		const uint32_t bit = 1u << sl;
+		if (__builtin_amdgcn_ballot_w64(fw == 0u) == 0) {
+			stage64_vel<VEL_BYTES, HALF>(b0, b1, b2, src_a * ES, slot + COL_BYTES + (uint32_t)wave * (64 * 4));
+			if (wave_has_b && has_b) stage64_vel<VEL_BYTES, HALF>(b0, b1, b2, src_b * ES, slot + COL_BYTES + (NT + (uint32_t)wave * 64) * 4);
+			if (!(zeroed & bit)) {
+				char* sc = lds + sl * SLOT_BYTES;
+				if (HALF) {
+					reinterpret_cast<uint32_t*>(sc)[tid] = 0u; reinterpret_cast<uint32_t*>(sc)[NCELL + tid] = 0u;
+					if (has_b) { reinterpret_cast<uint32_t*>(sc)[NT + tid] = 0u; reinterpret_cast<uint32_t*>(sc)[NCELL + NT + tid] = 0u; }
+				} else {
+					reinterpret_cast<float4*>(sc)[tid] = make_float4(0.0f, 0.0f, 0.0f, 0.0f);
+					if (has_b) reinterpret_cast<float4*>(sc)[NT + tid] = make_float4(0.0f, 0.0f, 0.0f, 0.0f);
+				}
+			}
+			empty |= bit; zeroed |= bit;
+		} else {
+			if (HALF) stage64h<VEL_BYTES>(bc, b0, b1, b2, src_a * CS, src_a * ES, slot + (uint32_t)wave * (64 * 4), slot + COL_BYTES + (uint32_t)wave * (64 * 4));
+			else stage64<VEL_BYTES>(bc, b0, b1, b2, src_a * CS, src_a * ES, slot + (uint32_t)wave * (64 * 16), slot + COL_BYTES + (uint32_t)wave * (64 * 4));
+			if (wave_has_b) {
+				if (has_b) {
+					if (HALF) stage64h<VEL_BYTES>(bc, b0, b1, b2, src_b * CS, src_b * ES, slot + (NT + (uint32_t)wave * 64) * 4, slot + COL_BYTES + (NT + (uint32_t)wave * 64) * 4);
+					else stage64<VEL_BYTES>(bc, b0, b1, b2, src_b * CS, src_b * ES, slot + (NT + (uint32_t)wave * 64) * 16, slot + COL_BYTES + (NT + (uint32_t)wave * 64) * 4);
+				}
+			}
+			empty &= ~bit; zeroed &= ~bit;
+		}
+	};
+
+	if (tid == 0) far_n = 0u;
+	if (wave == TY - 1) { fetch_flags(zb - 1); fetch_flags(zb); fetch_flags(zb + 1); fetch_flags(zb + 2); }
+	asm volatile("s_waitcnt vmcnt(0)" ::: "memory");
+	__syncthreads();
+	fill(zb - 1);
+	fill(zb);
+	fill(zb + 1);
+	asm volatile("s_waitcnt vmcnt(0)" ::: "memory");
+	__syncthreads();
+
+	const int x = x0t + lane, y = y0t + wave;
+	const float dt = sp.dt;
+	const float px = ((float)x + 0.5f) * rX, py = ((float)y + 0.5f) * rY;
+	const float dx = px + -0.5f, dy = py + -0.100000001f;
+	const float dxy2 = fmaf(dy, dy, dx * dx);
+	const uint32_t own = (uint32_t)((wave + 1) * HX + lane + 1);
+	const float atten = fmaxf(fmaf(-dt, 0.200000003f, 1.0f), 0.0f);
+	const uint32_t unit = dst_word0 + ((uint32_t)y << lg_gx) + (uint32_t)tx;
+
+	for (int z = zb; z < ze; ++z) {
+		if (z + 2 <= ze) fill(z + 2);
+		if (wave == TY - 1 && z + 1 < ze) fetch_flags(z + 3);
+
+		const float pz = ((float)z + 0.5f) * rZ;
+		const float dz = pz + -0.5f;
+		const float d2 = fmaf(dz, dz, dxy2);
+		const float ex = ((d2 * -4.0f) * inv_rr) * 1.44269502f;
+
+		const char* sc = lds + ((z + 4) & 3) * SLOT_BYTES;
+		const uint32_t* vs = reinterpret_cast<const uint32_t*>(sc + COL_BYTES);
+		auto vval = [](uint32_t d) -> float { return HALF ? lo_half(d) : __uint_as_float(d); };
+		const float u0x = vval(vs[own]), u0y = vval(vs[NCELL + own]), u0z = vval(vs[2 * NCELL + own]);
+		const float ax = fmaf(-u0x, dt, px), ay = fmaf(-u0y, dt, py), az = fmaf(-u0z, dt, pz);
+		const float tx_ = ax * (float)g.X - 0.5f, ty_ = ay * (float)g.Y - 0.5f, tz_ = az * (float)g.Zg - 0.5f;
+		const float flx = floorf(tx_), fly = floorf(ty_), flz = floorf(tz_);
+		const float fx = tx_ - flx, fy = ty_ - fly, fz = tz_ - flz;
+		const int ix = (int)flx, iy = (int)fly, iz = (int)flz;
+		const int jx = ix - x, jy = iy - y, jz = iz - z;
+		const int z0 = addr_tap(iz, g.Zg, sp.address), z1 = addr_tap(iz + 1, g.Zg, sp.address);
+		const bool z_present = z0 >= g.zlo && z0 <= g.zhi && z1 >= g.zlo && z1 <= g.zhi;
+		const bool inwin = (unsigned)(jx + 1) <= 1u && (unsigned)(jy + 1) <= 1u && (unsigned)(jz + 1) <= 1u && z_present;
+		const bool any_far = __builtin_amdgcn_ballot_w64(!inwin) != 0;
+
+		float u[3], c[4];
+		if (!inwin) {
+			const uint32_t slot = atomicAdd(&far_n, 1u);
+			far_list[(size_t)blockIdx.x * far_cap + slot] = (uint32_t)x | (uint32_t)y << lgX | (uint32_t)z << lgP;
+		}
+		const int kx = !inwin ? 0 : jx, ky = !inwin ? 0 : jy, kz = !inwin ? z : iz;
+		const uint32_t c0 = (uint32_t)((int)own + ky * HX + kx);
+		const char* s0 = lds + ((kz + 4) & 3) * SLOT_BYTES;
+		const char* s1 = lds + ((kz + 5) & 3) * SLOT_BYTES;
+#pragma unroll
+		for (int a = 0; a < 3; ++a) {
+			const uint32_t* p0 = reinterpret_cast<const uint32_t*>(s0 + COL_BYTES + a * VEL_BYTES) + c0;
+			const uint32_t* p1 = reinterpret_cast<const uint32_t*>(s1 + COL_BYTES + a * VEL_BYTES) + c0;
+			const float c00 = lerpf(vval(p0[0]), vval(p0[1]), fx);
+			const float c10 = lerpf(vval(p0[HX]), vval(p0[HX + 1]), fx);
+			const float c01 = lerpf(vval(p1[0]), vval(p1[1]), fx);
+			const float c11 = lerpf(vval(p1[HX]), vval(p1[HX + 1]), fx);
+			u[a] = lerpf(lerpf(c00, c10, fy), lerpf(c01, c11, fy), fz);
+		}
+		const uint32_t three = (1u << ((z + 3) & 3)) | (1u << ((z + 4) & 3)) | (1u << ((z + 5) & 3));
+		const bool frac_in = fx >= 0.0f && fx < 1.0f && fy >= 0.0f && fy < 1.0f && fz >= 0.0f && fz < 1.0f;
+		const bool zero = (empty & three) == three && !any_far && __builtin_amdgcn_ballot_w64(sp.impulse && ex > -6.5f) == 0 &&
+			__builtin_amdgcn_ballot_w64(!frac_in) == 0;
+		if (zero) {
+			c[0] = 0.0f; c[1] = 0.0f; c[2] = 0.0f; c[3] = 0.0f;
+		} else {
+			float4 t000, t100, t010, t110, t001, t101, t011, t111;
+			if (HALF) {
+				auto tex = [](const char* slot, uint32_t cell) -> float4 {
+					const uint32_t rg = reinterpret_cast<const uint32_t*>(slot)[cell], ba = reinterpret_cast<const uint32_t*>(slot)[NCELL + cell];
+					return make_float4(lo_half(rg), hi_half(rg), lo_half(ba), hi_half(ba));
+				};
+				t000 = tex(s0, c0); t100 = tex(s0, c0 + 1); t010 = tex(s0, c0 + HX); t110 = tex(s0, c0 + HX + 1);
+				t001 = tex(s1, c0); t101 = tex(s1, c0 + 1); t011 = tex(s1, c0 + HX); t111 = tex(s1, c0 + HX + 1);
+			} else {
+				const float4* q0 = reinterpret_cast<const float4*>(s0) + c0;
+				const float4* q1 = reinterpret_cast<const float4*>(s1) + c0;
+				t000 = q0[0]; t100 = q0[1]; t010 = q0[HX]; t110 = q0[HX + 1];
+				t001 = q1[0]; t101 = q1[1]; t011 = q1[HX]; t111 = q1[HX + 1];
+			}
+#define FX_TRI(m) lerpf(lerpf(lerpf(t000.m, t100.m, fx), lerpf(t010.m, t110.m, fx), fy), \
+	lerpf(lerpf(t001.m, t101.m, fx), lerpf(t011.m, t111.m, fx), fy), fz)
+			c[0] = FX_TRI(x); c[1] = FX_TRI(y); c[2] = FX_TRI(z); c[3] = FX_TRI(w);
+#undef FX_TRI
+		}
+		advect_impulse(sp, u, c, ex, dx, dz, dt);
+
+		const uint32_t id = planes<P2>((uint32_t)g.lz(z), lgP, g) + rows<P2>((uint32_t)y, lgX, g) + (uint32_t)x;
+		char* vo = static_cast<char*>(vel_out);
+		char* co = static_cast<char*>(col_out);
+		h16x4 hc;
+		float4 fc;
+		bool nonzero;
+		if (HALF) {
+			*reinterpret_cast<h16*>(vo + id * 2u) = to_h16(u[0] * atten);
+			*reinterpret_cast<h16*>(vo + (stride + id) * 2u) = to_h16(u[1] * atten);
+			*reinterpret_cast<h16*>(vo + (2u * stride + id) * 2u) = to_h16(u[2] * atten);
+			hc.x = to_h16(c[0] * atten); hc.y = to_h16(c[1] * atten); hc.z = to_h16(c[2] * atten); hc.w = to_h16(c[3] * atten);
+			nonzero = __builtin_bit_cast(uint64_t, hc) != 0ull;
+		} else {
+			*reinterpret_cast<float*>(vo + id * 4u) = u[0] * atten;
+			*reinterpret_cast<float*>(vo + (stride + id) * 4u) = u[1] * atten;
+			*reinterpret_cast<float*>(vo + (2u * stride + id) * 4u) = u[2] * atten;
+			fc = make_float4(c[0] * atten, c[1] * atten, c[2] * atten, c[3] * atten);
+			nonzero = (__float_as_uint(fc.x) | __float_as_uint(fc.y) | __float_as_uint(fc.z) | __float_as_uint(fc.w)) != 0u;
+		}
+		const uint32_t unit_empty = !any_far && __builtin_amdgcn_ballot_w64(nonzero) == 0 ? 1u : 0u;
+		const uint32_t dst_flag = dst_valid ? __builtin_amdgcn_readfirstlane(fl_lds[((z + 2) & 3) * FLAG_SET_WORDS + 32 + wave]) : 0u;
+		if (zero && dst_flag != 0u) {
+			asm volatile("s_waitcnt vmcnt(3)" ::: "memory");
+		} else {
+			if (HALF) *reinterpret_cast<h16x4*>(co + id * 8u) = hc;
+			else *reinterpret_cast<float4*>(co + id * 16u) = fc;
+			flags[unit + ((uint32_t)g.lz(z) << lgF)] = unit_empty;
+			asm volatile("s_waitcnt vmcnt(5)" ::: "memory");
+		}
+		__syncthreads();
+	}
+	const uint32_t n = far_n;
+	if (n != 0u) {
+		if (tid == 0) far_base = atomicAdd(far_total, n);
+		__syncthreads();
+		const uint32_t base = far_base;
+		const uint32_t* seg = far_list + (size_t)blockIdx.x * far_cap;
+		for (uint32_t i = (uint32_t)tid; i < n; i += (uint32_t)NT) far_flat[base + i] = seg[i];
+	}
+}
+
+template <bool HALF>
+__global__ __launch_bounds__(256) void k_colour_flags(const void* __restrict__ col, uint32_t* __restrict__ unit_flags, uint32_t nunits)
+{
+	const uint32_t lane = threadIdx.x & 63u, w = threadIdx.x >> 6;
+	for (uint32_t u = blockIdx.x * 4u + w; u < nunits; u += gridDim.x * 4u) {
+		bool nonzero;
+		if (HALF) nonzero = ldg32<uint64_t>(col, (u * 64u + lane) * 8u) != 0ull;
+		else { const uint4 t = ldg32<uint4>(col, (u * 64u + lane) * 16u); nonzero = (t.x | t.y | t.z | t.w) != 0u; }
+		const bool e = __builtin_amdgcn_ballot_w64(nonzero) == 0;
+		if (lane == 0) unit_flags[u] = e ? 1u : 0u;
+	}
+}
+
 hipError_t launch_advect_lds(const Geom& g, const SimParams& sp, int half_store, const void* vel_in, const void* col_in,
 	void* vel_out, void* col_out, int z_begin, int z_end, unsigned* halo_overflow, uint32_t* far_scratch, size_t far_words, int far_parity, bool* far_used, hipStream_t s, bool force,
-	AdvectAlpha* alpha)
+	AdvectAlpha* alpha, AdvectSparse* sparse)
 {
 	if (far_used) *far_used = false;
 	if (alpha) alpha->written = false;
+	if (sparse) sparse->used = false;
 	auto pow2 = [](int v) { return v > 0 && (v & (v - 1)) == 0; };
 	const int nzp = z_end - z_begin;
 	const bool p2 = pow2(g.X) && pow2(g.Y) && pow2(g.Zg);
@@ -444,7 +749,24 @@
 #define FX_FAR(H_, P_, A_) hipLaunchKernelGGL((k_advect_far<H_, P_, A_>), dim3(far_wgs), dim3(256), 0, s, g, sp, vel_in, col_in, vel_out, col_out, alpha_out, far_flat, far_total, far_total_next, halo_overflow, rX, rY, rZ, inv_rr, lgX, lgY)
 	const int far_wgs = 1024;
 	float* alpha_out = alpha && alpha->out && defer && TY == 8 && g.nzl() == g.Zg && z_begin == 0 && z_end == g.Zg ? alpha->out : nullptr;
-	if (alpha_out) {
+	if (sparse && sparse->flags && !alpha_out && p2 && TY == 8 && defer && g.nzl() == g.Zg && z_begin == 0 && z_end == g.Zg) {
+		const uint32_t nunits = (uint32_t)(flat_words >> 6);
+		uint32_t* fl = sparse->flags;
+		const uint32_t src0 = (uint32_t)sparse->src * nunits, dst0 = (uint32_t)sparse->dst * nunits;
+		if (!sparse->src_valid) {
+			const unsigned wgs = (unsigned)std::min<uint32_t>((nunits + 3u) / 4u, 16384u);
+			if (half_store) hipLaunchKernelGGL(k_colour_flags<true>, dim3(wgs), dim3(256), 0, s, col_in, fl + src0, nunits);
+			else hipLaunchKernelGGL(k_colour_flags<false>, dim3(wgs), dim3(256), 0, s, col_in, fl + src0, nunits);
+		}
+#define FX_SPARSE(H_) do { \
+		static bool attr_set = false; \
+		if (!attr_set) { (void)hipFuncSetAttribute(reinterpret_cast<const void*>(k_advect_sparse<H_>), hipFuncAttributeMaxDynamicSharedMemorySize, NSLOT * Lay<H_, 8>::SLOT_BYTES + FLAG_LDS_BYTES); attr_set = true; } \
+		hipLaunchKernelGGL((k_advect_sparse<H_>), dim3(tiles_xy * nchunks), dim3(512), (NSLOT * Lay<H_, 8>::SLOT_BYTES + FLAG_LDS_BYTES), s, g, sp, vel_in, col_in, vel_out, col_out, \
+			z_begin, nzp, zchunk, nchunks, halo_overflow, rX, rY, rZ, inv_rr, lgX, lgY, lg_gx, lg_gy, far_list, far_flat, far_total, far_cap, fl, src0, dst0, sparse->dst_valid ? 1 : 0); } while (0)
+		if (half_store) { FX_SPARSE(true); FX_FAR(true, true, false); } else { FX_SPARSE(false); FX_FAR(false, true, false); }
+#undef FX_SPARSE
+		sparse->used = true;
+	} else if (alpha_out) {
 		if (half_store) { if (p2) { FX_ADV(true, 8, true, true, true); FX_FAR(true, true, true); } else { FX_ADV(true, 8, true, false, true); FX_FAR(true, false, true); } }
 		else { if (p2) { FX_ADV(false, 8, true, true, true); FX_FAR(false, true, true); } else { FX_ADV(false, 8, true, false, true); FX_FAR(false, false, true); } }
 		alpha->written = true;
@@ -472,4 +794,11 @@
 	return 2 + (size_t)g.X * g.Y * (size_t)nzp + tiled * (size_t)(nzp + 32);
 }
 
-}
+size_t advect_flag_words(const Geom& g)
+{
+	auto pow2 = [](int v) { return v > 0 && (v & (v - 1)) == 0; };
+	if (!(pow2(g.X) && pow2(g.Y) && pow2(g.Zg)) || g.nzl() != g.Zg || advect_far_words(g, g.Zg) == 0) return 0;
+	return g.cells_local() >> 6;
+}
+
+}
diff --git a/fluidx12_amd/csrc/fx_api.cpp b/fluidx12_amd/csrc/fx_api.cpp
--- a/fluidx12_amd/csrc/fx_api.cpp
+++ b/fluidx12_amd/csrc/fx_api.cpp
@@ -715,7 +715,7 @@
 		parts[r].bytes = (size_t)nz * plane_bytes;
 		parts[r].src = m ? (const char*)m->col[m->frame_parity] + (size_t)m->g.H * plane_bytes : nullptr;
 		parts[r].dst = am_root ? (char*)full->col[full->frame_parity] + (size_t)z0 * plane_bytes : nullptr;
-		if (am_root) full->accel_alpha_of = nullptr;
+		if (am_root) { full->accel_alpha_of = nullptr; full->col_flags_valid[full->frame_parity] = false; }
 	}
 	DeviceGuard dg(ctx->device);
 	hipStream_t s = pick_stream(ctx, stream);
diff --git a/fluidx12_amd/csrc/fx_context.cpp b/fluidx12_amd/csrc/fx_context.cpp
--- a/fluidx12_amd/csrc/fx_context.cpp
+++ b/fluidx12_amd/csrc/fx_context.cpp
@@ -91,7 +91,7 @@
 		if (c->p[i]) (void)hipFree(c->p[i]);
 	}
 	void* others[] = { c->env, c->cube_depth, c->depth_own, c->accel.occ, c->accel.alpha, c->accel.bits, c->accel.list, c->accel.cells, c->accel.gi, c->accel.ctr, c->target, c->target_float, c->p_face[0], c->p_face[1], c->b, c->frozen, c->frozen_alt, c->lightmap, c->cube, c->sh_dev, c->halo_overflow, c->stage,
-		c->sh_scratch[0], c->sh_scratch[1], c->sh_scratch[2], c->sh_scratch[3], c->p_aux, c->fz_mask[0], c->fz_mask[1], c->fz_mask[2], c->fz_tile_next, c->fz_stat, c->fz_list[0], c->fz_list[1], c->fz_counts, c->sample_counters, c->adv_far, c->obst_code, c->obst_spare, c->obst_stats };
+		c->sh_scratch[0], c->sh_scratch[1], c->sh_scratch[2], c->sh_scratch[3], c->p_aux, c->fz_mask[0], c->fz_mask[1], c->fz_mask[2], c->fz_tile_next, c->fz_stat, c->fz_list[0], c->fz_list[1], c->fz_counts, c->sample_counters, c->adv_far, c->col_flags, c->obst_code, c->obst_spare, c->obst_stats };
 	for (void* q : others) if (q) (void)hipFree(q);
 	for (hipEvent_t e : c->ev) (void)hipEventDestroy(e);
 	if (c->step_rec) (void)hipFree(c->step_rec);
@@ -227,6 +227,13 @@
 					FX_HIP(hipMemsetAsync(ctx->adv_far, 0, 2 * sizeof(uint32_t), ctx->stream));
 					ctx->adv_far_words = words;
 				} else { (void)hipGetLastError(); ctx->adv_far = nullptr; }
+			}
+			const size_t fw = ctx->adv_far && !slab ? advect_flag_words(ctx->g) : 0;
+			if (fw) {
+				if (hipMalloc((void**)&ctx->col_flags, 2 * fw * sizeof(uint32_t)) == hipSuccess) {
+					FX_HIP(hipMemsetD32Async((hipDeviceptr_t)ctx->col_flags, 1, 2 * fw, ctx->stream));
+					ctx->col_flags_valid[0] = ctx->col_flags_valid[1] = true;
+				} else { (void)hipGetLastError(); ctx->col_flags = nullptr; }
 			}
 		}
 		if (d->grid_z > 1) {
@@ -459,6 +466,7 @@
 		}
 		char* dst = (char*)ctx->col[field == FX_FIELD_COLOR ? ctx->frame_parity : 1 - ctx->frame_parity];
 		if (ctx->accel_alpha_of == dst) ctx->accel_alpha_of = nullptr;
+		ctx->col_flags_valid[field == FX_FIELD_COLOR ? ctx->frame_parity : 1 - ctx->frame_parity] = false;
 		if ((rc = ensure_stage(ctx, need))) return rc;
 		FX_HIP(hipMemcpy(ctx->stage, host, need, hipMemcpyHostToDevice));
 		FX_HIP(launch_to_storage(ctx->stage, dst + off * 4 * es, 4 * n, ctx->half, ctx->stream));
@@ -601,6 +609,10 @@
 		if (value > 1) return FX_E_INVALID;
 		ctx->opt_render_accel = (int)value;
 		return FX_OK;
+	case FX_OPT_ADVECT_SPARSE:
+		if (value > 1) return FX_E_INVALID;
+		ctx->opt_advect_sparse = (int)value;
+		return FX_OK;
 	case FX_OPT_COUNT_SAMPLES: {
 		if (value > 1) return FX_E_INVALID;
 		DeviceGuard dgc(ctx->device);
diff --git a/fluidx12_amd/csrc/fx_context.h b/fluidx12_amd/csrc/fx_context.h
--- a/fluidx12_amd/csrc/fx_context.h
+++ b/fluidx12_amd/csrc/fx_context.h
@@ -40,6 +40,9 @@
 	bool adv_far_tried = false;
 	size_t adv_far_words = 0;
 	uint32_t adv_far_turn = 0;
+	uint32_t* col_flags = nullptr;
+	bool col_flags_valid[2] = { false, false };
+	int opt_advect_sparse = 1;
 	uint32_t fz_gen = 0;
 	uint32_t fz_gen_mark = 0;
 	std::vector<uint32_t> fz_iters;
diff --git a/fluidx12_amd/csrc/fx_internal.h b/fluidx12_amd/csrc/fx_internal.h
--- a/fluidx12_amd/csrc/fx_internal.h
+++ b/fluidx12_amd/csrc/fx_internal.h
@@ -48,13 +48,15 @@
 };
 
 struct AdvectAlpha { float* out; bool written; };
+struct AdvectSparse { uint32_t* flags; int src, dst; bool src_valid, dst_valid; bool used; };
 hipError_t launch_advect(const Geom& g, const SimParams& sp, int half_store, const void* vel_in, const void* col_in,
 	void* vel_out, void* col_out, int z_begin, int z_end, unsigned* halo_overflow, hipStream_t s, uint32_t* far_scratch = nullptr, size_t far_words = 0, int far_parity = 0, bool* far_used = nullptr,
-	AdvectAlpha* alpha = nullptr);
+	AdvectAlpha* alpha = nullptr, AdvectSparse* sparse = nullptr);
 hipError_t launch_advect_lds(const Geom& g, const SimParams& sp, int half_store, const void* vel_in, const void* col_in,
 	void* vel_out, void* col_out, int z_begin, int z_end, unsigned* halo_overflow, uint32_t* far_scratch, size_t far_words, int far_parity, bool* far_used, hipStream_t s, bool force,
-	AdvectAlpha* alpha = nullptr);
+	AdvectAlpha* alpha = nullptr, AdvectSparse* sparse = nullptr);
 size_t advect_far_words(const Geom& g, int nzp);
+size_t advect_flag_words(const Geom& g);
 hipError_t launch_confine_vorticity(const Geom& g, int half_store, const void* vel_in, void* vel_out, float eps, float dt, hipStream_t s);
 const int kEmitTileX = 64, kEmitTileY = 4;
 struct EmitBall { float c[3], rr, rate[4], force[3], swirl; int lo[3], hi[3]; };
diff --git a/fluidx12_amd/csrc/fx_schedule.cpp b/fluidx12_amd/csrc/fx_schedule.cpp
--- a/fluidx12_amd/csrc/fx_schedule.cpp
+++ b/fluidx12_amd/csrc/fx_schedule.cpp
@@ -97,8 +97,13 @@
 	ctx->rendered_since_step = false;
 	AdvectAlpha aa{ frame_was_rendered && ctx->accel_ok && ctx->opt_render_accel && FX_KNOB_INT("ADVECT_ALPHA", 1) ? ctx->accel.alpha : nullptr, false };
 	if (ctx->accel_alpha_of == ctx->col[par]) ctx->accel_alpha_of = nullptr;
+	AdvectSparse sx{ ctx->col_flags, 1 - par, par, ctx->col_flags_valid[1 - par], ctx->col_flags_valid[par], false };
+	const bool rewritten = sp.dt > 0.0f && (!ctx->emitters.empty() || (ctx->obst_code && ctx->obst_cells));
+	const bool sparse = ctx->opt_advect_sparse && ctx->col_flags && !ctx->group && !aa.out && !rewritten && r.lo == 0 && r.hi == g.Zg;
 	FX_HIP(launch_advect(g, sp, ctx->half, ctx->vel[0], ctx->col[1 - par], ctx->vel[1], ctx->col[par],
-		r.lo, r.hi, ctx->halo_overflow, s, lend ? ctx->adv_far : nullptr, lend ? ctx->adv_far_words : 0, (int)(ctx->adv_far_turn & 1u), &far_used, &aa));
+		r.lo, r.hi, ctx->halo_overflow, s, lend ? ctx->adv_far : nullptr, lend ? ctx->adv_far_words : 0, (int)(ctx->adv_far_turn & 1u), &far_used, &aa, sparse ? &sx : nullptr));
+	ctx->col_flags_valid[par] = sx.used;
+	if (sx.used) ctx->col_flags_valid[1 - par] = true;
 	if (aa.written) ctx->accel_alpha_of = ctx->col[par];
 	if (far_used) ++ctx->adv_far_turn;
 	return FX_OK;
@@ -246,6 +251,7 @@
 	const int par = ctx->frame_parity;
 	float* alpha = ctx->accel_alpha_of == ctx->col[par] ? ctx->accel.alpha : nullptr;
 	FX_HIP(launch_emit(ctx->g, ctx->half, ctx->vel[1], ctx->col[par], alpha, ctx->emitters.data(), (int)ctx->emitters.size(), ctx->time_step, s));
+	ctx->col_flags_valid[par] = false;
 	return FX_OK;
 }
 
@@ -257,6 +263,7 @@
 	const int par = ctx->frame_parity;
 	float* alpha = ctx->accel_alpha_of == ctx->col[par] ? ctx->accel.alpha : nullptr;
 	FX_HIP(launch_obstacle_enforce(ctx->g, ctx->half, ctx->obst_code, ctx->obst_lo, ctx->obst_hi, ctx->vel[1], ctx->col[par], alpha, s));
+	ctx->col_flags_valid[par] = false;
 	return FX_OK;
 }
 
diff --git a/fluidx12_amd/csrc/fx_sim.hip b/fluidx12_amd/csrc/fx_sim.hip
--- a/fluidx12_amd/csrc/fx_sim.hip
+++ b/fluidx12_amd/csrc/fx_sim.hip
@@ -780,10 +780,11 @@
 
 hipError_t launch_advect(const Geom& g, const SimParams& sp, int half_store, const void* vel_in, const void* col_in,
 	void* vel_out, void* col_out, int z_begin, int z_end, unsigned* halo_overflow, hipStream_t s, uint32_t* far_scratch, size_t far_words, int far_parity, bool* far_used,
-	AdvectAlpha* alpha)
+	AdvectAlpha* alpha, AdvectSparse* sparse)
 {
 	if (far_used) *far_used = false;
 	if (alpha) alpha->written = false;
+	if (sparse) sparse->used = false;
 	if (z_end <= z_begin) return hipSuccess;
 	int bx = 64, by = 4, bz = 1;
 	if (const char* e = FX_KNOB("ADVECT_BLOCK")) {
@@ -794,7 +795,7 @@
 	{
 		const char* le = FX_KNOB("ADVECT_LDS");
 		if (!(le && le[0] == '0') && bx == 64 && by == 4 && bz == 1 && !xcd_remap_on(REMAP_ADVECT)) {
-			const hipError_t e = launch_advect_lds(g, sp, half_store, vel_in, col_in, vel_out, col_out, z_begin, z_end, halo_overflow, far_scratch, far_words, far_parity, far_used, s, le && le[0] == '2', alpha);
+			const hipError_t e = launch_advect_lds(g, sp, half_store, vel_in, col_in, vel_out, col_out, z_begin, z_end, halo_overflow, far_scratch, far_words, far_parity, far_used, s, le && le[0] == '2', alpha, sparse);
 			if (e != hipErrorNotSupported) return e;
 		}
 	}
diff --git a/include/fluidx_hip.h b/include/fluidx_hip.h
--- a/include/fluidx_hip.h
+++ b/include/fluidx_hip.h
@@ -177,7 +177,7 @@
 
 int fx_comm_gather_color(fx_ctx* ctx, void* stream, fx_ctx* full, int root, const uint32_t* slab_z0, const uint32_t* slab_nz);
 
-enum fx_option { FX_OPT_OVERLAP = 1, FX_OPT_JACOBI_ROUND = 2, FX_OPT_ADAPTIVE_HALO = 3, FX_OPT_COUNT_SAMPLES = 4, FX_OPT_RENDER_ACCEL = 5 };
+enum fx_option { FX_OPT_OVERLAP = 1, FX_OPT_JACOBI_ROUND = 2, FX_OPT_ADAPTIVE_HALO = 3, FX_OPT_COUNT_SAMPLES = 4, FX_OPT_RENDER_ACCEL = 5, FX_OPT_ADVECT_SPARSE = 6 };
 int fx_set_option(fx_ctx* ctx, uint32_t option, uint32_t value);
 
 int fx_set_knob(const char* name, const char* value);
```

Result: slower. 22.16 billion (-1.9%).
